# Guillaume-SOULIER/SOS-Radiative-Transfer

Hardware: AMD Instinct MI355X
Metric: SOS columns/sec to 1e-4 convergence (Ntau=200, Nmu=128) (higher is better)
Workload: dtype f64

## Files before the change

__graft_entry__.py:

```python
import os
import subprocess
import sys

ROOT = os.path.dirname(os.path.abspath(__file__))
PKG = os.path.join(ROOT, "sos-radiative-transfer_amd")
CSRC = os.path.join(PKG, "csrc")
LIB = os.path.join(PKG, "libsosrt.so")
SOURCES = ["api.hip", "kernels.hip", "jn_gemm.hip", "jn_gemm_f32.hip", "transport_fast.hip", "transport_ring.hip", "transport_scan.hip", "order_loop.hip", "epilogue.hip", "plan.cpp", "comm.cpp"]
HEADERS = ["kernels.hpp", "plan.hpp", "transport_util.hpp", "transport_scan_body.hpp", "jn_gemm_tile.hpp", "comm.hpp", os.path.join(ROOT, "include", "sosrt.h")]


OBJDIR = os.path.join(PKG, "build")
FLAGS = ["-O3", "--offload-arch=gfx950", "-std=c++17", "-fPIC", "-Wno-unused-value"]


def _deps():
    return [h if os.path.isabs(h) else os.path.join(CSRC, h) for h in HEADERS]


def _obj(src):
    return os.path.join(OBJDIR, src + ".o")


def _obj_stale(src):
    o = _obj(src)
    if not os.path.exists(o):
        return True
    t = os.path.getmtime(o)
    return any(os.path.getmtime(d) > t for d in [os.path.join(CSRC, src)] + _deps())


def _stale():
    if not os.path.exists(LIB):
        return True
    t = os.path.getmtime(LIB)
    deps = [os.path.join(CSRC, s) for s in SOURCES] + _deps()
    return any(os.path.getmtime(d) > t for d in deps)


def _hipcc():
    return os.environ.get("HIPCC") or ("/opt/rocm/bin/hipcc" if os.path.exists("/opt/rocm/bin/hipcc") else "hipcc")


def build(force: bool = False) -> None:
    if force or _stale():
        import fcntl
        with open(os.path.join(PKG, ".build.lock"), "w") as lock:
            fcntl.flock(lock, fcntl.LOCK_EX)
            if force or _stale():
                os.makedirs(OBJDIR, exist_ok=True)
                extra = os.environ.get("SOSRT_CXXFLAGS", "").split()
                todo = [s for s in SOURCES if force or extra or _obj_stale(s)]
                procs = []
                for src in todo:
                    cmd = [_hipcc()] + FLAGS + extra + ["-c", src, "-o", _obj(src)]
                    print("[build]", " ".join(cmd), file=sys.stderr, flush=True)
                    procs.append((src, subprocess.Popen(cmd, cwd=CSRC)))
                bad = [src for src, p in procs if p.wait() != 0]
                if bad:
                    raise RuntimeError("hipcc failed for: " + ", ".join(bad))
                tmp = LIB + ".tmp.%d" % os.getpid()
                cmd = [_hipcc(), "--offload-arch=gfx950", "-shared", "-fPIC", "-o", tmp] + [_obj(s) for s in SOURCES] + ["-ldl"]
# ... 35 lines not shown
```

include/sosrt.h:

```cpp
#ifndef SOSRT_H
#define SOSRT_H

#ifdef __cplusplus
extern "C" {
#endif

typedef struct sosrt_handle sosrt_t;

#define SOSRT_OK              0
#define SOSRT_E_INVALID      -1
#define SOSRT_E_HIP          -2
#define SOSRT_E_STATE        -3
#define SOSRT_E_NOMEM        -4

#define SOSRT_COL_OK           0
#define SOSRT_COL_INDEXERROR   1
#define SOSRT_COL_MAXORDERS    2
#define SOSRT_COL_INTERNAL     3

#define SOSRT_GEOM_THREE_ZONE  0
#define SOSRT_GEOM_SINGLE_SLAB 1

#define SOSRT_SURFACE_NONE       0
#define SOSRT_SURFACE_SPECULAR   1
#define SOSRT_SURFACE_LAMBERTIAN 2
#define SOSRT_SURFACE_LAMBERTIAN_README 3

const char* sosrt_last_error(void);
#define SOSRT_VERSION 105
int sosrt_version(void);

int sosrt_create(int device, int L, int N, int max_batch, int max_orders, sosrt_t** out);
int sosrt_destroy(sosrt_t* h);
int sosrt_set_stream(sosrt_t* h, void* hip_stream);
int sosrt_use_own_stream(sosrt_t* h);
int sosrt_synchronize(sosrt_t* h);
int sosrt_set_saved_orders(sosrt_t* h, int slots);
int sosrt_set_order_budget(sosrt_t* h, int max_orders);

int sosrt_set_grid(sosrt_t* h, const double* mu);
int sosrt_set_phase(sosrt_t* h, const double* P_atm, const double* P_aer);

#define SOSRT_MAX_PHASE_SETS 64
int sosrt_set_phase_sets(sosrt_t* h, const double* P_atm, int S, const double* P_aer );
int sosrt_set_phase_sets_dev(sosrt_t* h, const double* P_atm , int S, const double* d_P_aer );
int sosrt_set_aerosol_sets(sosrt_t* h, int B, int nzmax, const int* zone_set );
int sosrt_phase_sets_info(sosrt_t* h, int* out );

int sosrt_set_atm_phase_sets(sosrt_t* h, int S_atm, const double* P_atm_sets );
int sosrt_set_atmosphere_sets(sosrt_t* h, int B, const int* col_set );
int sosrt_atm_sets_info(sosrt_t* h, int* out );

#define SOSRT_FIRST_ORDER_CODED 0
#define SOSRT_FIRST_ORDER_README 1
int sosrt_set_first_order(sosrt_t* h, int mode);

#define SOSRT_CONTRACT_F64 0
#define SOSRT_CONTRACT_F32 1
#define SOSRT_CONTRACT_F64_FULL 2
#define SOSRT_CONTRACT_F64_DENSE 3
#define SOSRT_SYMMETRY_TOL 1e-12
#define SOSRT_LOWRANK_TOL 1e-12
int sosrt_set_contraction(sosrt_t* h, int mode);

int sosrt_set_order_loop(sosrt_t* h, int mode);
int sosrt_order_loop_stats(sosrt_t* h, int* launches, int* refused, long long* column_orders );
int sosrt_phase_asymmetry(sosrt_t* h, double* asymmetry, int* uses_symmetry);
int sosrt_phase_rank(sosrt_t* h, int* rank, double* residual, int* uses);

int sosrt_set_columns(sosrt_t* h, int B, int geometry, int surface,
                      const int* idx_up, const int* idx_down,
                      const double* mu0, const double* grd_alb,
                      const double* alb_atm, const double* alb_aer,
                      const double* dtau_atm, const double* dtau_aer,
                      const double* tauStar_tot);

#define SOSRT_MAX_ZONES 8
int sosrt_set_columns_zones(sosrt_t* h, int B, int surface, int nzmax, const int* nz, const int* zone_r0, const int* zone_mix,
                            const double* mu0, const double* grd_alb, const double* alb_atm, const double* dtau_atm,
                            const double* zone_alb_aer, const double* zone_dtau_aer, const double* tauStar_tot);

int sosrt_first_order(sosrt_t* h, int B, const double* tau, const double* P0_atm, const double* P0_aer,
                      double* I1_out);
int sosrt_source(sosrt_t* h, int B, const double* In_1, double* Jn_out);
int sosrt_transport(sosrt_t* h, int B, const double* tau, const double* Jn, double* In_out, int* status_out);

int sosrt_solve(sosrt_t* h, int B, const double* tau, const double* P0_atm, const double* P0_aer,
                double tol, const double* I1_in,
                double* I_out, double* I_saved_out, int* n_orders_out, int* status_out);
int sosrt_solve_dev(sosrt_t* h, int B, const double* d_tau, const double* d_P0_atm, const double* d_P0_aer,
                    double tol, const double* d_I1_in,
                    double* d_I_out, double* d_I_saved_out, int* d_n_orders_out, int* d_status_out);
int sosrt_last_solve_stats(sosrt_t* h, int* max_orders_run, long long* sum_orders);

int sosrt_fluxes(sosrt_t* h, int B, const double* tau, const double* I, int beam_norm,
                 double* flux_down, double* flux_up);

int sosrt_epilogue_dev(sosrt_t* h, int B, const double* d_tau, const double* d_I, int beam_norm,
                       const double* d_z_profile, double* d_flux_down, double* d_flux_up, double* d_diffusivity,
                       double* d_heating_rate, double* d_net_toa);
int sosrt_epilogue(sosrt_t* h, int B, int beam_norm, const double* z_profile, double* flux_down, double* flux_up,
                   double* diffusivity, double* heating_rate, double* net_toa);

#define SOSRT_PHASE_ISO       0
#define SOSRT_PHASE_RAYLEIGH  1
#define SOSRT_PHASE_HG        2
#define SOSRT_PHASE_TABLE     3
int sosrt_phase_table(sosrt_t* h, const double* tab_mu, const double* tab_p, int ntab);
int sosrt_phase_table_dev(sosrt_t* h, const double* d_tab_mu, const double* d_tab_p, int ntab);

#define SOSRT_MIE_MAX_X 20000.0
#define SOSRT_MIE_MAX_MX 200000.0
#define SOSRT_MIE_MAX_WORKSPACE (2ull << 30)
int sosrt_mie_ensembles(sosrt_t* h, int S, const double* wl, const double* m_re, const double* m_im, const double* r_m,
                        const double* sig, int nb_radius, double r_min, double r_max, int ntab, double* p_out, double* bulk_out);
int sosrt_mie_ensembles_dev(sosrt_t* h, int S, const double* wl, const double* m_re, const double* m_im, const double* r_m,
                            const double* sig, int nb_radius, double r_min, double r_max, int ntab, double* d_p_out,
                            double* d_bulk_out);
int sosrt_mie_efficiencies(sosrt_t* h, int K, const double* m_re, const double* m_im, const double* x, double* out);
// ... 63 lines not shown
```

sos-radiative-transfer_amd/csrc/api.hip:

```cpp
#include <hip/hip_runtime.h>

#include <algorithm>
#include <cmath>
#include <cstdarg>
#include <cstdio>
#include <cstdlib>
#include <chrono>
#include <cstring>
#include <mutex>
#include <new>
#include <string>
#include <vector>

#include "../../include/sosrt.h"
#include "comm.hpp"
#include "kernels.hpp"
#include "plan.hpp"

using namespace sosrt;

namespace {
thread_local std::string g_err;

int fail(int code, const char* fmt, ...) {
// ... 111 lines not shown
    int mix_groups = 0;
    bool mix_dirty = true;
    double *d_Wmix = nullptr, *d_mixca = nullptr, *d_mixcr = nullptr;
    int* d_mixgroup = nullptr;
    int* d_slabtilegroup = nullptr;
    int contraction = SOSRT_CONTRACT_F64;
    double asymmetry = 0;
    bool sym_ok = false;
    bool sym_dirty = true, symmix_dirty = true, symsets_dirty = true;
    double *d_Wa_s = nullptr, *d_Wr_s = nullptr, *d_Wmix_s = nullptr;
    int lr_rank = -1;
    double lr_residual = 0;
    double *d_lrU = nullptr, *d_lrV = nullptr;
    size_t mixs_capacity = 0;
    float *d_Wa32 = nullptr, *d_Wmix32 = nullptr;
    size_t mix32_capacity = 0;
    bool w32_dirty = true;
    int* d_livelist = nullptr;
    size_t mix_capacity = 0;
    double *d_tau = nullptr, *d_P0a = nullptr, *d_P0r = nullptr;
    double *d_Jn = nullptr, *d_InA = nullptr, *d_InB = nullptr, *d_I = nullptr, *d_E = nullptr;
    int use_etab = 1;
    int *d_active = nullptr, *d_norders = nullptr, *d_status = nullptr, *d_redo = nullptr, *d_erep = nullptr;
    int *d_nactive_sets = nullptr, *d_nactive = nullptr;
    int nactive_set = 0;
    unsigned long long* d_tauhash = nullptr;
    int transport_mode = 3;
    int scan_cols = 200;
    bool ring_ok = false, scan_ok = false, scan_split_ok = false;
    int scan_split = 1;
    int cu_count = 0;
    double* d_scan_scratch = nullptr;
    int* d_scan_sync = nullptr;
    int gemm_tail_cols = 1 << 30;
    double gemm_tail_frac = 0.6;
    int gemm_small_cols = 200;
    int dense_live_list = 1;
    int gemm_regs_cols = -1;
    bool fast_ok = false;
    double* d_ratio = nullptr;
    int* h_pub = nullptr;
    bool need_small = true;
    int pub_seq = 0;
    int last_max_orders = 0;
    long long last_sum_orders = 0;
    Prof prof[kMaxGroups];
    int order_loop = 0;
    double ol_frac = 0.5;
    int* d_olsync = nullptr;
    int* h_oldone = nullptr;
    unsigned long long* d_ollog = nullptr;
    int ol_launches = 0, ol_refused = 0;
    bool ol_group_used[kMaxGroups] = {false, false};
    Rccl::comm_t comm = nullptr;
    int comm_rank = -1, comm_world = 0;
};

namespace {

size_t field_elems(const sosrt_handle* h) { return (size_t)h->max_batch * h->L * h->D; }

template <class T>
int dalloc(T** p, size_t n) {
    hipError_t e = hipMalloc((void**)p, n * sizeof(T));
    if (e != hipSuccess) return fail(SOSRT_E_NOMEM, "hipMalloc of %zu bytes failed: %s", n * sizeof(T), hipGetErrorString(e));
    return 0;
}

void mie_linspace(double a, double b, int n, double* out) {
    if (n == 1) { out[0] = a; return; }
    const double step = (b - a) / (n - 1);
    for (int i = 0; i < n; ++i) {
        volatile double t = i * step;
        out[i] = t + a;
    }
    out[n - 1] = b;
}

bool prof_room(Prof& p) {
    if (p.used + 2 > p.ev.size()) {
        const size_t n0 = p.ev.size();
        p.ev.resize(n0 + 4096);
        for (size_t i = n0; i < p.ev.size(); ++i)
            if (hipEventCreateWithFlags(&p.ev[i], hipEventDisableSystemFence) != hipSuccess) { p.ev.resize(i); break; }
        if (p.used + 2 > p.ev.size()) return false;
    }
    if (p.nint >= p.kind.size()) {
        const size_t n = p.kind.size() + 4096;
        p.kind.resize(n, -1); p.first.resize(n, 0); p.last.resize(n, 0);
    }
    return true;
}
hipStream_t group_stream(sosrt_handle* h, int grp) { return grp == 0 ? h->stream : h->stream2; }
void prof_begin(sosrt_handle* h, int kind, int grp = 0) {
    Prof& p = h->prof[grp];
    p.open = -1;
    if (!p.on || !prof_room(p)) return;
    if (p.adjacent >= 0) {
        p.open = p.adjacent;
    } else {
        p.open = (int)p.used++;
        hipEventRecord(p.ev[p.open], group_stream(h, grp));
    }
}
void prof_end(sosrt_handle* h, int kind, int grp = 0) {
    Prof& p = h->prof[grp];
// ... 138 lines not shown
}

int ensure_matrices(sosrt_handle* h, hipStream_t s) {
    const Grid& g = h->g;
    const size_t per = (size_t)g.Dp * g.Wld;
    const bool mixed = h->mix_groups > 0 && h->mix_dirty;
    if (mixed) {
        prof_break(h);
        const bool sets = h->max_set_used > 0, atm = h->max_atm_used > 0;
        launch_wmix(s, per, h->mix_groups, atm ? h->d_Wasets : h->d_Wa, sets ? h->d_Wrsets : h->d_Wr, h->d_mixca, h->d_mixcr,
                    h->d_Wmix, sets ? h->d_mixset : nullptr, atm ? h->d_mixatm : nullptr);
        h->mix_dirty = false;
        h->symmix_dirty = true;
    }
    if (!use_sym(h)) return 0;
    if (h->sym_dirty) {
        prof_break(h);
        if (!h->d_Wa_s) { if (int e = dalloc(&h->d_Wa_s, per)) return e; }
        if (!h->d_Wr_s) { if (int e = dalloc(&h->d_Wr_s, per)) return e; }
        launch_symfold(s, 1, g.N, g.D, g.Dp, g.Wld, h->d_Wa, h->d_Wa_s);
        launch_symfold(s, 1, g.N, g.D, g.Dp, g.Wld, h->d_Wr, h->d_Wr_s);
        h->sym_dirty = false;
        h->symsets_dirty = true;
    }
    if (h->symsets_dirty && h->nsets > 1 && h->mix_groups == 0 && h->max_set_used > 0) {
        prof_break(h);
        {
            if (per * h->nsets > h->wrsets_s_capacity) {
                if (h->d_Wrsets_s) hipFree(h->d_Wrsets_s);
                h->d_Wrsets_s = nullptr; h->wrsets_s_capacity = 0;
                if (int e = dalloc(&h->d_Wrsets_s, per * h->nsets)) return e;
                h->wrsets_s_capacity = per * h->nsets;
            }
            launch_symfold(s, h->nsets, g.N, g.D, g.Dp, g.Wld, h->d_Wrsets, h->d_Wrsets_s);
        }
        h->symsets_dirty = false;
    }
    if (h->mix_groups > 0 && h->symmix_dirty) {
        prof_break(h);
        const size_t need = per * h->mix_groups;
        if (need > h->mixs_capacity) {
            if (h->d_Wmix_s) hipFree(h->d_Wmix_s);
            h->d_Wmix_s = nullptr; h->mixs_capacity = 0;
            if (int e = dalloc(&h->d_Wmix_s, need)) return e;
            h->mixs_capacity = need;
        }
        launch_symfold(s, h->mix_groups, g.N, g.D, g.Dp, g.Wld, h->d_Wmix, h->d_Wmix_s);
        h->symmix_dirty = false;
    }
    return 0;
}

void run_source(sosrt_handle* h, const double* In_1, double* Jn, const int* active, int tail_cols = 0, int pub_tag = 0,
                int grp = -1, bool all_live = false, bool regs_tile = false, int dense_live_cap = 0) {
    const int g0 = grp < 0 ? 0 : grp, g1 = grp < 0 ? h->ngroups : grp + 1;
    const int pg = grp < 0 ? 0 : grp;
    hipStream_t s = group_stream(h, pg);
    GemmArgs ga;
    ga.A = In_1; ga.Wa = h->d_Wa; ga.Wr = h->d_Wr; ga.ca = h->d_rca; ga.cr = h->d_rcr;
    if (h->nslab > 0) {
        ga.rows_main = h->d_mainrows + h->main_off[g0];
        ga.n_main = h->main_off[g1] - h->main_off[g0];
    } else {
        ga.rows_main = nullptr;
        ga.n_main = (h->gb[g1] - h->gb[g0]) * h->L;
        ga.A = In_1 + (size_t)h->gb[g0] * h->L * h->D;
        Jn += (size_t)h->gb[g0] * h->L * h->D;
        ga.ca = h->d_rca + (size_t)h->gb[g0] * h->L;
        ga.cr = h->d_rcr + (size_t)h->gb[g0] * h->L;
        if (active) active += h->gb[g0];
    }
    ga.rows_slab = h->d_slabrows + h->slab_off[g0]; ga.n_slab = h->slab_off[g1] - h->slab_off[g0];
    ga.D = h->g.D; ga.Dp = h->g.Dp; ga.Wld = h->g.Wld; ga.L = h->L; ga.C = Jn; ga.active = active;
    if (grp >= 0 && h->ngroups > 1) ga.pad_lds = h->coresident_pad;
    if (pub_tag) {
        ga.nactive = h->d_nactive + pg; ga.need_small = h->d_nactive + sosrt_handle::kMaxGroups;
        ga.host_pub = h->h_pub + 8 * pg; ga.tag = pub_tag;
    }
    ga.check_tiles = all_live ? 0 : 1;
    if (ensure_matrices(h, s)) return;
    if (h->mix_groups > 0) {
        ga.Wmix = h->d_Wmix; ga.mix_group = h->d_mixgroup; ga.slab_tile_group = h->d_slabtilegroup + h->slab_off[g0] / 32;
    }
    const bool two_pass_sets = h->mix_groups == 0 && h->max_set_used > 0 && h->nslab > 0;
    if (two_pass_sets) {
        ga.Wr = h->d_Wrsets; ga.mix_group = h->d_mixgroup; ga.slab_tile_group = h->d_slabtilegroup + h->slab_off[g0] / 32;
    }
    if (use_lowrank(h)) { ga.lr_rank = h->lr_rank; ga.lrU = h->d_lrU; ga.lrV = h->d_lrV; }
    AtmSets at;
    const AtmSets* atp = nullptr;
    if (h->max_atm_used > 0) {
        at.col_atm = h->d_colatm + (h->nslab > 0 ? 0 : h->gb[g0]);
        at.lr_ranks = h->d_lrranks;
        ga.lrU = h->d_lrUsets; ga.lrV = h->d_lrVsets;
        atp = &at;
    }
    if (use_sym(h)) {
        ga.sym = 1; ga.Ks = (h->g.N + GEMM_KC - 1) / GEMM_KC * GEMM_KC;
#ifdef SOSRT_DIAG
        if (h->diag_ks_mult > 1 && ga.Ks * h->diag_ks_mult <= h->g.Dp) ga.Ks *= h->diag_ks_mult;
#endif
        ga.Wa = h->d_Wa_s; ga.Wr = two_pass_sets ? h->d_Wrsets_s : h->d_Wr_s;
        if (ga.Wmix) ga.Wmix = h->d_Wmix_s;
    }
    if (h->contraction == SOSRT_CONTRACT_F32) {
        if (h->w32_dirty) {
            prof_break(h);
            const size_t per = (size_t)h->g.Dp * h->g.Wld;
            launch_to_float(s, per, h->d_Wa, h->d_Wa32);
            if (h->mix_groups > 0) launch_to_float(s, per * h->mix_groups, h->d_Wmix, h->d_Wmix32);
            h->w32_dirty = false;
        }
        prof_begin(h, SOSRT_K_GEMM, pg);
        launch_gemm_f32(s, ga, h->d_Wa32, h->d_Wmix32);
        prof_end(h, SOSRT_K_GEMM, pg);
        return;
    }
    prof_begin(h, SOSRT_K_GEMM, pg);
    if (tail_cols > 0 && active && h->nslab >= 0) {
        ga.col0 = h->nslab > 0 ? h->gb[g0] : 0; ga.B = h->gb[g1] - h->gb[g0];
        ga.max_main = h->max_main; ga.max_slab = h->max_slab;
        ga.idx_up = h->nslab > 0 ? h->d_idx_up : nullptr; ga.idx_down = h->nslab > 0 ? h->d_idx_down : nullptr;
        ga.live_list = h->d_livelist + h->gb[g0]; ga.live_cap = tail_cols;
        launch_gemm_tail(s, ga, tail_cols, tail_cols <= h->gemm_small_cols, regs_tile, atp);
    } else {
        if (dense_live_cap > 0 && active && h->nslab >= 0) {
            ga.col0 = h->nslab > 0 ? h->gb[g0] : 0; ga.B = h->gb[g1] - h->gb[g0];
            ga.live_list = h->d_livelist + h->gb[g0]; ga.live_cap = dense_live_cap;
        }
        launch_gemm(s, ga, atp);
    }
    prof_end(h, SOSRT_K_GEMM, pg);
}

struct SolveShape {
    bool ring_like = false;
    bool fast = false;
    int nzcap = kRingZones;
    int ring_mode = 1;
};
SolveShape solve_shape(const sosrt_handle* h, int max_nz) {
    SolveShape sh;
    sh.ring_like = h->transport_mode >= 2 && h->ring_ok && (max_nz <= kRingZones || transport_ring_fits(h->g, max_nz));
    sh.fast = h->transport_mode >= 1 && h->fast_ok && (max_nz <= kRingZones || sh.ring_like);
    sh.nzcap = max_nz > kRingZones ? max_nz : kRingZones;
    sh.ring_mode = (h->transport_mode >= 2 && h->ring_ok) ? 3 : 1;
    return sh;
}
struct OrderInputs {
    int nb = 0;
    int known = 0;
    int surface = SOSRT_SURFACE_NONE;
    bool simple_zones = true;
    bool slabs_mixed = true;
    bool need_small = false;
    bool saving = false;
    int orders_left = 1 << 30;
    int cu_share = 0;
};
struct LaunchPlan {
    int tail_cols = 0;
    int live_cap = 0;
    int gemm = SOSRT_PLAN_GEMM_DENSE;
    int transport = SOSRT_PLAN_TRANSPORT_GENERAL;
    int parts = 1;
    int repair = 0;
    int order_loop = 0;
    int ol_parts = 0;
    int ol_grid = 0;
};
LaunchPlan plan_order(const sosrt_handle* h, const SolveShape& sh, const OrderInputs& in) {
    LaunchPlan pl;
    const Grid& g = h->g;
    const bool live_tiling = h->contraction != SOSRT_CONTRACT_F32 && in.simple_zones && in.known <= h->gemm_tail_cols &&
                             (in.known <= h->gemm_tail_frac * in.nb || in.nb <= h->gemm_small_cols) &&
                             (in.known < in.nb || in.nb <= h->gemm_small_cols);
    pl.tail_cols = live_tiling ? in.known : 0;
    pl.gemm = !live_tiling ? SOSRT_PLAN_GEMM_DENSE
                           : (pl.tail_cols <= h->gemm_small_cols ? ((use_sym(h) && pl.tail_cols <= 32) ? SOSRT_PLAN_GEMM_LIVE32_DEEP : SOSRT_PLAN_GEMM_LIVE32)
                                                                 : SOSRT_PLAN_GEMM_LIVE64);
    {
        const int nct = (g.D + GEMM_BN - 1) / GEMM_BN;
        const int auto_cap = (3 * h->cu_count / 2) / (((g.L + 15) / 16 + 1) * nct);
        const int cap = h->gemm_regs_cols >= 0 ? h->gemm_regs_cols : auto_cap;
        if (live_tiling && use_sym(h) && pl.tail_cols <= cap && 16 * (g.D + 2) * 8 <= 150 * 1024 &&
            ((g.N + GEMM_KC - 1) / GEMM_KC * GEMM_KC) % 64 == 0) pl.gemm = SOSRT_PLAN_GEMM_LIVE16_REGS;
    }
    pl.live_cap = live_tiling ? pl.tail_cols : ((h->contraction != SOSRT_CONTRACT_F32 && h->dense_live_list && in.known < in.nb) ? in.known : 0);
    {
        const int cols_now = pl.live_cap > 0 ? pl.live_cap : in.nb;
        const int split_cap = sh.ring_mode == 3 ? h->cu_count : 4 * h->cu_count;
        const bool can_split = h->scan_split && h->scan_split_ok && transport_scan_parts(g) * cols_now <= split_cap &&
                               (in.surface == SOSRT_SURFACE_SPECULAR || in.surface == SOSRT_SURFACE_NONE);
        const bool want_scan = h->transport_mode == 4 || (h->transport_mode == 3 && cols_now <= h->scan_cols);
        const bool split = can_split && transport_scan_fits(g, sh.nzcap, true) && (sh.fast || (h->use_etab && h->transport_mode >= 3));
        const bool scan = want_scan && ((sh.fast && sh.ring_mode == 3 && h->scan_ok && transport_scan_fits(g, sh.nzcap, false)) || split);
        pl.transport = scan ? SOSRT_PLAN_TRANSPORT_SCAN
                            : (!sh.fast ? SOSRT_PLAN_TRANSPORT_GENERAL : (sh.ring_mode == 3 ? SOSRT_PLAN_TRANSPORT_RING : SOSRT_PLAN_TRANSPORT_FAST));
        if (scan && split) pl.parts = transport_scan_parts(g);
        pl.repair = (h->N - 3 > 61 && pl.transport == SOSRT_PLAN_TRANSPORT_FAST) ? 1 : 0;
    }
    if (h->order_loop && in.cu_share > 0 && h->transport_mode == 3 && sh.fast && sh.ring_mode == 3 && sh.nzcap <= kRingZones &&
        use_sym(h) && in.simple_zones && in.slabs_mixed && !in.saving && !in.need_small && in.orders_left >= 1 &&
        in.known <= kOrderLoopMaxCols) {
        Grid gt = g;
        gt.nsmall = 0;
        const bool split_ok = h->scan_split && (in.surface == SOSRT_SURFACE_SPECULAR || in.surface == SOSRT_SURFACE_NONE) && order_loop_ok(gt, true);
        const int sp = order_loop_parts(gt, true);
        if (split_ok && sp * in.known <= h->ol_frac * in.cu_share) {
            pl.order_loop = 1; pl.ol_parts = sp;
        } else if (order_loop_ok(gt, false) && in.known <= h->ol_frac * in.cu_share) {
            pl.order_loop = 1; pl.ol_parts = 1;
        }
        if (pl.order_loop) pl.ol_grid = in.cu_share;
    }
    return pl;
}

std::mutex g_ol_mutex;
int g_ol_held[64];
int ol_acquire(int device, int total, int want, int least) {
    if (device < 0 || device >= 64) return 0;
    std::lock_guard<std::mutex> lk(g_ol_mutex);
    int got = total - g_ol_held[device];
    if (got > want) got = want;
    if (got < least || got <= 0) return 0;
    g_ol_held[device] += got;
    return got;
}
void ol_release(int device, int n) {
    if (device < 0 || device >= 64 || n <= 0) return;
    std::lock_guard<std::mutex> lk(g_ol_mutex);
    g_ol_held[device] -= n;
}

}

extern "C" {

const char* sosrt_last_error(void) { return g_err.c_str(); }
int sosrt_version(void) { return SOSRT_VERSION; }

int sosrt_plan_fix_count(double tau_ref, int N) { return fix_count(tau_ref, N); }

int sosrt_create(int device, int L, int N, int max_batch, int max_orders, sosrt_t** out) {
    if (!out) return fail(SOSRT_E_INVALID, "out is null");
    *out = nullptr;
    if (L < 2) return fail(SOSRT_E_INVALID, "nb_layers must be >= 2 (got %d)", L);
    if (N < 4) return fail(SOSRT_E_INVALID, "nb_angles must be >= 4 (got %d)", N);
    if (N > 1024) return fail(SOSRT_E_INVALID, "nb_angles must be <= 1024 (got %d)", N);
    if (max_batch < 1 || max_orders < 1) return fail(SOSRT_E_INVALID, "max_batch and max_orders must be >= 1");
    {
        const int nt = (N + 63) / 64 * 64;
        const size_t need = (size_t)(3 * (size_t)L + nt + nt / 64 + 4) * sizeof(double);
        if (need > 64 * 1024)
            return fail(SOSRT_E_INVALID, "nb_layers = %d does not fit: at most %d layers at nb_angles = %d", L,
                        (int)((64 * 1024 / sizeof(double) - nt - nt / 64 - 4) / 3), N);
    }
    sosrt_handle* h = new (std::nothrow) sosrt_handle();
    if (!h) return fail(SOSRT_E_NOMEM, "out of host memory");
    h->device = device; h->L = L; h->N = N; h->D = 2 * N; h->max_batch = max_batch; h->max_orders = max_orders;
    h->order_budget = max_orders;
    h->saved_slots = max_orders;
    h->gpu = device >= 0;
    h->cu_count = 256;
    if (const char* ev = getenv("SOSRT_ETAB")) h->use_etab = atoi(ev);
    if (const char* ev = getenv("SOSRT_CONTRACT"))
        if (strcmp(ev, "full") == 0) h->contraction = SOSRT_CONTRACT_F64_FULL;
    if (const char* ev = getenv("SOSRT_TRANSPORT"))
        h->transport_mode = strcmp(ev, "general") == 0 ? 0 : (strcmp(ev, "ring") == 0 ? 2 : (strcmp(ev, "scan") == 0 ? 4 : (strcmp(ev, "auto") == 0 ? 3 : 1)));
    if (const char* ev = getenv("SOSRT_SCAN_COLS")) h->scan_cols = atoi(ev);
    if (const char* ev = getenv("SOSRT_SCAN_SPLIT")) h->scan_split = atoi(ev);
    if (const char* ev = getenv("SOSRT_GEMM_TAIL")) h->gemm_tail_cols = atoi(ev);
    if (const char* ev = getenv("SOSRT_GEMM_TAIL_FRAC")) h->gemm_tail_frac = atof(ev);
    if (const char* ev = getenv("SOSRT_GEMM_SMALL")) h->gemm_small_cols = atoi(ev);
    if (const char* ev = getenv("SOSRT_DENSE_LIVE_LIST")) h->dense_live_list = atoi(ev) != 0;
    if (const char* ev = getenv("SOSRT_GEMM_REGS")) h->gemm_regs_cols = atoi(ev);
    if (const char* ev = getenv("SOSRT_GROUPS")) h->want_groups = atoi(ev) >= 2 ? 2 : (atoi(ev) == 1 ? 1 : 0);
    if (const char* ev = getenv("SOSRT_SPLIT_MIN")) h->split_min = atoi(ev);
    if (const char* ev = getenv("SOSRT_MIX_GROUPS")) h->mix_groups_max = atoi(ev);
#ifdef SOSRT_DIAG
    if (const char* ev = getenv("SOSRT_STAGGER")) h->stagger = atof(ev);
    if (const char* ev = getenv("SOSRT_GROUP_SPLIT")) h->split_at = atoi(ev);
    if (const char* ev = getenv("SOSRT_GROUP_PRIO")) h->prio2 = atoi(ev);
    if (const char* ev = getenv("SOSRT_GEMM_PAD_LDS")) h->coresident_pad = atoi(ev);
    if (const char* ev = getenv("SOSRT_GEMM_KS_MULT")) h->diag_ks_mult = atoi(ev);
#endif
    if (const char* ev = getenv("SOSRT_GROUP_RING_SLOTS")) h->coresident_slots = atoi(ev);
    if (const char* ev = getenv("SOSRT_ORDER_LOOP")) h->order_loop = atoi(ev) != 0;
    if (const char* ev = getenv("SOSRT_RING_SLOTS")) g_ring_slots = atoi(ev);
#ifdef SOSRT_RING_DEBUG
    if (const char* ev = getenv("SOSRT_RING_DEBUG")) g_ring_debug = atoi(ev);
#endif
    Grid& g = h->g;
    g.L = L; g.N = N; g.D = 2 * N;
    g.Dp = (g.D + GEMM_KC - 1) / GEMM_KC * GEMM_KC;
    g.Wld = (g.D + GEMM_BN - 1) / GEMM_BN * GEMM_BN;
    if (h->gpu) {
        int e = 0;
        auto body = [&]() -> int {
            HIPCHK(hipSetDevice(device));
            HIPCHK(hipStreamCreateWithFlags(&h->own_stream, hipStreamDefault));
            h->stream = h->own_stream;
            HIPCHK(hipEventCreateWithFlags(&h->ev_fork, hipEventDisableTiming));
            HIPCHK(hipEventCreateWithFlags(&h->ev_join, hipEventDisableTiming));
            const size_t mb = max_batch, fe = field_elems(h);
            if ((e = dalloc(&h->d_mu, g.D))) return e;
            if ((e = dalloc(&h->d_Wa, (size_t)g.Dp * g.Wld))) return e;
            if ((e = dalloc(&h->d_Wr, (size_t)g.Dp * g.Wld))) return e;
            if ((e = dalloc(&h->d_lrU, (size_t)kLowRankMax * g.D))) return e;
            if ((e = dalloc(&h->d_lrV, (size_t)kLowRankMax * g.D))) return e;
            if ((e = dalloc(&h->d_wfdn, N))) return e;
            if ((e = dalloc(&h->d_wfup, N))) return e;
            if ((e = dalloc(&h->d_w, g.D))) return e;
            if ((e = dalloc(&h->d_phi, 2 * kNPhi))) return e;
            if ((e = dalloc(&h->d_z, L))) return e;
            if ((e = dalloc(&h->d_fix, 4))) return e;
            if ((e = dalloc(&h->d_small, N))) return e;
            if ((e = dalloc(&h->d_idx_up, mb))) return e;
            if ((e = dalloc(&h->d_idx_down, mb))) return e;
            if ((e = dalloc(&h->d_nz, mb))) return e;
            if ((e = dalloc(&h->d_zr0, mb * kMaxZones))) return e;
            if ((e = dalloc(&h->d_zmix, mb * kMaxZones))) return e;
            if ((e = dalloc(&h->d_zwr, mb * kMaxZones))) return e;
            if ((e = dalloc(&h->d_zdtr, mb * kMaxZones))) return e;
            if ((e = dalloc(&h->d_scal, 7 * mb))) return e;
            if ((e = dalloc(&h->d_desc, mb))) return e;
            if ((e = dalloc(&h->d_rca, mb * L))) return e;
            if ((e = dalloc(&h->d_rcr, mb * L))) return e;
            if ((e = dalloc(&h->d_slabrows, mb * L + 64 * (size_t)sosrt_handle::kMaxMixGroupsSets * sosrt_handle::kMaxGroups))) return e;
            if ((e = dalloc(&h->d_slabtilegroup, mb * L / 32 + 2 * sosrt_handle::kMaxMixGroupsSets * sosrt_handle::kMaxGroups + 2))) return e;
            if ((e = dalloc(&h->d_mainrows, mb * L))) return e;
            if ((e = dalloc(&h->d_tau, mb * L))) return e;
            if ((e = dalloc(&h->d_P0a, mb * g.D))) return e;
            if ((e = dalloc(&h->d_P0r, mb * g.D))) return e;
            if ((e = dalloc(&h->d_Jn, fe))) return e;
            if ((e = dalloc(&h->d_InA, fe))) return e;
            if ((e = dalloc(&h->d_InB, fe))) return e;
            if ((e = dalloc(&h->d_I, fe))) return e;
            if ((e = dalloc(&h->d_E, fe))) return e;
            if ((e = dalloc(&h->d_active, mb))) return e;
            if ((e = dalloc(&h->d_norders, mb))) return e;
            if ((e = dalloc(&h->d_status, mb))) return e;
            if ((e = dalloc(&h->d_nactive_sets, 2 * (sosrt_handle::kMaxGroups + 1)))) return e;
            HIPCHK(hipMemset(h->d_nactive_sets, 0, 2 * (sosrt_handle::kMaxGroups + 1) * sizeof(int)));
            h->d_nactive = h->d_nactive_sets;
            if ((e = dalloc(&h->d_redo, mb))) return e;
            if ((e = dalloc(&h->d_erep, mb))) return e;
            if ((e = dalloc(&h->d_mixgroup, mb))) return e;
            if ((e = dalloc(&h->d_livelist, mb))) return e;
            if ((e = dalloc(&h->d_mixca, sosrt_handle::kMaxMixGroupsSets))) return e;
            if ((e = dalloc(&h->d_mixcr, sosrt_handle::kMaxMixGroupsSets))) return e;
            if ((e = dalloc(&h->d_mixset, sosrt_handle::kMaxMixGroupsSets))) return e;
            if ((e = dalloc(&h->d_mixatm, sosrt_handle::kMaxMixGroupsSets))) return e;
            if ((e = dalloc(&h->d_colatm, mb))) return e;
            if ((e = dalloc(&h->d_tauhash, mb))) return e;
            if ((e = dalloc(&h->d_ratio, mb))) return e;
            if ((e = dalloc(&h->d_scan_scratch, mb * transport_scan_scratch_doubles()))) return e;
            if ((e = dalloc(&h->d_scan_sync, 2 * mb))) return e;
            if ((e = dalloc(&h->d_olsync, sosrt_handle::kMaxGroups * order_loop_sync_ints(kOrderLoopMaxCols)))) return e;
            HIPCHK(hipHostMalloc((void**)&h->h_oldone, 2 * sosrt_handle::kMaxGroups * sizeof(int), hipHostMallocCoherent));
            memset(h->h_oldone, 0, 2 * sosrt_handle::kMaxGroups * sizeof(int));
            HIPCHK(hipMemset(h->d_scan_sync, 0, 2 * mb * sizeof(int)));
            HIPCHK(hipDeviceGetAttribute(&h->cu_count, hipDeviceAttributeMultiprocessorCount, device));
            HIPCHK(hipHostMalloc((void**)&h->h_pub, (8 * sosrt_handle::kMaxGroups + 2) * sizeof(int), hipHostMallocCoherent));
            memset(h->h_pub, 0, (8 * sosrt_handle::kMaxGroups + 2) * sizeof(int));

            HIPCHK(hipMemset(h->d_Wa, 0, (size_t)g.Dp * g.Wld * sizeof(double)));
            HIPCHK(hipMemset(h->d_Wr, 0, (size_t)g.Dp * g.Wld * sizeof(double)));
            HIPCHK(hipMemset(h->d_status, 0, mb * sizeof(int)));
            HIPCHK(hipMemset(h->d_redo, 0, mb * sizeof(int)));
            HIPCHK(hipMemset(h->d_tau, 0, mb * L * sizeof(double)));
            return 0;
        };
        if ((e = body())) { sosrt_destroy(h); return e; }
        g.mu = h->d_mu; g.Wa = h->d_Wa; g.Wr = h->d_Wr; g.fix = h->d_fix; g.small_lanes = h->d_small;
        g.wflux_dn = h->d_wfdn; g.wflux_up = h->d_wfup; g.nsmall = 0;
    }
    *out = h;
    return 0;
}

int sosrt_destroy(sosrt_t* h) {
    if (!h) return 0;
    if (h->gpu) {
        hipSetDevice(h->device);
        if (h->comm) { rccl().CommDestroy(h->comm); h->comm = nullptr; }
        if (h->own_stream) hipStreamSynchronize(h->own_stream);
        void* ptrs[] = {h->d_mu, h->d_Wa, h->d_Wr, h->d_wfdn, h->d_wfup, h->d_fix, h->d_small, h->d_idx_up,
                        h->d_idx_down, h->d_scal, h->d_desc, h->d_rca, h->d_rcr, h->d_slabrows, h->d_mainrows, h->d_tau, h->d_P0a,
                        h->d_P0r, h->d_Jn, h->d_InA, h->d_InB, h->d_I, h->d_E, h->d_active, h->d_norders, h->d_status,
                        h->d_nactive_sets, h->d_ratio, h->d_redo, h->d_erep, h->d_tauhash, h->d_Wmix, h->d_mixca, h->d_mixcr,
                        h->d_mixgroup, h->d_Wa_s, h->d_Wr_s, h->d_Wmix_s, h->d_scan_scratch, h->d_scan_sync, h->d_w, h->d_phi, h->d_z, h->d_tab, h->d_slabtilegroup, h->d_livelist, h->d_Wa32, h->d_Wmix32, h->d_nz, h->d_zr0, h->d_zmix, h->d_zwr, h->d_zdtr, h->d_olsync, h->d_ollog, h->d_modetab, h->d_lrU, h->d_lrV, h->d_Wrsets, h->d_Wrsets_s, h->d_mixset, h->d_P0rz,
                        h->d_Wasets, h->d_lrUsets, h->d_lrVsets, h->d_lrranks, h->d_colatm, h->d_mixatm};
        for (void* p : ptrs)
            if (p) hipFree(p);
        if (h->h_pub) hipHostFree(h->h_pub);
        if (h->h_oldone) hipHostFree(h->h_oldone);
        if (h->d_mie) hipFree(h->d_mie);
        if (h->h_mie) hipHostFree(h->h_mie);
        if (h->mie_ev) hipEventDestroy(h->mie_ev);
        for (auto& e : h->mie_t)
            if (e) hipEventDestroy(e);

        for (auto& p : h->prof)
            for (auto& e : p.ev) hipEventDestroy(e);
        if (h->stream2) { hipStreamSynchronize(h->stream2); hipStreamDestroy(h->stream2); }
        if (h->ev_fork) hipEventDestroy(h->ev_fork);
        if (h->ev_join) hipEventDestroy(h->ev_join);
        if (h->own_stream) hipStreamDestroy(h->own_stream);
    }
    delete h;
    return 0;
}

int sosrt_set_stream(sosrt_t* h, void* s) {
    if (int e = need_gpu(h)) return e;
    h->stream = (hipStream_t)s;
    return 0;
}

int sosrt_use_own_stream(sosrt_t* h) {
    if (int e = need_gpu(h)) return e;
    h->stream = h->own_stream;
    return 0;
}

int sosrt_set_saved_orders(sosrt_t* h, int slots) {
    if (!h) return fail(SOSRT_E_INVALID, "null handle");
    if (slots < 1 || slots > h->max_orders) return fail(SOSRT_E_INVALID, "slots must be in 1..max_orders=%d (got %d)", h->max_orders, slots);
    h->saved_slots = slots;
    return 0;
}

int sosrt_set_order_budget(sosrt_t* h, int max_orders) {
    if (!h) return fail(SOSRT_E_INVALID, "null handle");
    if (max_orders < 1 || max_orders > h->max_orders)
        return fail(SOSRT_E_INVALID, "the order budget must be in 1..max_orders=%d of sosrt_create (got %d)", h->max_orders, max_orders);
    h->order_budget = max_orders;
    return 0;
}

int sosrt_set_first_order(sosrt_t* h, int mode) {
    if (int e = need_gpu(h)) return e;
    if (mode != SOSRT_FIRST_ORDER_CODED && mode != SOSRT_FIRST_ORDER_README) return fail(SOSRT_E_INVALID, "unknown first-order mode %d", mode);
    if (mode == SOSRT_FIRST_ORDER_README && (h->nsets > 1 || h->p0_zones > 0))
        return fail(SOSRT_E_INVALID, "SOSRT_FIRST_ORDER_README reads one aerosol matrix: it cannot be combined with several phase sets");
    if (mode == SOSRT_FIRST_ORDER_README && (h->natm > 1 || h->max_atm_used > 0))
        return fail(SOSRT_E_INVALID, "SOSRT_FIRST_ORDER_README reads one atmosphere matrix: it cannot be combined with atmosphere phase sets");
    if (mode == SOSRT_FIRST_ORDER_README && h->geom != SOSRT_GEOM_THREE_ZONE)
        return fail(SOSRT_E_INVALID, "the README's Lambertian first order needs the three-zone geometry (it has a surface)");
    h->first_order_mode = mode;
    return 0;
}

int sosrt_set_contraction(sosrt_t* h, int mode) {
    if (int e = need_gpu(h)) return e;
    if (mode != SOSRT_CONTRACT_F64 && mode != SOSRT_CONTRACT_F32 && mode != SOSRT_CONTRACT_F64_FULL && mode != SOSRT_CONTRACT_F64_DENSE) return fail(SOSRT_E_INVALID, "unknown contraction mode %d", mode);
    if (mode != SOSRT_CONTRACT_F64 && (h->natm > 1 || h->max_atm_used > 0))
        return fail(SOSRT_E_INVALID, "atmosphere phase sets are in use: their plain rows exist in the low-rank form of SOSRT_CONTRACT_F64 only "
                                     "(the other contractions tile row lists that straddle columns)");
    if (mode == SOSRT_CONTRACT_F32) {
        HIPCHK(hipSetDevice(h->device));
        const size_t per = (size_t)h->g.Dp * h->g.Wld;
        if (!h->d_Wa32) { if (int e = dalloc(&h->d_Wa32, per)) return e; }
        h->w32_dirty = true;
    }
    h->contraction = mode;
    return 0;
}

int sosrt_set_order_loop(sosrt_t* h, int mode) {
    if (!h) return fail(SOSRT_E_INVALID, "null handle");
    if (mode < 0 || mode > 2) return fail(SOSRT_E_INVALID, "order-loop mode must be 0, 1 or 2 (got %d)", mode);
    h->order_loop = mode;
    return 0;
}

int sosrt_order_loop_stats(sosrt_t* h, int* launches, int* refused, long long* column_orders) {
    if (!h) return fail(SOSRT_E_INVALID, "null handle");
    if (launches) *launches = h->ol_launches;
    if (refused) *refused = h->ol_refused;
    if (column_orders) {
        *column_orders = 0;
        if (h->gpu && h->ol_launches > 0) {
            HIPCHK(hipSetDevice(h->device));
            HIPCHK(hipStreamSynchronize(h->stream));
            if (h->stream2) HIPCHK(hipStreamSynchronize(h->stream2));
            for (int k = 0; k < sosrt_handle::kMaxGroups; ++k) {
                if (!h->ol_group_used[k]) continue;
                int v = 0;
                HIPCHK(hipMemcpy(&v, h->d_olsync + (size_t)k * order_loop_sync_ints(kOrderLoopMaxCols) + kOlOrders, sizeof v, hipMemcpyDeviceToHost));
                *column_orders += v;
            }
        }
    }
    return 0;
}

int sosrt_plan_launch(sosrt_t* h, int batch, int live, int surface, int zones, int cus, int* out) {
    if (!h || !out) return fail(SOSRT_E_INVALID, "null argument");
    if (!h->have_grid) return fail(SOSRT_E_STATE, "sosrt_set_grid has not been called");
    if (batch < 1 || live < 0 || live > batch) return fail(SOSRT_E_INVALID, "need 0 <= live <= batch, batch >= 1");
    if (zones < 1 || zones > kMaxZones) return fail(SOSRT_E_INVALID, "zones must be in 1..%d", kMaxZones);
    int want = h->want_groups;
    if (want == 0) want = batch > h->split_min ? 2 : 1;
    const int ng = (want >= 2 && batch >= h->split_min && batch >= 2) ? 2 : 1;
    const int nb = ng == 2 ? batch / 2 : batch;
    const int saved_cus = h->cu_count;
    if (cus > 0) h->cu_count = cus;
    const SolveShape sh = solve_shape(h, zones);
    OrderInputs oi;
    oi.nb = nb; oi.known = live < nb ? live : nb; oi.surface = surface;
    oi.simple_zones = zones == 3 || zones == 1;
    oi.cu_share = h->cu_count / ng;
    const bool saved_sym = h->sym_ok;
    if (!h->have_phase) h->sym_ok = true;
    const LaunchPlan pl = plan_order(h, sh, oi);
    h->sym_ok = saved_sym;
    h->cu_count = saved_cus;
    out[0] = ng; out[1] = pl.gemm; out[2] = pl.tail_cols; out[3] = pl.transport; out[4] = pl.parts; out[5] = pl.repair;
    out[6] = pl.order_loop; out[7] = pl.ol_parts; out[8] = pl.ol_grid;
    return 0;
}

int sosrt_phase_asymmetry(sosrt_t* h, double* asymmetry, int* uses_symmetry) {
    if (!h) return fail(SOSRT_E_INVALID, "null handle");
    if (!h->have_phase) return fail(SOSRT_E_STATE, "sosrt_set_phase has not been called");
    if (asymmetry) *asymmetry = h->asymmetry;
    if (uses_symmetry) *uses_symmetry = use_sym(h) ? 1 : 0;
    return 0;
}

int sosrt_phase_rank(sosrt_t* h, int* rank, double* residual, int* uses) {
    if (!h) return fail(SOSRT_E_INVALID, "null handle");
    if (!h->have_phase) return fail(SOSRT_E_STATE, "sosrt_set_phase has not been called");
    if (rank) *rank = h->lr_rank;
    if (residual) *residual = h->lr_residual;
    if (uses) *uses = use_lowrank(h) ? 1 : 0;
    return 0;
}

int sosrt_synchronize(sosrt_t* h) {
    if (int e = need_gpu(h)) return e;
    HIPCHK(hipStreamSynchronize(h->stream));
    return 0;
}

int sosrt_set_grid(sosrt_t* h, const double* mu) {
// ... 279 lines not shown
    if (h->ngroups > 1 && !h->stream2) {
        HIPCHK(hipSetDevice(h->device));
        if (h->prio2) {
            int least = 0, greatest = 0;
            HIPCHK(hipDeviceGetStreamPriorityRange(&least, &greatest));
            HIPCHK(hipStreamCreateWithPriority(&h->stream2, hipStreamNonBlocking, h->prio2 > 0 ? greatest : least));
        } else {
            HIPCHK(hipStreamCreateWithFlags(&h->stream2, hipStreamNonBlocking));
        }
    }
    h->gb[0] = 0; h->gb[1] = h->ngroups == 2 ? ((h->split_at > 0 && h->split_at < B) ? h->split_at : B / 2) : B; h->gb[2] = B;
    for (int k = 0; k <= sosrt_handle::kMaxGroups; ++k) { h->main_off[k] = 0; h->slab_off[k] = 0; }
    h->max_nz = 1;
    h->simple_zones = true;
    if (geometry == SOSRT_GEOM_THREE_ZONE) {
        for (int b = 0; b < B; ++b) {
            h->max_nz = nz[b] > h->max_nz ? nz[b] : h->max_nz;
            const int* m = &zmix[b * kMaxZones];
            if (!(nz[b] == 3 && m[0] == 0 && m[1] == 1 && m[2] == 0)) h->simple_zones = false;
            if (nz[b] == 3) { iup[b] = zr0[b * kMaxZones + 1]; idn[b] = zr0[b * kMaxZones + 2] - 1; }
        }
        for (int k = 0; k < h->ngroups; ++k) {
            for (int b = h->gb[k]; b < h->gb[k + 1]; ++b)
                for (int z = 0; z < nz[b]; ++z)
                    for (int t = zr0[b * kMaxZones + z]; t <= zone_end(b, z); ++t) (zmix[b * kMaxZones + z] ? slab : plain).push_back(b * L + t);
            h->main_off[k + 1] = (int)plain.size();
            h->slab_off[k + 1] = (int)slab.size();
        }
    }
    for (int b = 0; b < B; ++b) {
        if (!(mu0[b] > 0)) return fail(SOSRT_E_INVALID, "column %d: mu0 must be > 0", b);
        sc[0 * mb + b] = mu0[b];
        sc[1 * mb + b] = grd_alb ? grd_alb[b] : 0.0;
        sc[2 * mb + b] = alb_atm[b];
        sc[4 * mb + b] = dtau_atm ? dtau_atm[b] : 1.0;
        sc[6 * mb + b] = tauStar_tot[b];
    }
    HIPCHK(hipSetDevice(h->device));
    HIPCHK(hipMemcpyAsync(h->d_scal, sc.data(), 7 * mb * sizeof(double), hipMemcpyHostToDevice, h->stream));
    if (geometry == SOSRT_GEOM_THREE_ZONE) {
        HIPCHK(hipMemcpyAsync(h->d_nz, nz.data(), B * sizeof(int), hipMemcpyHostToDevice, h->stream));
        HIPCHK(hipMemcpyAsync(h->d_zr0, zr0.data(), (size_t)B * kMaxZones * sizeof(int), hipMemcpyHostToDevice, h->stream));
        HIPCHK(hipMemcpyAsync(h->d_zmix, zmix.data(), (size_t)B * kMaxZones * sizeof(int), hipMemcpyHostToDevice, h->stream));
        HIPCHK(hipMemcpyAsync(h->d_zwr, zwr.data(), (size_t)B * kMaxZones * sizeof(double), hipMemcpyHostToDevice, h->stream));
        HIPCHK(hipMemcpyAsync(h->d_zdtr, zdtr.data(), (size_t)B * kMaxZones * sizeof(double), hipMemcpyHostToDevice, h->stream));
        HIPCHK(hipMemcpyAsync(h->d_idx_up, iup.data(), B * sizeof(int), hipMemcpyHostToDevice, h->stream));
        HIPCHK(hipMemcpyAsync(h->d_idx_down, idn.data(), B * sizeof(int), hipMemcpyHostToDevice, h->stream));
        if (!slab.empty())
            HIPCHK(hipMemcpyAsync(h->d_slabrows, slab.data(), slab.size() * sizeof(int), hipMemcpyHostToDevice, h->stream));
        if (!plain.empty())
            HIPCHK(hipMemcpyAsync(h->d_mainrows, plain.data(), plain.size() * sizeof(int), hipMemcpyHostToDevice, h->stream));
    }
    HIPCHK(hipStreamSynchronize(h->stream));
    h->nslab = (int)slab.size();
    h->nmain = (int)plain.size();
    h->max_main = L; h->max_slab = 0;
    if (geometry == SOSRT_GEOM_THREE_ZONE) {
        h->max_main = 0;
        for (int b = 0; b < B; ++b) {
            int ns = 0;
            for (int z = 0; z < nz[b]; ++z)
                if (zmix[b * kMaxZones + z]) ns += zone_end(b, z) - zr0[b * kMaxZones + z] + 1;
            h->max_slab = ns > h->max_slab ? ns : h->max_slab;
            h->max_main = L - ns > h->max_main ? L - ns : h->max_main;
        }
    }
    h->mix_groups = 0;
    h->mix_dirty = true;
    h->w32_dirty = true;
    h->max_set_used = 0;
    h->max_atm_used = 0;
    h->c_atmset.assign(B, 0);
    h->p0_zones = 0;
    h->c_nz = nz; h->c_zr0 = zr0; h->c_zmix = zmix; h->c_zwr = zwr; h->c_zdtr = zdtr;
    h->c_zset.assign((size_t)B * kMaxZones, 0);
    h->c_alb_atm.assign(alb_atm, alb_atm + B);
    h->c_dtau_atm.assign(B, 1.0);
    if (dtau_atm) h->c_dtau_atm.assign(dtau_atm, dtau_atm + B);
    if (geometry == SOSRT_GEOM_THREE_ZONE && h->nslab > 0) {
        MixGroups mg;
        if (collect_mix_groups(h, B, h->c_zset, h->c_atmset, mix_group_cap(h, false), mg))
            if (int e = apply_mix_groups(h, B, mg)) return e;
    }
    h->B = B; h->geom = geometry; h->surface = surface;
    h->have_cols = true;
    return 0;
}

int sosrt_set_columns(sosrt_t* h, int B, int geometry, int surface, const int* idx_up, const int* idx_down,
                      const double* mu0, const double* grd_alb, const double* alb_atm, const double* alb_aer,
                      const double* dtau_atm, const double* dtau_aer, const double* tauStar_tot) {
    if (int e = need_gpu(h)) return e;
    if (B < 1 || B > h->max_batch) return fail(SOSRT_E_INVALID, "B=%d outside 1..max_batch=%d", B, h->max_batch);
    if (!mu0 || !alb_atm || !tauStar_tot) return fail(SOSRT_E_INVALID, "mu0, alb_atm and tauStar_tot are required");
    std::vector<int> nz(B, 1), zr0((size_t)B * kMaxZones, 0), zmix((size_t)B * kMaxZones, 0);
    std::vector<double> zwr((size_t)B * kMaxZones, 0.0), zdtr((size_t)B * kMaxZones, 0.0);
    if (geometry == SOSRT_GEOM_THREE_ZONE) {
        if (!idx_up || !idx_down || !grd_alb || !alb_aer || !dtau_atm || !dtau_aer)
            return fail(SOSRT_E_INVALID, "three-zone geometry needs idx_up, idx_down, grd_alb, alb_aer, dtau_atm, dtau_aer");
        if (surface != SOSRT_SURFACE_SPECULAR && surface != SOSRT_SURFACE_LAMBERTIAN && surface != SOSRT_SURFACE_LAMBERTIAN_README)
            return fail(SOSRT_E_INVALID, "three-zone geometry needs a specular or lambertian surface");
        for (int b = 0; b < B; ++b) {
            if (idx_up[b] < 1 || idx_down[b] < idx_up[b] || idx_down[b] > h->L - 2)
                return fail(SOSRT_E_INVALID, "column %d: need 1 <= idx_up <= idx_down <= nb_layers-2 (got %d, %d)", b,
                            idx_up[b], idx_down[b]);
            nz[b] = 3;
// ... 377 lines not shown
    if (int e = ensure_w32(h)) return e;
    hipStream_t s = h->stream;
    const Grid& g = h->g;
    const size_t LD = (size_t)h->L * h->D;
    const size_t saved_stride = (size_t)h->saved_slots * LD;
    const int NG = h->ngroups;

    prof_break(h);
    h->nactive_set ^= 1;
    h->d_nactive = h->d_nactive_sets + h->nactive_set * (sosrt_handle::kMaxGroups + 1);
    SolveSetup su;
    su.zero_next = h->d_nactive_sets + (h->nactive_set ^ 1) * (sosrt_handle::kMaxGroups + 1);
    su.n_zero = sosrt_handle::kMaxGroups + 1;
    su.redo = h->d_redo;
    su.hash = h->d_tauhash;
    su.scan_sync = h->d_scan_sync;
    launch_prepare(s, g, B, h->geom, h->surface, scalars_of(h), d_tau, h->d_desc, h->d_rca, h->d_rcr,
                   h->d_nactive + sosrt_handle::kMaxGroups, su);
    h->need_small = true;
    const int small_tag = ((++h->pub_seq) & 0x3fffffff) | 0x40000000;
    bool small_published = false;
    const SolveShape shape = solve_shape(h, h->max_nz);
    const bool fast = shape.fast;
    const int nzcap = shape.nzcap;
    if (h->use_etab || fast) {
        launch_tau_groups(s, g, B, d_tau, h->d_tauhash, h->d_erep, h->d_nactive + sosrt_handle::kMaxGroups,
                          h->h_pub + 8 * sosrt_handle::kMaxGroups, small_tag);
        launch_attenuation(s, g, B, d_tau, h->d_E, h->d_erep);
        small_published = true;
    }
    if (int e = ensure_matrices(h, s)) return e;
    bool forked = false;
    int ol_held[sosrt_handle::kMaxGroups] = {0, 0};
    auto bail = [&](int code) {
        if (forked && hipEventRecord(h->ev_join, h->stream2) == hipSuccess) (void)hipStreamWaitEvent(s, h->ev_join, 0);
        for (int k = 0; k < NG; ++k)
            if (ol_held[k]) {
                (void)hipStreamSynchronize(group_stream(h, k));
                ol_release(h->device, ol_held[k]);
                ol_held[k] = 0;
            }
        return code;
    };

    struct GroupState {
        int b0 = 0, nb = 0, n = 1, known = 0;
        bool done = false, started = false;
        bool ol_pending = false, ol_off = false;
        int ol_tag = 0;
        unsigned ol_polls = 0;
        double *In_1 = nullptr, *In = nullptr;
        Conv cv;
    } gs[sosrt_handle::kMaxGroups];
    h->ol_launches = 0; h->ol_refused = 0;
    for (bool& u : h->ol_group_used) u = false;
    bool used_order_loop = false;
    const int tagbase = ((++h->pub_seq) & 0x3fff) << 16;
    for (int k = 0; k < NG; ++k) {
        GroupState& q = gs[k];
        q.b0 = h->gb[k]; q.nb = h->gb[k + 1] - h->gb[k]; q.known = q.nb;
        q.In_1 = h->d_InA; q.In = h->d_InB;
        if (!d_I1_in && h->first_order_mode != SOSRT_FIRST_ORDER_README) q.In_1 = d_I_out;
        q.cv = make_conv(h, tol);
        q.cv.active += q.b0; q.cv.norders += q.b0; q.cv.status += q.b0; q.cv.ratio += q.b0; q.cv.redo += q.b0;
        q.cv.nactive = h->d_nactive + k;
        if (h->d_targets) q.cv.target = h->d_targets + q.b0;
    }
    auto start_group = [&](int k) {
        GroupState& q = gs[k];
        q.started = true;
        hipStream_t sg = group_stream(h, k);
        const size_t fo = (size_t)q.b0 * LD;
        prof_begin(h, SOSRT_K_FIRST, k);
        if (d_I1_in)
            hipLaunchKernelGGL(k_init_from_I1, dim3(q.nb), dim3(256), 0, sg, g, d_I1_in + fo, q.In_1 + fo, d_I_out + fo,
                               d_I_saved_out ? d_I_saved_out + (size_t)q.b0 * saved_stride : nullptr, saved_stride, q.cv);
        else if (h->first_order_mode == SOSRT_FIRST_ORDER_README)
            launch_first_order_readme(sg, g, h->d_w, q.nb, d_tau + (size_t)q.b0 * h->L, d_P0_atm + (size_t)q.b0 * g.D,
                                      d_P0_aer ? d_P0_aer + (size_t)q.b0 * g.D : nullptr, h->d_desc + q.b0, q.In_1 + fo,
                                      d_I_out + fo, d_I_saved_out ? d_I_saved_out + (size_t)q.b0 * saved_stride : nullptr,
                                      saved_stride, q.cv, 1);
        else
            launch_first_order(sg, g, q.nb, d_tau + (size_t)q.b0 * h->L, d_P0_atm + (size_t)q.b0 * g.D,
                               d_P0_aer ? d_P0_aer + (size_t)q.b0 * g.D * (h->p0_zones > 0 ? h->p0_zones : 1) : nullptr, h->d_desc + q.b0,
                               d_I_out + fo, nullptr, d_I_saved_out ? d_I_saved_out + (size_t)q.b0 * saved_stride : nullptr, saved_stride,
                               q.cv, 1, h->p0_zones);
        prof_end(h, SOSRT_K_FIRST, k);
    };
    start_group(0);
    if (NG > 1) {
        HIPCHK(hipEventRecord(h->ev_fork, s));
        HIPCHK(hipStreamWaitEvent(h->stream2, h->ev_fork, 0));
        forked = true;
    }
    if (small_published && g.nsmall > 0) {
        volatile int* slot = h->h_pub + 8 * sosrt_handle::kMaxGroups;
        const auto t0 = std::chrono::steady_clock::now();
        for (unsigned it = 1; __atomic_load_n(&slot[1], __ATOMIC_ACQUIRE) != small_tag; ++it) {
            if ((it & 0x3fff) == 0 && std::chrono::steady_clock::now() - t0 > std::chrono::seconds(120))
                return bail(fail(SOSRT_E_HIP, "order loop: no progress for 120 s"));
            __builtin_ia32_pause();
        }
        h->need_small = slot[0] != 0;
    }
    int live_groups = NG, n_max = 1;
    while (live_groups > 0) {
        bool progressed = false;
// ... 19 lines not shown
                if (h->d_ollog && getenv("SOSRT_OL_LOG")) {
                    std::vector<unsigned long long> lg(65001);
                    (void)hipStreamSynchronize(group_stream(h, k));
                    (void)hipMemcpy(lg.data(), h->d_ollog, lg.size() * 8, hipMemcpyDeviceToHost);
                    if (FILE* f = fopen(getenv("SOSRT_OL_LOG"), "a")) {
                        fprintf(f, "# launch columns<=%d order0=%d events=%llu\n", q.known, q.n + 1, lg[0]);
                        for (unsigned long long i = 0; i < lg[0] && i < 65000; ++i)
                            fprintf(f, "%llu %llu %llu %llu\n", lg[1 + i] >> 48, (lg[1 + i] >> 40) & 0xff, (lg[1 + i] >> 32) & 0xff, lg[1 + i] & 0xffffffffull);
                        fclose(f);
                    }
                }
#endif
                if (state == kOlReady) { q.done = true; --live_groups; h->ol_group_used[k] = true; continue; }
                if (state == kOlAborted) {
                    std::vector<int> w(order_loop_sync_ints(q.known < 6 ? q.known : 6));
                    (void)hipStreamSynchronize(group_stream(h, k));
                    (void)hipMemcpy(w.data(), h->d_olsync + (size_t)k * order_loop_sync_ints(kOrderLoopMaxCols), w.size() * sizeof(int), hipMemcpyDeviceToHost);
                    std::string cols;
                    for (int c = 0; c < (q.known < 6 ? q.known : 6); ++c) {
                        char buf[96];
                        const int* cs = w.data() + kOlCols + c * kOlColStride;
                        snprintf(buf, sizeof buf, " [%d: orders %d stop %d tiles %d]", c, cs[kOlOrdDone], cs[kOlColStop], cs[kOlJnDone]);
                        cols += buf;
                    }
                    return bail(fail(SOSRT_E_HIP, "order loop: a workgroup of the order-loop launch gave up waiting (arrived %d, left %d, order %d on, %d columns:%s)",
                                     w[kOlArrive], w[kOlLeft], q.n + 1, q.known, cols.c_str()));
                }
                q.ol_off = true;
                ++h->ol_refused;
            }
            if (!q.started) {
                const GroupState& p = gs[k - 1];
                if (!(p.done || (p.n >= 2 && p.known <= h->stagger * p.nb))) continue;
                start_group(k);
            }
            progressed = true;
            if (q.n >= h->order_budget) { q.done = true; --live_groups; continue; }
            if (q.n >= 2) {
                const int live = wait_published(h, k, tagbase + q.n - 1);
                if (live < 0) return bail(live);
                if (live == 0) { q.done = true; --live_groups; continue; }
                q.known = live;
            }
            hipStream_t sg = group_stream(h, k);
            const size_t fo = (size_t)q.b0 * LD;
            const double* tau_g = d_tau + (size_t)q.b0 * h->L;
            const int* erep_g = h->d_erep + q.b0;
            OrderInputs oi;
            oi.nb = q.nb; oi.known = q.known; oi.surface = h->surface;
            oi.simple_zones = h->simple_zones; oi.slabs_mixed = h->nslab == 0 || h->mix_groups > 0;
            oi.need_small = g.nsmall > 0 && h->need_small; oi.saving = d_I_saved_out != nullptr;
            oi.orders_left = h->order_budget - q.n;
            oi.cu_share = (q.ol_off || h->d_targets || h->max_atm_used > 0) ? 0 : h->cu_count / NG;
            LaunchPlan pl = plan_order(h, shape, oi);
            if (pl.order_loop) {
                const int got = ol_acquire(h->device, h->cu_count, pl.ol_grid, (int)(pl.ol_parts * q.known / h->ol_frac));
                if (got == 0) { oi.cu_share = 0; pl = plan_order(h, shape, oi); }
                else { pl.ol_grid = got; ol_held[k] = got; }
            }
            if (pl.order_loop && h->order_loop == 2) pl.ol_grid = 2 * h->cu_count;
            if (pl.order_loop) {
                OrderLoopArgs oa;
                Grid gt = g;
                gt.nsmall = 0;
                oa.t = TransportArgs{gt, tau_g, h->d_Jn + fo, nullptr, d_I_out + fo, nullptr, 0, h->d_desc + q.b0, q.cv, 0, 1, h->d_E, erep_g, nullptr};
                oa.t.nzcap = kRingZones;
                oa.t.scan_split = pl.ol_parts > 1 ? 1 : 0;
                oa.t.scan_scratch = h->d_scan_scratch + (size_t)q.b0 * transport_scan_scratch_doubles();
                oa.t.scan_sync = h->d_scan_sync + 2 * q.b0;
                GemmArgs& ga = oa.gm;
                ga.A = nullptr; ga.Wa = h->d_Wa_s; ga.Wr = h->d_Wr_s; ga.ca = h->d_rca; ga.cr = h->d_rcr;
                ga.D = g.D; ga.Dp = g.Dp; ga.Wld = g.Wld; ga.L = h->L; ga.C = h->d_Jn;
                ga.sym = 1; ga.Ks = (g.N + GEMM_KC - 1) / GEMM_KC * GEMM_KC;
                if (use_lowrank(h)) { ga.lr_rank = h->lr_rank; ga.lrU = h->d_lrU; ga.lrV = h->d_lrV; }
                ga.max_main = h->max_main; ga.max_slab = h->max_slab;
                ga.idx_up = h->nslab > 0 ? h->d_idx_up : nullptr; ga.idx_down = h->nslab > 0 ? h->d_idx_down : nullptr;
                if (h->mix_groups > 0) { ga.Wmix = h->d_Wmix_s; ga.mix_group = h->d_mixgroup; }
                oa.in0 = q.In_1;
                oa.gbufP = q.In;
                oa.gbufQ = (q.In_1 == d_I_out) ? h->d_InA : q.In_1;
                oa.bufP = oa.gbufP + fo; oa.bufQ = oa.gbufQ + fo;
                oa.order0 = q.n + 1; oa.kmax = h->order_budget - q.n;
                oa.B = q.nb; oa.col0 = q.b0;
                oa.fixcap = (int)(0.06 * g.N) + 1;
                oa.sync = h->d_olsync + (size_t)k * order_loop_sync_ints(kOrderLoopMaxCols);
                oa.host_done = h->h_oldone + 2 * k;
                oa.tag = q.ol_tag = ((++h->pub_seq) & 0x3fffffff) | 0x40000000;
#ifdef SOSRT_OL_STAMPS
                if (getenv("SOSRT_OL_LOG")) {
                    if (!h->d_ollog) { if (int e = dalloc(&h->d_ollog, 65001)) return bail(e); }
                    HIPCHK(hipMemsetAsync(h->d_ollog, 0, 8, sg));
                    oa.log = h->d_ollog;
                }
#endif
                prof_break(h);
                HIPCHK(hipMemsetAsync(oa.sync, 0, order_loop_sync_ints(q.known) * sizeof(int), sg));
                prof_begin(h, SOSRT_K_ORDER_LOOP, k);
                const hipError_t le = launch_order_loop(sg, pl.ol_grid, pl.ol_parts > 1, oa);
                prof_end(h, SOSRT_K_ORDER_LOOP, k);
                if (le != hipSuccess) return bail(fail(SOSRT_E_HIP, "order-loop launch failed: %s", hipGetErrorString(le)));
                q.ol_pending = true;
                used_order_loop = true;
                ++h->ol_launches;
                continue;
            }
            const int n = ++q.n;
            n_max = n > n_max ? n : n_max;
            const int tail_cols = pl.tail_cols;
            run_source(h, q.In_1, h->d_Jn, h->d_active, tail_cols, tagbase + n - 1, k, q.known == q.nb, pl.gemm == SOSRT_PLAN_GEMM_LIVE16_REGS,
                       tail_cols > 0 ? 0 : pl.live_cap);
            if (g.nsmall > 0 && h->need_small) {
                prof_begin(h, SOSRT_K_SMALLMU, k);
                launch_smallmu(sg, g, q.nb, tau_g, h->d_Jn + fo, q.In + fo, h->d_desc + q.b0, q.cv.active);
                prof_end(h, SOSRT_K_SMALLMU, k);
            }
            prof_begin(h, SOSRT_K_TRANSPORT, k);
            double* sv_n = (d_I_saved_out && n <= h->saved_slots) ? d_I_saved_out + (size_t)q.b0 * saved_stride + (size_t)(n - 1) * LD : nullptr;
            if (pl.transport != SOSRT_PLAN_TRANSPORT_GENERAL) {
                Grid gt = g;
                if (pl.transport >= SOSRT_PLAN_TRANSPORT_RING && !h->need_small) gt.nsmall = 0;
                launch_transport(sg, gt, q.nb, tau_g, h->d_Jn + fo, q.In + fo, d_I_out + fo, sv_n, saved_stride, h->d_desc + q.b0, q.cv, n, 1,
                                 h->d_E, pl.transport, erep_g, pl.live_cap, h->d_livelist + q.b0, NG > 1 ? h->coresident_slots : 0,
                                 pl.parts > 1 ? 1 : 0, h->d_scan_scratch + (size_t)q.b0 * transport_scan_scratch_doubles(),
                                 h->d_scan_sync + 2 * q.b0, nzcap);
                if (pl.repair)
                    launch_transport(sg, g, q.nb, tau_g, h->d_Jn + fo, q.In + fo, d_I_out + fo, sv_n, saved_stride, h->d_desc + q.b0, q.cv, n, 1,
                                     h->d_E, 2, erep_g);
            } else {
                launch_transport(sg, g, q.nb, tau_g, h->d_Jn + fo, q.In + fo, d_I_out + fo, sv_n, saved_stride, h->d_desc + q.b0, q.cv, n, 1,
                                 h->use_etab ? h->d_E : nullptr, 0, erep_g);
            }
            prof_end(h, SOSRT_K_TRANSPORT, k);
            if (q.In_1 == d_I_out) { q.In_1 = q.In; q.In = h->d_InA; }
            else { double* tmp = q.In_1; q.In_1 = q.In; q.In = tmp; }
        }
        if (!progressed) __builtin_ia32_pause();
    }
    if (NG > 1) {
        HIPCHK(hipEventRecord(h->ev_join, h->stream2));
        HIPCHK(hipStreamWaitEvent(s, h->ev_join, 0));
    }
    prof_break(h);
    launch_finalize(s, B, make_conv(h, tol), h->order_budget, d_n_orders_out, d_status_out);
    HIPCHK(hipGetLastError());
    h->last_max_orders = used_order_loop ? -1 : n_max;
    h->last_sum_orders = -1;
    return 0;
}

int sosrt_solve(sosrt_t* h, int B, const double* tau, const double* P0_atm, const double* P0_aer, double tol,
                const double* I1_in, double* I_out, double* I_saved_out, int* n_orders_out, int* status_out) {
    if (int e = check_ready(h, B, true)) return e;
    if (!tau) return fail(SOSRT_E_INVALID, "null argument");
    HIPCHK(hipSetDevice(h->device));
    hipStream_t s = h->stream;
    h->resident = false;
    const size_t LD = (size_t)h->L * h->D, n = (size_t)B * LD;
    HIPCHK(hipMemcpyAsync(h->d_tau, tau, (size_t)B * h->L * sizeof(double), hipMemcpyHostToDevice, s));
    if (P0_atm) HIPCHK(hipMemcpyAsync(h->d_P0a, P0_atm, (size_t)B * h->D * sizeof(double), hipMemcpyHostToDevice, s));
    const double* d_p0r = nullptr;
    if (int e = stage_p0_aer(h, B, P0_aer, s, &d_p0r)) return e;
    double* d_I1 = nullptr;
    double* d_saved = nullptr;
    int rc = 0;
    auto body = [&]() -> int {
        if (I1_in) {
            if (int e = dalloc(&d_I1, n)) return e;
            HIPCHK(hipMemcpyAsync(d_I1, I1_in, n * sizeof(double), hipMemcpyHostToDevice, s));
        }
        if (I_saved_out) {
            if (int e = dalloc(&d_saved, (size_t)B * h->saved_slots * LD)) return e;
            HIPCHK(hipMemsetAsync(d_saved, 0, (size_t)B * h->saved_slots * LD * sizeof(double), s));
        }
        if (int e = sosrt_solve_dev(h, B, h->d_tau, P0_atm ? h->d_P0a : nullptr, d_p0r, tol, d_I1,
                                    h->d_I, d_saved, nullptr, nullptr))
            return e;
        if (I_out) HIPCHK(hipMemcpyAsync(I_out, h->d_I, n * sizeof(double), hipMemcpyDeviceToHost, s));
// ... 792 lines not shown
```

sos-radiative-transfer_amd/csrc/jn_gemm_tile.hpp:

```cpp
#pragma once
#include "kernels.hpp"
#include "transport_util.hpp"

namespace sosrt {

namespace {

typedef double f64x4 __attribute__((ext_vector_type(4)));

constexpr int A_LD = GEMM_KC + 2;
constexpr int B_LD = GEMM_BN + 16;

struct ListRows {
    const int* rows;
    int n;
    __device__ int operator()(int lr) const { return lr < n ? (rows ? rows[lr] : lr) : -1; }
};
struct ColumnRows {
    int base, iu, ns, n;
    bool slab;
    __device__ int operator()(int lr) const {
        if (lr >= n) return -1;
        return base + (slab ? iu + lr : (lr < iu ? lr : lr + ns));
    }
};

template <int RT, bool SLAB, bool DEEP = false, bool SYM = false, class RowOf = ListRows, bool COH = false, bool ASTAGE = false>
__device__ __forceinline__ void gemm_tile(const GemmArgs& g, double* sA, double* sB, int* s_any, int tile, int bn0,
                                          RowOf row_of, bool check_active, const double* __restrict__ wmix = nullptr,
                                          double* sRaw = nullptr) {
    static_assert(!ASTAGE || (COH && DEEP), "ASTAGE is a form of the order-loop launch's tile");
    constexpr int BM = 16 * RT;
    double* const sAv = sA + BM * A_LD;
    const int Nn = g.D >> 1, Nh = g.Wld >> 1;
    int tid_ = threadIdx.x;
    if (COH) asm volatile("" : "+v"(tid_));
    const int tid = tid_, lane = tid & 63;
    const int wave = __builtin_amdgcn_readfirstlane(tid) >> 6;
    const int D = g.D, Dp = g.Dp, Wld = g.Wld;
    constexpr bool slab = SLAB;
    const int bm0 = tile * BM;

    const int arow = tid >> 2, akq = (tid & 3) * (GEMM_KC / 4);
    int grow = -1;
    if (arow < BM) grow = row_of(bm0 + arow);
    if (check_active && g.active && g.check_tiles) {
        if (tid == 0) *s_any = 0;
        __syncthreads();
        if ((tid & 3) == 0 && grow >= 0 && g.active[grow / g.L]) *s_any = 1;
        __syncthreads();
        if (!*s_any) return;
    }
    __shared__ int s_rowid[16 * (GEMM_RT > 2 ? GEMM_RT : 2)];
    if ((tid & 3) == 0 && arow < BM) s_rowid[arow] = grow;
// ... 323 lines not shown
        const int r = rows[i] >= 0 ? rows[i] : rows[0];
        const int bytes = rows[i] >= 0 ? D * 8 : 0;
        rA[i] = make_rsrc(g.A + (size_t)r * D, bytes);
        rC[i] = make_rsrc(g.C + (size_t)r * D, bytes);
        cf[i] = rows[i] >= 0 ? g.ca[rows[i]] : 0.0;
        if constexpr (ATM) {
            const int st = __builtin_amdgcn_readfirstlane(at.col_atm[r / g.L]);
            Ri[i] = __builtin_amdgcn_readfirstlane(at.lr_ranks[st]);
            Ui[i] = g.lrU + (size_t)st * kLowRankMax * D;
            Vi[i] = g.lrV + (size_t)st * kLowRankMax * D;
        }
    }
    const double* __restrict__ U = g.lrU;
    const double* __restrict__ V = g.lrV;
    double m[LR_ROWS][kLowRankMax];
#pragma unroll
    for (int i = 0; i < LR_ROWS; ++i)
#pragma unroll
        for (int q = 0; q < kLowRankMax; ++q) m[i][q] = 0.0;
#pragma unroll 2
    for (int k = 2 * lane; k < D; k += 128) {
        double2 x[LR_ROWS];
#pragma unroll
        for (int i = 0; i < LR_ROWS; ++i) x[i] = bload2_aux<COH ? 16 : 0>(rA[i], k * 8, 0);
#pragma unroll
        for (int q = 0; q < kLowRankMax; ++q) {
            if constexpr (ATM) {
#pragma unroll
                for (int i = 0; i < LR_ROWS; ++i)
                    if (q < Ri[i]) {
                        const double2 u = *reinterpret_cast<const double2*>(Ui[i] + (size_t)q * D + k);
                        m[i][q] = __builtin_fma(x[i].y, u.y, __builtin_fma(x[i].x, u.x, m[i][q]));
                    }
            } else if (q < R) {
                const double2 u = *reinterpret_cast<const double2*>(U + (size_t)q * D + k);
#pragma unroll
                for (int i = 0; i < LR_ROWS; ++i) m[i][q] = __builtin_fma(x[i].y, u.y, __builtin_fma(x[i].x, u.x, m[i][q]));
            }
        }
    }
#pragma unroll
    for (int s = 32; s >= 1; s >>= 1)
#pragma unroll
        for (int q = 0; q < kLowRankMax; ++q) {
            if constexpr (ATM) {
#pragma unroll
                for (int i = 0; i < LR_ROWS; ++i)
                    if (q < Ri[i]) m[i][q] += __shfl_xor(m[i][q], s);
            } else if (q < R) {
#pragma unroll
                for (int i = 0; i < LR_ROWS; ++i) m[i][q] += __shfl_xor(m[i][q], s);
            }
        }
#pragma unroll 2
    for (int k = 2 * lane; k < D; k += 128) {
        double2 o[LR_ROWS];
#pragma unroll
        for (int i = 0; i < LR_ROWS; ++i) o[i] = make_double2(0.0, 0.0);
#pragma unroll
        for (int q = 0; q < kLowRankMax; ++q) {
            if constexpr (ATM) {
#pragma unroll
                for (int i = 0; i < LR_ROWS; ++i)
                    if (q < Ri[i]) {
                        const double2 v = *reinterpret_cast<const double2*>(Vi[i] + (size_t)q * D + k);
                        o[i].x = __builtin_fma(m[i][q], v.x, o[i].x);
                        o[i].y = __builtin_fma(m[i][q], v.y, o[i].y);
                    }
            } else if (q < R) {
                const double2 v = *reinterpret_cast<const double2*>(V + (size_t)q * D + k);
#pragma unroll
                for (int i = 0; i < LR_ROWS; ++i) {
                    o[i].x = __builtin_fma(m[i][q], v.x, o[i].x);
                    o[i].y = __builtin_fma(m[i][q], v.y, o[i].y);
                }
            }
        }
#pragma unroll
        for (int i = 0; i < LR_ROWS; ++i) bstore2_aux<COH ? 17 : 0>(rC[i], k * 8, 0, make_double2(cf[i] * o[i].x, cf[i] * o[i].y));
    }
}
template <bool COH, class RowOf, bool ATM = false>
__device__ __forceinline__ void lowrank_tile(const GemmArgs& g, RowOf row_of, int tile, int BM, int bn0, bool check_active,
                                             const AtmSets& at = AtmSets()) {
    const int nct = (g.D + GEMM_BN - 1) / GEMM_BN, ct = bn0 / GEMM_BN;
    const int lane = threadIdx.x & 63, wave = __builtin_amdgcn_readfirstlane(threadIdx.x) >> 6;
    const int per = (BM - ct + nct - 1) / nct;
    const bool chk = check_active && g.active && g.check_tiles;
    for (int j = LR_ROWS * wave; j < per; j += 4 * LR_ROWS) {
        int rows[LR_ROWS];
        int n = 0;
#pragma unroll
        for (int i = 0; i < LR_ROWS; ++i) {
            int r = j + i < per ? __builtin_amdgcn_readfirstlane(row_of(tile * BM + ct + nct * (j + i))) : -1;
            if (chk && r >= 0 && !g.active[r / g.L]) r = -1;
            rows[i] = r;
            n += r >= 0 ? 1 : 0;
        }
        if (n == 0) continue;
        if (rows[0] < 0)
#pragma unroll
            for (int i = 1; i < LR_ROWS; ++i)
                if (rows[i] >= 0) { rows[0] = rows[i]; rows[i] = -1; break; }
        lowrank_rows<COH, ATM>(g, rows, lane, at);
    }
}

constexpr int TAIL_RT_SLAB = 1;
constexpr int TAIL_RT = 2;

}
}
```

sos-radiative-transfer_amd/csrc/kernels.hip:

```cpp
#include <cstdlib>

#include "kernels.hpp"

#include "../../include/sosrt.h"

namespace sosrt {


typedef double f64x4 __attribute__((ext_vector_type(4)));

#define SOSRT_PI 3.14159265358979323846

__device__ __forceinline__ double wave_fmax(double v) {
#pragma unroll
    for (int o = 32; o > 0; o >>= 1) v = fmax(v, __shfl_xor(v, o, 64));
    return v;
}
__device__ __forceinline__ double wave_sum(double v) {
#pragma unroll
    for (int o = 32; o > 0; o >>= 1) v += __shfl_xor(v, o, 64);
    return v;
}

__device__ double block_pymax(double x, bool valid, double* s_red, int first_tid = 0) {
// ... 957 lines not shown
            bool same = true;
            for (int i = lane; i < L; i += 64) same = same && (tb[i] == tc[i]);
            if (__ballot(!same) == 0) rep = cc;
        }
    }
    if (lane == 0) erep[b] = rep;
}
void launch_tau_groups(hipStream_t s, const Grid& g, int B, const double* tau, unsigned long long* hash, int* erep,
                       const int* need_small, int* host_flag, int tag) {
    hipLaunchKernelGGL(k_tau_rep, dim3(B), dim3(64), 0, s, g.L, tau, hash, erep, need_small, host_flag, tag);
}

template <int MAXT>
static void launch_transport_t(hipStream_t s, dim3 grid, dim3 block, size_t shm, const TransportArgs& a, int mode) {
    if (mode == 1) {
        launch_transport_fast(s, grid, block, a);
    } else if (mode == 3) {
        launch_transport_ring(s, grid, a, g_ring_slots);
    } else if (mode == 4) {
        launch_transport_scan(s, grid, a);
    } else if (mode == 2) {
        if (a.accumulate) {
            if (a.saved) hipLaunchKernelGGL((k_transport<MAXT, true, true, true, true>), grid, block, shm, s, a);
            else hipLaunchKernelGGL((k_transport<MAXT, true, false, true, true>), grid, block, shm, s, a);
        } else {
            hipLaunchKernelGGL((k_transport<MAXT, false, false, true, true>), grid, block, shm, s, a);
        }
    } else if (a.accumulate) {
        if (a.Etab) {
            if (a.saved) hipLaunchKernelGGL((k_transport<MAXT, true, true, true>), grid, block, shm, s, a);
            else hipLaunchKernelGGL((k_transport<MAXT, true, false, true>), grid, block, shm, s, a);
        } else {
            if (a.saved) hipLaunchKernelGGL((k_transport<MAXT, true, true, false>), grid, block, shm, s, a);
            else hipLaunchKernelGGL((k_transport<MAXT, true, false, false>), grid, block, shm, s, a);
        }
    } else {
        if (a.Etab) hipLaunchKernelGGL((k_transport<MAXT, false, false, true>), grid, block, shm, s, a);
        else hipLaunchKernelGGL((k_transport<MAXT, false, false, false>), grid, block, shm, s, a);
    }
}

unsigned long long* g_transport_stamps = nullptr;
int g_ring_slots = 3, g_ring_debug = 0;

bool transport_fast_ok(const Plan& plan) {
    for (int bkt = 0; bkt < 4; ++bkt)
        if (plan.fix[bkt].idx > 0 && (plan.fix[bkt].s0 >> 6) != ((plan.N - 1) >> 6)) return false;
    return true;
}

void launch_transport(hipStream_t s, const Grid& g, int B, const double* tau, const double* Jn, double* In, double* I,
                      double* saved, size_t saved_col_stride, const ColDesc* desc, Conv cv, int order,
                      int accumulate, const double* Etab, int mode, const int* erep, int live, const int* live_list,
                      int ring_slots, int scan_split, double* scan_scratch, int* scan_sync, int nzcap) {
    const int nt = round64(g.N);
    const size_t shm = (size_t)(g.L + 2 * TC * (nt + 2) + 2 * nt + nt / 64 + 2) * sizeof(double);
    TransportArgs a{g, tau, Jn, In, I, accumulate ? saved : nullptr, saved_col_stride, desc, cv, order, accumulate, Etab, Etab ? erep : nullptr, g_transport_stamps};
    a.slots = ring_slots;
    a.nzcap = nzcap > kRingZones ? nzcap : kRingZones;
    if (mode == 4 && scan_split && scan_scratch && scan_sync) { a.scan_split = 1; a.scan_scratch = scan_scratch; a.scan_sync = scan_sync; }
    if ((mode == 3 || mode == 4) && accumulate && live > 0 && live < B && live_list) {
        a.live = live;
        a.live_list = live_list;
        B = live;
    }
    if (nt <= 128) launch_transport_t<128>(s, dim3(B), dim3(nt), shm, a, mode);
    else if (nt <= 256) launch_transport_t<256>(s, dim3(B), dim3(nt), shm, a, mode);
    else if (nt <= 512) launch_transport_t<512>(s, dim3(B), dim3(nt), shm, a, mode);
    else launch_transport_t<1024>(s, dim3(B), dim3(nt), shm, a, mode);
}

__global__ void k_finalize(int B, Conv cv, int max_orders, int* __restrict__ n_out, int* __restrict__ status_out) {
    const int b = blockIdx.x * blockDim.x + threadIdx.x;
    if (b >= B) return;
    int st = cv.status[b];
    if (cv.active[b]) { st = SOSRT_COL_MAXORDERS; cv.status[b] = st; }
    if (n_out) n_out[b] = cv.norders[b];
    if (status_out) status_out[b] = st;
}
void launch_finalize(hipStream_t s, int B, Conv cv, int max_orders, int* n_out, int* status_out) {
    hipLaunchKernelGGL(k_finalize, dim3((B + 127) / 128), dim3(128), 0, s, B, cv, max_orders, n_out, status_out);
}

__global__ void k_fluxes(Grid g, int B, const double* __restrict__ tau_all, const double* __restrict__ I_all,
                         const ColDesc* __restrict__ desc, int beam_norm, double* __restrict__ fdn,
                         double* __restrict__ fup) {
    const int row = blockIdx.x * (blockDim.x >> 6) + (threadIdx.x >> 6);
    if (row >= B * g.L) return;
    const int lane = threadIdx.x & 63, b = row / g.L, t = row % g.L;
    const double* I = I_all + (size_t)row * g.D;
    double sd = 0, su = 0;
    for (int k = lane; k < g.N; k += 64) {
        sd += g.wflux_dn[k] * I[k];
        su += g.wflux_up[k] * I[g.N + k];
    }
    sd = wave_sum(sd);
    su = wave_sum(su);
    if (lane == 0) {
        const ColDesc& d = desc[b];
        const double* tau = tau_all + (size_t)b * g.L;
        const double F0 = SOSRT_PI / d.mu0;
        const double fb = beam_norm ? F0 : F0 / (4 * SOSRT_PI);
        fdn[row] = sd - fb * exp(-tau[t] / d.mu0);
        fup[row] = su + fb * d.rho * exp(-(2 * tau[g.L - 1] - tau[t]) / d.mu0);
    }
}
void launch_fluxes(hipStream_t s, const Grid& g, int B, const double* tau, const double* I, const ColDesc* desc,
                   int beam_norm, double* fdn, double* fup) {
    const int rows = B * g.L;
    hipLaunchKernelGGL(k_fluxes, dim3((rows + 3) / 4), dim3(256), 0, s, g, B, tau, I, desc, beam_norm, fdn, fup);
}

// ... 103 lines not shown
```

sos-radiative-transfer_amd/csrc/kernels.hpp:

```cpp
#pragma once
#include <hip/hip_runtime.h>

#include "plan.hpp"

namespace sosrt {

constexpr int kMaxZones = 8;
constexpr int kRingZones = 3;

struct alignas(16) ColDesc {
    int nz;
    int r0[kMaxZones];
    int r1[kMaxZones];
    int mix[kMaxZones];
    int nfix[kMaxZones];
    int fixtab[kMaxZones];
    int surface;
    int geom;
    double mu0, rho, T, tau_bottom;
    double wa;
    double wr[kMaxZones];
    double fa[kMaxZones];
    double fr[kMaxZones];
    double ca[kMaxZones];
// ... 35 lines not shown
    const double* wflux_dn;
    const double* wflux_up;
};

struct Conv {
    int* active;
    int* norders;
    int* status;
    int* nactive;
    double* ratio;
    int* redo;
    const int* target;
    double tol;
};

__device__ __forceinline__ bool conv_go(const Conv& cv, int b, int order, double r) {
    return cv.target ? order < cv.target[b] : r >= cv.tol;
}

constexpr int GEMM_BM = 64, GEMM_BN = 128, GEMM_KC = 16;
#ifndef SOSRT_GEMM_RT
#define SOSRT_GEMM_RT 4
#endif
#ifndef SOSRT_GEMM_WPS
#define SOSRT_GEMM_WPS 3
#endif
constexpr int GEMM_RT = SOSRT_GEMM_RT;
constexpr int GEMM_WPS = SOSRT_GEMM_WPS;

constexpr int TC = 8;

struct TransportArgs {
    Grid g;
    const double* tau;
    const double* Jn;
    double* In;
    double* I;
    double* saved;
    size_t saved_col_stride;
    const ColDesc* desc;
    Conv cv;
    int order;
    int accumulate;
    const double* Etab;
    const int* erep;
    unsigned long long* stamps;
    int live = 0;
    const int* live_list = nullptr;
    int slots = 0;
    int nzcap = kRingZones;
    int scan_split = 0;
    double* scan_scratch = nullptr;
    int* scan_sync = nullptr;
};
void launch_transport_fast(hipStream_t s, dim3 grid, dim3 block, const TransportArgs& a);
bool transport_ring_ok(const Grid& g);
bool transport_ring_fits(const Grid& g, int nzcap);
void launch_transport_ring(hipStream_t s, dim3 grid, const TransportArgs& a, int slots);
bool transport_scan_ok(const Grid& g);
bool transport_scan_split_ok(const Grid& g);
bool transport_scan_fits(const Grid& g, int nzcap, bool split);
int transport_scan_parts(const Grid& g);
size_t transport_scan_scratch_doubles();
void launch_transport_scan(hipStream_t s, dim3 grid, const TransportArgs& a);
constexpr int kOrderLoopMaxCols = 256;
constexpr int kOlArrive = 0, kOlState = 32, kOlLeft = 64, kOlAbort = 96, kOlOrders = 100, kOlCols = 128;
constexpr int kOlColStride = 64, kOlOrdDone = 0, kOlColStop = 1, kOlJnDone = 32;
constexpr int kOlReady = 1, kOlNotResident = 2, kOlAborted = 3;
inline size_t order_loop_sync_ints(int cols) { return (size_t)kOlCols + (size_t)cols * kOlColStride; }
extern int g_ring_slots, g_ring_debug;
extern unsigned long long* g_transport_stamps;

struct SolveSetup {
    int* zero_next = nullptr;
    int n_zero = 0;
    int* redo = nullptr;
    unsigned long long* hash = nullptr;
    int* scan_sync = nullptr;
};
void launch_prepare(hipStream_t s, const Grid& g, int B, int geom, int surface, ColScalars sc, const double* tau,
                    ColDesc* desc, double* rowcoef_a, double* rowcoef_r, int* need_small = nullptr, SolveSetup su = SolveSetup());
void launch_first_order_readme(hipStream_t s, const Grid& g, const double* w, int B, const double* tau, const double* P0a,
                               const double* P0r, const ColDesc* desc, double* I1_out, double* I_out, double* saved,
                               size_t saved_col_stride, Conv cv, int do_conv);
void launch_first_order(hipStream_t s, const Grid& g, int B, const double* tau, const double* P0a, const double* P0r,
                        const ColDesc* desc, double* I1_out, double* I_out, double* saved, size_t saved_col_stride,
                        Conv cv, int do_conv, int p0r_zones = 0 );
struct GemmArgs {
    const double* A;
    const double* Wa;
    const double* Wr;
    const double* ca;
    const double* cr;
    const int* rows_main;
    int n_main;
    const int* rows_slab;
    int n_slab;
    int D, Dp, Wld, L;
    double* C;
    const int* active;
    int B = 0;
    int col0 = 0;
    const int* idx_up = nullptr;
    const int* idx_down = nullptr;
    int max_main = 0, max_slab = 0;
    const double* Wmix = nullptr;
    const int* mix_group = nullptr;
    int pad_lds = 0;
    int* live_list = nullptr;
    int live_cap = 0;
    const int* slab_tile_group = nullptr;
    const int* nactive = nullptr;
    const int* need_small = nullptr;
    int* host_pub = nullptr;
    int tag = 0;
    int sym = 0;
    int Ks = 0;
    int check_tiles = 1;
    int lr_rank = -1;
    const double* lrU = nullptr;
    const double* lrV = nullptr;
};
struct AtmSets {
    const int* col_atm = nullptr;
    const int* lr_ranks = nullptr;
};
constexpr int kLowRankMax = 4;

__device__ inline void publish_live_now(const GemmArgs& g) {
    const int live = __hip_atomic_load(g.nactive, __ATOMIC_RELAXED, __HIP_MEMORY_SCOPE_AGENT);
    int* slot = g.host_pub + 4 * (g.tag & 1);
    __hip_atomic_store(slot, live, __ATOMIC_RELAXED, __HIP_MEMORY_SCOPE_SYSTEM);
    __hip_atomic_store(slot + 2, g.need_small ? g.need_small[0] : 1, __ATOMIC_RELAXED, __HIP_MEMORY_SCOPE_SYSTEM);
    __hip_atomic_store(slot + 1, g.tag, __ATOMIC_RELEASE, __HIP_MEMORY_SCOPE_SYSTEM);
}
__device__ inline void publish_live(const GemmArgs& g) {
    if (g.host_pub && blockIdx.x == 0 && blockIdx.y == 0 && threadIdx.x == 0) publish_live_now(g);
}
struct PerDeviceOnce {
    bool seen[64] = {};
    bool first() {
        int d = 0;
        if (hipGetDevice(&d) != hipSuccess || d < 0 || d >= 64) return true;
        if (seen[d]) return false;
        seen[d] = true;
        return true;
    }
};
void launch_gemm(hipStream_t s, const GemmArgs& a, const AtmSets* at = nullptr);
struct OrderLoopArgs {
    TransportArgs t;
    GemmArgs gm;
    const double* in0;
    double* gbufP;
    double* gbufQ;
    double* bufP;
    double* bufQ;
    int order0;
    int kmax;
    int B, col0;
    int fixcap;
    int* sync;
    int* host_done;
    int tag;
    unsigned long long* log = nullptr;
    int astage = 0;
};
bool order_loop_ok(const Grid& g, bool split);
int order_loop_parts(const Grid& g, bool split);
hipError_t launch_order_loop(hipStream_t s, int grid, bool split, const OrderLoopArgs& p);
void launch_gemm_f32(hipStream_t s, const GemmArgs& a, const float* Wa32, const float* Wmix32);
void launch_to_float(hipStream_t s, size_t n, const double* src, float* dst);
void launch_wmix(hipStream_t s, size_t n, int ngroups, const double* Wa, const double* Wr, const double* ca, const double* cr,
                 double* Wmix, const int* gset = nullptr ,
                 const int* gatm = nullptr );
void launch_fold_sets(hipStream_t s, int S, int D, int Wld, size_t per, const double* w, const double* P, double* W);
void launch_fold_asymmetry(hipStream_t s, int S, int nblk, int D, int Wld, size_t per, const double* W, double* out);
void launch_symfold(hipStream_t s, int nmat, int N, int D, int Dp, int Wld, const double* W, double* SA);
void launch_gemm_tail(hipStream_t s, const GemmArgs& a, int cols, bool small_tiles, bool regs = false, const AtmSets* at = nullptr);
void launch_smallmu(hipStream_t s, const Grid& g, int B, const double* tau, const double* Jn, double* In,
                    const ColDesc* desc, const int* active);
void launch_transport(hipStream_t s, const Grid& g, int B, const double* tau, const double* Jn, double* In, double* I,
                      double* saved, size_t saved_col_stride, const ColDesc* desc, Conv cv, int order, int accumulate,
                      const double* Etab, int mode, const int* erep = nullptr, int live = 0, const int* live_list = nullptr,
                      int ring_slots = 0, int scan_split = 0, double* scan_scratch = nullptr, int* scan_sync = nullptr,
                      int nzcap = kRingZones);
bool transport_fast_ok(const Plan& plan);
void launch_attenuation(hipStream_t s, const Grid& g, int B, const double* tau, double* Etab, const int* erep);
void launch_tau_groups(hipStream_t s, const Grid& g, int B, const double* tau, unsigned long long* hash, int* erep,
                       const int* need_small = nullptr, int* host_flag = nullptr, int tag = 0);
void launch_fluxes(hipStream_t s, const Grid& g, int B, const double* tau, const double* I, const ColDesc* desc,
                   int beam_norm, double* fdn, double* fup);
struct EpilogueOut {
    double* flux_down;
    double* flux_up;
    double* diffusivity;
    double* heating_rate;
    double* net_toa;
};
void launch_epilogue(hipStream_t s, const Grid& g, const double* w, int B, const double* tau, const double* I,
                     const ColDesc* desc, int beam_norm, const double* z_profile, const EpilogueOut& out);
void launch_phase_p0(hipStream_t s, const Grid& g, const double* w, int B, int kind, double gpar, const double* tab_mu,
                     const double* tab_p, int ntab, const double* cosphi, const double* wphi, int nphi,
                     const double* mu0, double* P0);
void launch_phase_matrix(hipStream_t s, const Grid& g, const double* w, int kind, double gpar, const double* tab_mu,
                         const double* tab_p, int ntab, const double* cosphi, const double* wphi, int nphi, double* P);
constexpr int kMaxModes = 64;
void launch_phase_modes(hipStream_t s, const Grid& g, const double* w, int kind, double gpar, const double* tab_mu,
                        const double* tab_p, int ntab, const double* cosphi, const double* tab, int nphi, int m_first,
                        int m_count, double* P_out);
void launch_phase_p0_modes(hipStream_t s, const Grid& g, const double* w, int B, int kind, double gpar, const double* tab_mu,
                           const double* tab_p, int ntab, const double* cosphi, const double* tab, int nphi, int m_first,
                           int m_count, const double* mu0, double* P0_out);
void launch_azimuth_accumulate(hipStream_t s, const Grid& g, int B, int m, const double* Im, int nlev, const int* levels,
                               int nphi_out, const double* phi, double* out);
void launch_azimuth_synthesize(hipStream_t s, const Grid& g, int B, int M, const double* I0, const double* Im, int nlev,
                               const int* levels, int nphi_out, const double* phi, double* out);
void launch_negate_odd_modes(hipStream_t s, size_t n, int m_first, int m_count, double* P);
constexpr int kMieQ = 6;
constexpr int kMieChunk = 4;
inline int mie_chunks(int R) { return (R + kMieChunk - 1) / kMieChunk; }
void launch_mie_coefficients(hipStream_t s, int nlanes, int R, int n_cap, const double* x, const int* nmax, const int* nstart,
                             const double* m_re, const double* m_im, const double* radii, const double* r_m, const double* sig,
                             double* ab, double* qw);
void launch_mie_angles(hipStream_t s, int S, int R, int ntab, int n_cap, const double* mu, const double* ab, const int* nmax,
                       const double* tn, const double* qw, double* part);
void launch_mie_integrate(hipStream_t s, int S, int R, int ntab, const double* part, const double* radii, const double* qw,
                          double* p, double* bulk);
void launch_limit_rows(hipStream_t s, const Grid& g, int R, int table, const double* rows, double* out);
void launch_asymptotic(hipStream_t s, int R, int stride, const int* len, const double* J, const double* tau,
                       const double* tau_t, const double* mu, double* out);
void launch_finalize(hipStream_t s, int B, Conv cv, int max_orders, int* n_out = nullptr, int* status_out = nullptr);
void launch_bench(hipStream_t s, int which, double* a, double* b, size_t n, int iters);

}
```

sos-radiative-transfer_amd/csrc/transport_ring.hip:

```cpp
#include <type_traits>

#include "../../include/sosrt.h"
#include "kernels.hpp"
#include "transport_util.hpp"

namespace sosrt {

namespace {

#ifndef SOSRT_RING_STORE_AUX
#define SOSRT_RING_STORE_AUX 0
#endif
__device__ __forceinline__ void rstore(__amdgpu_buffer_rsrc_t r, int voff, int soff, double x) { bstore_aux<SOSRT_RING_STORE_AUX>(r, voff, soff, x); }

typedef __attribute__((address_space(3))) void* lds_ptr_t;

constexpr size_t kRingLdsBytes = 152 * 1024;

template <int CNT>
__device__ __forceinline__ void wait_vm() {
    asm volatile("s_waitcnt vmcnt(%0)" ::"n"(CNT) : "memory");
}
__device__ __forceinline__ void wg_barrier() {
    asm volatile("s_waitcnt lgkmcnt(0)\n\ts_barrier" ::: "memory");
}

template <bool ACC, bool SAVED, int PIECES, bool MZ>
__global__ __launch_bounds__(512) void k_transport_ring(TransportArgs a, int NS, int dbg_arg, int fixcap) {
    constexpr int NWL = 2;
#ifdef SOSRT_RING_DEBUG
    const int dbg = dbg_arg;
#else
    constexpr int dbg = 0;
    (void)dbg_arg;
#endif
    int b = blockIdx.x;
    if (ACC && a.live > 0) {
        b = a.live_list[blockIdx.x];
        if (b < 0) return;
    } else if (ACC && !a.cv.active[b]) {
        return;
    }
    const Grid& g = a.g;
    const int tid = threadIdx.x, lane = tid & 63;
    const int wid = __builtin_amdgcn_readfirstlane(tid) >> 6;
    const int L = g.L, N = g.N, D = g.D;
    const int nwc = (N + 63) >> 6;
    const bool loader = wid >= nwc;
    const int lid = wid - nwc;
    const bool w0 = wid == 0 && !(dbg & 8);
    const bool wl = wid == ((N - 1) >> 6) && !(dbg & 4);
    auto stamp = [&](int i) {
        if (a.stamps && (tid == 0 || tid == 64)) a.stamps[((size_t)b * 2 + (tid >> 6)) * 8 + i] = clock64();
    };
    stamp(0);
    constexpr int NARR = ACC ? 3 : 2;
    constexpr int RS = 128 * PIECES;
    constexpr int SLOT = NARR * TC * RS;
    constexpr int IPC = NARR * TC * PIECES;
    extern __shared__ double sm[];
    double* ring = sm;
    double* s_sfc = ring + (size_t)NS * SLOT;
    double* s_fixc = s_sfc;
    double* s_red = s_sfc + max(RS, (MZ ? a.nzcap : kRingZones) * fixcap * kFixMaxSrc);
    double* s_hd = s_red + (blockDim.x >> 6) + 2;
    double* s_S = s_hd + L + 1;
    double* s_x = s_S + (size_t)g.nsmall * L;
    double* s_prmu = s_x + TC * 16;
    int* s_nf = reinterpret_cast<int*>(s_prmu + 16);
    const int xb_dn = max(((N - 1) & 63) - 15, 0);
    __shared__ int s_flag[3];
    const ColDesc* __restrict__ dg = a.desc + b;
    const int nz = dg->nz;
    const ZoneRows<MZ> zr(dg);
    const int nfix0 = dg->nfix[0], nfix1 = dg->nfix[1], nfix2 = dg->nfix[2];
    const int surface = dg->surface;
    const double rho = dg->rho;
    const int fbytes = L * D * 8, RB = D * 8;
    const int lbytes = (dbg & 1) ? 0 : fbytes, sbytes = (dbg & 2) ? 0 : fbytes;
    const __amdgpu_buffer_rsrc_t rJ = make_rsrc(a.Jn + (size_t)b * L * D, lbytes);
    const __amdgpu_buffer_rsrc_t rE = make_rsrc(a.Etab + (size_t)(a.erep ? a.erep[b] : b) * L * D, lbytes);
    const __amdgpu_buffer_rsrc_t rIn = make_rsrc(a.In + (size_t)b * L * D, sbytes);
    const __amdgpu_buffer_rsrc_t rIl = make_rsrc(ACC ? a.I + (size_t)b * L * D : a.In, ACC ? lbytes : 0);
    const __amdgpu_buffer_rsrc_t rI = make_rsrc(ACC ? a.I + (size_t)b * L * D : a.In, ACC ? sbytes : 0);
    const __amdgpu_buffer_rsrc_t rS = make_rsrc(SAVED ? a.saved + (size_t)b * a.saved_col_stride : a.In, SAVED ? sbytes : 0);
    const int NCH = (L + TC - 1) / TC, NQ = 2 * NCH, R = NS - 1;
    const bool valid = tid < N;
    const int tidc = valid ? tid : N - 1;
    unsigned long long sp_dn = NCH > 64 ? ~0ull : 1ull << (NCH - 1), sp_up = sp_dn;
    if (NCH <= 64) {
        sp_dn |= zr.boundary_chunks(L, TC, false);
        sp_up |= zr.boundary_chunks(L, TC, true);
    }
    auto plain_run = [&](unsigned long long mask, int j) {
        const unsigned long long rest = NCH > 64 ? 1ull : mask >> j;
        return rest ? __builtin_ctzll(rest) : 0;
    };
    double rdn_v = 0, rdn_i = 1, rup_v = 0, rup_i = 1;
    double sfc_own = 0;
    int slot_rd = 0;

    int slot_ld = 0;
    auto issue = [&](int q) {
        const bool up = q >= NCH;
        const int j = up ? q - NCH : q;
        double* dst = ring + (size_t)slot_ld * SLOT;
        slot_ld = slot_ld + 1 == NS ? 0 : slot_ld + 1;
        const int half = up ? N * 8 : 0;
        const int vo = lane * 16;
#pragma unroll
        for (int i = 0; i < TC / NWL; ++i) {
            const int u = i * NWL + lid;
            const int row = up ? max(L - 1 - j * TC - u, 0) : min(j * TC + u, L - 1);
#pragma unroll
            for (int p = 0; p < PIECES; ++p) {
                const int so = row * RB + half + p * 1024;
                __builtin_amdgcn_raw_ptr_buffer_load_lds(rJ, (lds_ptr_t)(dst + (0 * TC + u) * RS + p * 128), 16, vo, so, 0, 0);
                __builtin_amdgcn_raw_ptr_buffer_load_lds(rE, (lds_ptr_t)(dst + (1 * TC + u) * RS + p * 128), 16, vo, so, 0, 0);
                if (ACC) __builtin_amdgcn_raw_ptr_buffer_load_lds(rIl, (lds_ptr_t)(dst + (2 * TC + u) * RS + p * 128), 16, vo, so, 0, 0);
            }
        }
    };
    auto loader_phase = [&](auto keep_t, int qa, int qb) {
        constexpr int KEEP = decltype(keep_t)::value;
        for (int q = qa; q < qb; ++q) {
            if (q + R < NQ) {
                issue(q + R);
                wait_vm<KEEP>();
            } else {
                wait_vm<0>();
            }
            wg_barrier();
        }
    };
    const int ncomp = nwc * 64;
    if (loader) {
        for (int q = 0; q < min(R, NQ); ++q) issue(q);
    } else {
        for (int zz = 0; zz < (MZ ? nz : kRingZones); ++zz) {
            const FixTab& src = g.fix[dg->fixtab[zz]];
            for (int i = tid; i < fixcap * kFixMaxSrc; i += ncomp) s_fixc[zz * fixcap * kFixMaxSrc + i] = src.C[i];
        }
        if (tid < 3) s_flag[tid] = 0;
        for (int i = tid; i < (L + 31) / 32; i += ncomp) s_nf[i] = 0;
        const double* __restrict__ tau = a.tau + (size_t)b * L;
        for (int t = tid; t <= L; t += ncomp) s_hd[t] = (t == 0 || t == L) ? 0.0 : (tau[t] - tau[t - 1]) * 0.5;
        if (tid < 16) s_prmu[tid] = (tid > 0 && tid < N) ? 1.0 / g.mu[N + tid] : 0.0;
        const double* __restrict__ In0 = a.In + (size_t)b * L * D;
        for (int i = tid; i < g.nsmall * L; i += ncomp) {
            const int k = i / L, t = i - k * L;
            s_S[i] = In0[(size_t)t * D + g.small_lanes[k]];
        }
    }
    __syncthreads();

    const int seam_barriers = surface == SOSRT_SURFACE_NONE ? 0 : (surface == SOSRT_SURFACE_SPECULAR ? 1 : 3);
    double Bv = 0;
    if (loader) {
        constexpr int PER = IPC / NWL;
        auto run = [&](auto keep_t) {
            loader_phase(keep_t, 0, NCH);
            for (int i = 0; i < seam_barriers; ++i) wg_barrier();
            loader_phase(keep_t, NCH, NQ);
            wait_vm<0>();
        };
        if (R <= 1) run(std::integral_constant<int, 0>{});
        else if (R == 2) run(std::integral_constant<int, (PER < 60 ? PER : 60)>{});
        else if (R == 3) run(std::integral_constant<int, (2 * PER < 60 ? 2 * PER : 60)>{});
        else run(std::integral_constant<int, (3 * PER < 60 ? 3 * PER : 60)>{});
    } else {
    stamp(1);
    const double mu_up = (valid && tid > 0) ? g.mu[N + tidc] : 1.0;
    const int uT = lane >> 3, pT = lane & 7;
    const double muT = (pT + 1 < N) ? g.mu[N + pT + 1] : 1.0;
    const double* xrow = s_x + uT * 16;
    {
        const int m = tidc;
        const int vo = m * 8;
        const double mu = g.mu[m];
        const bool tr = valid && m <= N - 2;
        const bool small = tr && fabs(mu) < kMuThreshold;
        const bool stdl = tr && !small;
        const double nrmu = stdl ? -1.0 / mu : 0.0;
        const bool has_small = wl && g.nsmall > 0;
        double Dv = 0, Jprev = 0;
        double c[kFixMaxSrc] = {0, 0, 0, 0, 0};
        double cT[kFixMaxSrc] = {0, 0, 0, 0, 0};
        int sl[kFixMaxSrc] = {0, 0, 0, 0, 0};
        int nfx = 0;
        bool fixlane = false;
        auto load_fix = [&](int zz) {
            const double* ftC = s_fixc + zz * fixcap * kFixMaxSrc;
            nfx = zz == 0 ? nfix0 : (zz == 1 ? nfix1 : ((!MZ || zz == 2) ? nfix2 : zr.nfix(zz)));
            const int ns = nfx < 2 ? 2 : (nfx < kFixMaxSrc ? nfx : kFixMaxSrc);
            fixlane = valid && nfx > 0 && m >= N - nfx;
            const int i = fixlane ? N - 1 - m : 0;
            const int s0 = nfx < 2 ? N - nfx - 2 : N - nfx - ns;
#pragma unroll
            for (int q = 0; q < kFixMaxSrc; ++q) {
                c[q] = (fixlane && q < ns) ? ftC[i * ns + min(q, ns - 1)] : 0.0;
                cT[q] = (pT < nfx && q < ns) ? ftC[pT * ns + min(q, ns - 1)] : 0.0;
                sl[q] = (s0 + min(q, ns - 1)) & 63;
            }
        };
        if (wl) load_fix(0);
        const int sbase = small ? (m - g.small_lanes[0]) * L : 0;
        int t0 = 0, q = 0;
        auto process = [&](auto special_t, auto mode_t, const double* slot, double (&Jc)[TC], double (&Ic)[TC], double (&Ec)[TC]) __attribute__((always_inline)) {
            constexpr bool SP = decltype(special_t)::value;
            constexpr int MODE = decltype(mode_t)::value;
            double cc[TC], v[TC], Sc[TC];
#pragma unroll
            for (int u = 0; u < TC; ++u) Sc[u] = 0;
            if ((SP || MODE == 2) && has_small) {
#pragma unroll
                for (int u = 0; u < TC; ++u) {
                    const double sv = s_S[sbase + min(t0 + u, L - 1)];
                    Sc[u] = small ? sv : 0.0;
                }
            }
#pragma unroll
            for (int u = 0; u < TC; ++u) {
                const int t = SP ? min(t0 + u, L - 1) : t0 + u;
                const double hk = s_hd[t];
                const double Jp = u == 0 ? Jprev : Jc[u - 1];
                cc[u] = rec_src(rec_hr(hk, nrmu), Jp, Ec[u], Jc[u]);
            }
            if (!SP) {
// ... 29 lines not shown
                        if (ACC) rstore(rI, voT, 0, IcT + acc);
                        if (SAVED) rstore(rS, voT, 0, acc);
                    }
                } else if (MODE == 2 && wl && nfx > 0) {
#pragma unroll
                    for (int u = 0; u < TC; ++u) {
                        double acc = 0;
#pragma unroll
                        for (int k = 0; k < kFixMaxSrc; ++k) acc = fix_acc(c[k], readlane_f64(v[u], sl[k]), acc);
                        v[u] = fixlane ? acc : v[u];
                    }
                }
                if (valid && !(tfix && fixlane)) {
#pragma unroll
                    for (int u = 0; u < TC; ++u) {
                        const int so = (t0 + u) * RB;
                        rstore(rIn, vo, so, v[u]);
                        if (ACC) rstore(rI, vo, so, Ic[u] + v[u]);
                        if (SAVED) rstore(rS, vo, so, v[u]);
                    }
                }
            } else {
#pragma unroll
                for (int u = 0; u < TC; ++u) {
                    const int t = t0 + u;
                    if (wl) { const int zs = zr.starts(t); if (zs) load_fix(zs); }
                    const double Dn = rec_step(Dv, Ec[u], cc[u]);
                    double x = has_small ? rec_add(Dn, Sc[u]) : Dn;
                    if (wl && nfx > 0) {
                        double acc = 0;
#pragma unroll
                        for (int k = 0; k < kFixMaxSrc; ++k) acc = fix_acc(c[k], readlane_f64(x, sl[k]), acc);
                        x = fixlane ? acc : x;
                    }
                    v[u] = x;
                    const bool zone_end = zr.ends(t);
                    Dv = t < L ? (zone_end ? (stdl ? x : 0.0) : Dn) : Dv;
                    if (valid && t < L) {
                        const int so = t * RB;
                        rstore(rIn, vo, so, x);
                        if (ACC) rstore(rI, vo, so, Ic[u] + x);
                        if (SAVED) rstore(rS, vo, so, x);
                    }
                }
            }
            if (SP && t0 + TC >= L) {
#pragma unroll
                for (int u = 0; u < TC; ++u)
                    if (t0 + u == L - 1) { sfc_own = v[u]; rdn_v = v[u]; rdn_i = Ic[u] + v[u]; }
            }
            Jprev = Jc[TC - 1];
            t0 += TC;
        };
        auto chunk = [&](auto special_t, auto mode_t) __attribute__((always_inline)) {
            const double* sp = ring + (size_t)slot_rd * SLOT + tid;
            slot_rd = slot_rd + 1 == NS ? 0 : slot_rd + 1;
            double Jc[TC], Ic[TC], Ec[TC];
#pragma unroll
            for (int u = 0; u < TC; ++u) {
                Jc[u] = sp[(0 * TC + u) * RS];
                Ec[u] = sp[(1 * TC + u) * RS];
                Ic[u] = ACC ? sp[(2 * TC + u) * RS] : 0.0;
            }
            process(special_t, mode_t, sp - tid, Jc, Ic, Ec);
            wg_barrier();
        };
        using M0 = std::integral_constant<int, 0>;
        using M1 = std::integral_constant<int, 1>;
        using M2 = std::integral_constant<int, 2>;
        while (q < NCH) {
            const int qe = q + plain_run(sp_dn, q);
            const int mode = (!wl || (nfx == 0 && !has_small)) ? 0 : ((!has_small && nfx <= 8 && sl[0] >= xb_dn) ? 1 : 2);
            if (mode == 0) for (; q < qe; ++q) chunk(std::false_type{}, M0{});
            else if (mode == 1) for (; q < qe; ++q) chunk(std::false_type{}, M1{});
            else for (; q < qe; ++q) chunk(std::false_type{}, M2{});
            if (q < NCH) { chunk(std::true_type{}, M2{}); ++q; }
        }
    }

    stamp(2);
    if (surface != SOSRT_SURFACE_NONE) {
        if (valid) s_sfc[tid] = sfc_own;
        wg_barrier();
    }
    if (surface == SOSRT_SURFACE_SPECULAR) {
        Bv = valid ? rho * s_sfc[N - 1 - tid] : 0.0;
    } else if (surface == SOSRT_SURFACE_LAMBERTIAN || surface == SOSRT_SURFACE_LAMBERTIAN_README) {
        double term = 0;
        if (tid <= N - 3) {
            const int k0 = N - 2 - tid, k1 = k0 - 1;
            const double x0 = g.mu[k0], x1 = g.mu[k1];
            term = (x1 - x0) * (s_sfc[k1] * x1 + s_sfc[k0] * x0) / 2;
        }
        double ws = wave_sum_(term);
        wg_barrier();
        if (lane == 0) s_red[tid >> 6] = ws;
        wg_barrier();
        double S = 0;
        for (int i = 0; i < nwc; ++i) S += s_red[i];
        Bv = (surface == SOSRT_SURFACE_LAMBERTIAN_README ? 2 : -2) * rho * S;
    }

    stamp(3);
    {
        const int mj = N + tidc;
        const int vo = mj * 8;
        const bool tr = valid && tid > 0;
        const double mu = mu_up;
        const double prmu = tr ? 1.0 / mu : 0.0;
        const int last_cand = min(N - 3, 61);
        bool notfound = false;
        double U = Bv, Jnext = 0;
        auto blend = [&](double x, int t) {
            const double x1 = lane_up1(x), x2 = lane_up1(x1);
            const bool stop = lane >= 1 && lane <= last_cand && !(fabs((x - x1) - (x1 - x2)) > 0.0001);
            const unsigned long long mk = __ballot(stop);
            const int kf = mk ? __ffsll((long long)mk) : 1;
            if (mk == 0) {
                notfound = true;
                if (N - 3 > 61 && lane == 0) {
                    if (zr.starts(t)) s_flag[0] = 1;
                    else { flag_row(s_nf, t); s_flag[2] = 1; }
                }
            }
            const double r0 = readlane_f64(x, 0), rk = readlane_f64(x, kf);
            const double w = blend_weight(mu, readlane_f64(prmu, kf));
            const double bl = blend_val(w, r0, rk);
            return (tr && tid < kf) ? bl : x;
        };
// ... 47 lines not shown
                            const int voT = (t0 - uT) * RB + (N + k) * 8;
                            rstore(rIn, voT, 0, val);
                            if (ACC) rstore(rI, voT, 0, IcT + val);
                            if (SAVED) rstore(rS, voT, 0, val);
                        }
                    } else {
#pragma unroll
                        for (int u = 0; u < TC; ++u) {
                            const double xb_ = blend(v[u], t0 - u);
                            if (valid) {
                                const int so = (t0 - u) * RB;
                                rstore(rIn, vo, so, xb_);
                                if (ACC) rstore(rI, vo, so, Ic[u] + xb_);
                                if (SAVED) rstore(rS, vo, so, xb_);
                            }
                        }
                    }
                }
                if (valid && (MODE == 0 || (tblend && !(tid >= 1 && tid <= 8)))) {
#pragma unroll
                    for (int u = 0; u < TC; ++u) {
                        const int so = (t0 - u) * RB;
                        rstore(rIn, vo, so, v[u]);
                        if (ACC) rstore(rI, vo, so, Ic[u] + v[u]);
                        if (SAVED) rstore(rS, vo, so, v[u]);
                    }
                }
            } else {
#pragma unroll
                for (int u = 0; u < TC; ++u) {
                    const int t = t0 - u;
                    const double Un = rec_step(U, Ec[u], cc[u]);
                    double x = Un;
                    if (w0 && t >= 0) x = blend(tid == 0 ? Jc[u] : Un, t);
                    v[u] = x;
                    const bool zone_start = zr.starts(t) != 0;
                    U = t >= 0 ? ((zone_start && tr) ? x : Un) : U;
                    if (valid && t >= 0) {
                        const int so = t * RB;
                        rstore(rIn, vo, so, x);
                        if (ACC) rstore(rI, vo, so, Ic[u] + x);
                        if (SAVED) rstore(rS, vo, so, x);
                    }
                }
            }
            if (SP && t0 - TC < 0) {
#pragma unroll
                for (int u = 0; u < TC; ++u)
                    if (t0 - u == 0) { rup_v = v[u]; rup_i = Ic[u] + v[u]; }
            }
            Jnext = Jc[TC - 1];
            t0 -= TC;
        };
        auto chunk = [&](auto special_t, auto mode_t) __attribute__((always_inline)) {
            const double* sp = ring + (size_t)slot_rd * SLOT + tid;
            slot_rd = slot_rd + 1 == NS ? 0 : slot_rd + 1;
            double Jc[TC], Ic[TC], Ec[TC];
#pragma unroll
            for (int u = 0; u < TC; ++u) {
                Jc[u] = sp[(0 * TC + u) * RS];
                Ec[u] = sp[(1 * TC + u) * RS];
                Ic[u] = ACC ? sp[(2 * TC + u) * RS] : 0.0;
            }
            process(special_t, mode_t, sp - tid, Jc, Ic, Ec);
            wg_barrier();
        };
        using M0 = std::integral_constant<int, 0>;
        using M1 = std::integral_constant<int, 1>;
        while (q < NQ) {
            const int qe = q + plain_run(sp_up, q - NCH);
            if (!w0) for (; q < qe; ++q) chunk(std::false_type{}, M0{});
            else for (; q < qe; ++q) chunk(std::false_type{}, M1{});
            if (q < NQ) { chunk(std::true_type{}, M1{}); ++q; }
        }
        if (w0 && notfound && lane == 0 && N - 3 <= 61) s_flag[1] = 1;
    }
    }
    stamp(4);
    __syncthreads();
    stamp(5);
    if (s_flag[1]) {
        if (tid == 0) {
            a.cv.status[b] = SOSRT_COL_INDEXERROR;
            if (ACC) { a.cv.active[b] = 0; a.cv.norders[b] = a.order; atomicSub(a.cv.nactive, 1); }
        }
        return;
    }
    if (!s_flag[0] && s_flag[2]) {
        if (finish_flagged_rows<ACC, SAVED>(s_nf, L, N, RB, g.mu, rIn, rI, rS, ring, rup_v, rup_i)) {
            if (tid == 0) {
                a.cv.status[b] = SOSRT_COL_INDEXERROR;
                if (ACC) { a.cv.active[b] = 0; a.cv.norders[b] = a.order; atomicSub(a.cv.nactive, 1); }
            }
            return;
        }
    }
    if (s_flag[0]) {
        const bool missing = redo_upward_sweep<ACC, SAVED, MZ>(L, N, RB, zr, s_hd, g.mu, rJ, rE, rIn, rI, rS, Bv, ring,
                                                            rup_v, rup_i);
        if (missing) {
            if (tid == 0) {
                a.cv.status[b] = SOSRT_COL_INDEXERROR;
                if (ACC) { a.cv.active[b] = 0; a.cv.norders[b] = a.order; atomicSub(a.cv.nactive, 1); }
            }
            return;
        }
    }
    if (ACC) {
        const double ra = block_pymax_(rup_v / rup_i, valid, s_red, 0);
        const double rb = block_pymax_(rdn_v / rdn_i, valid, s_red, 0);
        const double r = (rb > ra) ? rb : ra;
        if (tid == 0) {
            a.cv.ratio[b] = r;
            a.cv.norders[b] = a.order;
            if (!conv_go(a.cv, b, a.order, r)) {
                a.cv.active[b] = 0;
                atomicSub(a.cv.nactive, 1);
            }
        }
    } else if (tid == 0 && a.cv.status) {
        a.cv.status[b] = SOSRT_COL_OK;
    }
}

inline int ring_fixcap(const Grid& g) { return (int)(0.06 * g.N) + 1; }
inline size_t ring_extra_doubles(const Grid& g, int nt, int nzcap = kRingZones) {
    const int rs = g.N <= 128 ? 128 : 256, fc = nzcap * ring_fixcap(g) * kFixMaxSrc;
    return (size_t)(rs > fc ? rs : fc) + nt / 64 + 2 + g.L + 1 + (size_t)g.nsmall * g.L + TC * 16 + 16 + (g.L + 63) / 64;
}

template <int PIECES>
void launch_p(hipStream_t s, dim3 grid, dim3 block, const TransportArgs& a, int NS) {
    const int nt = (int)block.x;
    const int narr = a.accumulate ? 3 : 2;
    const size_t shm = ((size_t)NS * narr * TC * 128 * PIECES + ring_extra_doubles(a.g, nt, a.nzcap)) * sizeof(double);
#define SOSRT_RING_LAUNCH_Z(ACC_, SAVED_, MZ_)                                                                 \
    do {                                                                                                       \
        auto kern = k_transport_ring<ACC_, SAVED_, PIECES, MZ_>;                                               \
        static PerDeviceOnce big_lds;                                                                                 \
        if (big_lds.first()) {                                                                                        \
            hipFuncSetAttribute(reinterpret_cast<const void*>(kern), hipFuncAttributeMaxDynamicSharedMemorySize, \
                                (int)kRingLdsBytes);                                                                   \
        }                                                                                                      \
        hipLaunchKernelGGL(kern, grid, block, shm, s, a, NS, g_ring_debug, ring_fixcap(a.g));                           \
    } while (0)
#define SOSRT_RING_LAUNCH(ACC_, SAVED_)                                                                        \
    do {                                                                                                       \
        if (a.nzcap > kRingZones) SOSRT_RING_LAUNCH_Z(ACC_, SAVED_, true);                                     \
        else SOSRT_RING_LAUNCH_Z(ACC_, SAVED_, false);                                                         \
    } while (0)
    if (a.accumulate) {
        if (a.saved) SOSRT_RING_LAUNCH(true, true);
        else SOSRT_RING_LAUNCH(true, false);
    } else {
        SOSRT_RING_LAUNCH(false, false);
    }
#undef SOSRT_RING_LAUNCH
#undef SOSRT_RING_LAUNCH_Z
}

}

bool transport_ring_ok(const Grid& g) {
    if (g.N % 2 || g.N < 4 || g.N > 256) return false;
    const int nwc = (g.N + 63) / 64, pieces = g.N <= 128 ? 1 : 2;
    const size_t slot_bytes = (size_t)3 * TC * 128 * pieces * sizeof(double);
    if (flagged_rows_work_doubles(g.L, g.N) * sizeof(double) > 2 * slot_bytes * 2 / 3) return false;
    return 2 * slot_bytes + ring_extra_doubles(g, (nwc + 4) * 64) * sizeof(double) <= kRingLdsBytes;
}

bool transport_ring_fits(const Grid& g, int nzcap) {
    if (!transport_ring_ok(g)) return false;
    const int nwc = (g.N + 63) / 64, pieces = g.N <= 128 ? 1 : 2;
    const size_t slot_bytes = (size_t)3 * TC * 128 * pieces * sizeof(double);
    return 2 * slot_bytes + ring_extra_doubles(g, (nwc + 4) * 64, nzcap < kRingZones ? kRingZones : nzcap) * sizeof(double) <= kRingLdsBytes;
}

void launch_transport_ring(hipStream_t s, dim3 grid, const TransportArgs& a, int slots) {
    if (a.slots > 0) slots = a.slots;
    const int N = a.g.N;
    const int nwc = (N + 63) / 64;
    const int pieces = N <= 128 ? 1 : 2;
    const int narr = a.accumulate ? 3 : 2;
    const dim3 block((nwc + 2) * 64);
    const size_t slot_bytes = (size_t)narr * TC * 128 * pieces * sizeof(double);
    const size_t extra = ring_extra_doubles(a.g, (int)block.x, a.nzcap) * sizeof(double);
    int NS = slots < 2 ? 2 : slots;
    while (NS > 2 && NS * slot_bytes + extra > kRingLdsBytes) --NS;
    if (pieces == 1) launch_p<1>(s, grid, block, a, NS);
    else launch_p<2>(s, grid, block, a, NS);
}

}
```

sos-radiative-transfer_amd/csrc/transport_util.hpp:

```cpp
#pragma once
#include <hip/hip_runtime.h>

#include "kernels.hpp"

namespace sosrt {
namespace {

__device__ __forceinline__ double readlane_f64(double v, int srclane) {
    int lo = __double2loint(v), hi = __double2hiint(v);
    lo = __builtin_amdgcn_readlane(lo, srclane);
    hi = __builtin_amdgcn_readlane(hi, srclane);
    return __hiloint2double(hi, lo);
}

typedef unsigned int u32x2 __attribute__((ext_vector_type(2)));

__device__ __forceinline__ __amdgpu_buffer_rsrc_t make_rsrc(const void* p, int bytes) {
    return __builtin_amdgcn_make_buffer_rsrc(const_cast<void*>(p), 0, bytes, 0x00020000);
}
__device__ __forceinline__ double bload(__amdgpu_buffer_rsrc_t r, int voff, int soff) {
    const u32x2 v = __builtin_amdgcn_raw_buffer_load_b64(r, voff, soff, 0);
    return __hiloint2double((int)v.y, (int)v.x);
}
__device__ __forceinline__ double bload_glc(__amdgpu_buffer_rsrc_t r, int voff, int soff) {
// ... 185 lines not shown
    __syncthreads();
    const int cnt = *s_cnt;
    const bool act = tid < N, tr = act && tid > 0;
    const int j = act ? tid : 0;
    const double mu = tr ? gmu[N + j] : 1.0;
    const int vo = (N + j) * 8;
    bool missing = false;
    for (int c0 = 0; c0 < cnt; c0 += kNfBatch) {
        const int nb = min(kNfBatch, cnt - c0);
        double xo[kNfBatch], Io[kNfBatch];
#pragma unroll
        for (int i = 0; i < kNfBatch; ++i) {
            const int t = s_list[c0 + min(i, nb - 1)];
            xo[i] = bload_aux<LDX ? LDX : 1>(rIn, vo, t * RB);
            Io[i] = ACC ? bload_aux<LDX ? LDX : 1>(rI, vo, t * RB) : 0.0;
        }
#pragma unroll
        for (int i = 0; i < kNfBatch; ++i)
            if (act) s_rows[i * NP + j] = xo[i];
        if (tid < kNfBatch) s_kf[tid] = 1 << 30;
        __syncthreads();
#pragma unroll
        for (int i = 0; i < kNfBatch; ++i) {
            const double* r = s_rows + i * NP;
            if (i < nb && act && j >= 1 && j <= N - 3 && !(fabs((r[j] - r[j + 1]) - (r[j + 1] - r[j + 2])) > 0.0001)) atomicMin(&s_kf[i], j);
        }
        __syncthreads();
#pragma unroll
        for (int i = 0; i < kNfBatch; ++i) {
            if (i >= nb) continue;
            const double* r = s_rows + i * NP;
            const int ks = s_kf[i];
            missing |= ks == (1 << 30);
            const int kf = ks == (1 << 30) ? 1 : ks + 1;
            const int t = s_list[c0 + i];
            if (tr && tid < kf) {
                const double x = blend_val(blend_weight(mu, 1.0 / gmu[N + kf]), r[0], r[kf]);
                bstore_aux<STX>(rIn, vo, t * RB, x);
                double It = 0;
                if (ACC) {
                    It = Io[i] + (x - xo[i]);
                    bstore_aux<STX>(rI, vo, t * RB, It);
                }
                if (SAVED) bstore_aux<STX>(rS, vo, t * RB, x);
                if (t == 0) { rup_v = x; rup_i = It; }
            }
        }
        __syncthreads();
    }
    return missing;
}

constexpr int kRedoRows = 8;
template <bool ACC, bool SAVED, bool MZ, int LDX = 0, int STX = 0>
__device__ SOSRT_HELPER_INLINE bool redo_upward_sweep(int L, int N, int RB, const ZoneRows<MZ>& zr, const double* s_hd,
                                  const double* __restrict__ gmu, __amdgpu_buffer_rsrc_t rJ, __amdgpu_buffer_rsrc_t rE,
                                  __amdgpu_buffer_rsrc_t rIn, __amdgpu_buffer_rsrc_t rI, __amdgpu_buffer_rsrc_t rS, double U0,
                                  double* s_work, double& rup_v, double& rup_i) {
    const int tid = threadIdx.x;
    double* s_row = s_work;
    int* s_kf = reinterpret_cast<int*>(s_work + 2 * (N + 2));
    const bool act = tid < N, tr = act && tid > 0;
    const int j = act ? tid : 0;
    const double mu = tr ? gmu[N + j] : 1.0;
    const double prmu = tr ? 1.0 / mu : 0.0;
    const int vo = (N + j) * 8;
    double U = U0, Jnext = 0;
    bool missing = false;
    if (tid < 2) s_kf[tid] = 1 << 30;
    __syncthreads();
    int par = 0;
    for (int t0 = L - 1; t0 >= 0; t0 -= kRedoRows) {
        double Jc[kRedoRows], Ec[kRedoRows], xo[kRedoRows], Io[kRedoRows];
#pragma unroll
        for (int u = 0; u < kRedoRows; ++u) {
            const int t = max(t0 - u, 0);
            Jc[u] = bload_aux<LDX>(rJ, vo, t * RB);
            Ec[u] = bload(rE, vo, t * RB);
            xo[u] = bload_aux<LDX ? LDX : 1>(rIn, vo, t * RB);
            Io[u] = ACC ? bload_aux<LDX ? LDX : 1>(rI, vo, t * RB) : 0.0;
        }
#pragma unroll
        for (int u = 0; u < kRedoRows; ++u) {
            const int t = t0 - u;
            if (t < 0) break;
            double* row = s_row + par * (N + 2);
            const double src = rec_src(rec_hr(s_hd[t + 1], prmu), Jnext, Ec[u], Jc[u]);
            const double Un = rec_step(U, Ec[u], zr.ends(t) ? 0.0 : src);
            if (act) row[j] = tid == 0 ? Jc[u] : Un;
            __syncthreads();
            if (act && j >= 1 && j <= N - 3 && !(fabs((row[j] - row[j + 1]) - (row[j + 1] - row[j + 2])) > 0.0001)) atomicMin(&s_kf[par], j);
            if (tid == 0) s_kf[par ^ 1] = 1 << 30;
            __syncthreads();
            const int ks = s_kf[par];
            missing |= ks == (1 << 30);
            const int kf = ks == (1 << 30) ? 1 : ks + 1;
            double x = act ? row[j] : 0.0;
            if (tr && tid < kf) x = blend_val(blend_weight(mu, 1.0 / gmu[N + kf]), row[0], row[kf]);
            const bool zone_start = zr.starts(t) != 0;
            U = (zone_start && tr) ? x : Un;
            Jnext = Jc[u];
            if (act) {
                bstore_aux<STX>(rIn, vo, t * RB, x);
                double It = 0;
                if (ACC) {
                    It = Io[u] + (x - xo[u]);
                    bstore_aux<STX>(rI, vo, t * RB, It);
                }
                if (SAVED) bstore_aux<STX>(rS, vo, t * RB, x);
                if (t == 0) { rup_v = x; rup_i = It; }
            }
            par ^= 1;
        }
    }
    __syncthreads();
    return missing;
}

__device__ __forceinline__ double block_pymax_(double x, bool valid, double* s_red, int first_tid) {
    const int tid = threadIdx.x, nw = blockDim.x >> 6;
    double v = wave_fmax_(valid ? x : __builtin_nan(""));
    __syncthreads();
    if ((tid & 63) == 0) s_red[tid >> 6] = v;
    if (tid == first_tid) s_red[nw] = x;
    __syncthreads();
    double r = s_red[0];
    for (int i = 1; i < nw; ++i) r = fmax(r, s_red[i]);
    const double first = s_red[nw];
    return (first != first) ? first : r;
}
// ... 4 lines not shown
```

sos-radiative-transfer_amd/sosrt/_lib.py:

```python
import ctypes
import os
from ctypes import POINTER, c_char_p, c_double, c_int, c_longlong, c_void_p

_HERE = os.path.dirname(os.path.abspath(__file__))
LIB_PATH = os.environ.get("SOSRT_LIB") or os.path.join(os.path.dirname(_HERE), "libsosrt.so")

SOSRT_OK, E_INVALID, E_HIP, E_STATE, E_NOMEM = 0, -1, -2, -3, -4
COL_OK, COL_INDEXERROR, COL_MAXORDERS, COL_INTERNAL = 0, 1, 2, 3
GEOM_THREE_ZONE, GEOM_SINGLE_SLAB = 0, 1
SURFACE_NONE, SURFACE_SPECULAR, SURFACE_LAMBERTIAN, SURFACE_LAMBERTIAN_README = 0, 1, 2, 3
K_GEMM, K_TRANSPORT, K_FIRST, K_SMALLMU, K_ORDER_LOOP = 0, 1, 2, 3, 4
PLAN_GEMM_DENSE, PLAN_GEMM_LIVE64, PLAN_GEMM_LIVE32, PLAN_GEMM_LIVE32_DEEP, PLAN_GEMM_LIVE16_REGS = 0, 1, 2, 3, 4
PLAN_TRANSPORT_GENERAL, PLAN_TRANSPORT_FAST, PLAN_TRANSPORT_RING, PLAN_TRANSPORT_SCAN = 0, 1, 3, 4
CONTRACT_F64, CONTRACT_F32, CONTRACT_F64_FULL, CONTRACT_F64_DENSE = 0, 1, 2, 3
FIRST_ORDER_CODED, FIRST_ORDER_README = 0, 1
PHASE_ISO, PHASE_RAYLEIGH, PHASE_HG, PHASE_TABLE = 0, 1, 2, 3
MAX_MODES = 64
MAX_PHASE_SETS = 64

_dp = POINTER(c_double)
_ip = POINTER(c_int)

SIGNATURES = {
    "sosrt_last_error": (c_char_p, []),
    "sosrt_version": (c_int, []),
    "sosrt_create": (c_int, [c_int, c_int, c_int, c_int, c_int, POINTER(c_void_p)]),
    "sosrt_destroy": (c_int, [c_void_p]),
    "sosrt_set_stream": (c_int, [c_void_p, c_void_p]),
    "sosrt_use_own_stream": (c_int, [c_void_p]),
    "sosrt_synchronize": (c_int, [c_void_p]),
    "sosrt_set_saved_orders": (c_int, [c_void_p, c_int]),
    "sosrt_set_order_budget": (c_int, [c_void_p, c_int]),
    "sosrt_set_contraction": (c_int, [c_void_p, c_int]),
    "sosrt_phase_asymmetry": (c_int, [c_void_p, POINTER(c_double), _ip]),
    "sosrt_phase_rank": (c_int, [c_void_p, _ip, POINTER(c_double), _ip]),
    "sosrt_set_order_loop": (c_int, [c_void_p, c_int]),
    "sosrt_order_loop_stats": (c_int, [c_void_p, _ip, _ip, POINTER(c_longlong)]),
    "sosrt_plan_launch": (c_int, [c_void_p, c_int, c_int, c_int, c_int, c_int, _ip]),
    "sosrt_set_first_order": (c_int, [c_void_p, c_int]),
    "sosrt_set_grid": (c_int, [c_void_p, c_void_p]),
    "sosrt_set_phase": (c_int, [c_void_p, c_void_p, c_void_p]),
    "sosrt_set_phase_sets": (c_int, [c_void_p, c_void_p, c_int, c_void_p]),
    "sosrt_set_phase_sets_dev": (c_int, [c_void_p, c_void_p, c_int, c_void_p]),
    "sosrt_phase_matrix_dev": (c_int, [c_void_p, c_int, c_double, c_void_p]),
    "sosrt_set_aerosol_sets": (c_int, [c_void_p, c_int, c_int, c_void_p]),
    "sosrt_phase_sets_info": (c_int, [c_void_p, _ip]),
    "sosrt_set_atm_phase_sets": (c_int, [c_void_p, c_int, c_void_p]),
    "sosrt_set_atmosphere_sets": (c_int, [c_void_p, c_int, c_void_p]),
    "sosrt_atm_sets_info": (c_int, [c_void_p, _ip]),
    "sosrt_set_columns": (c_int, [c_void_p, c_int, c_int, c_int] + [c_void_p] * 9),
    "sosrt_set_columns_zones": (c_int, [c_void_p, c_int, c_int, c_int] + [c_void_p] * 10),
    "sosrt_first_order": (c_int, [c_void_p, c_int, c_void_p, c_void_p, c_void_p, c_void_p]),
    "sosrt_source": (c_int, [c_void_p, c_int, c_void_p, c_void_p]),
    "sosrt_transport": (c_int, [c_void_p, c_int, c_void_p, c_void_p, c_void_p, c_void_p]),
    "sosrt_solve": (c_int, [c_void_p, c_int, c_void_p, c_void_p, c_void_p, c_double, c_void_p, c_void_p, c_void_p, c_void_p, c_void_p]),
    "sosrt_solve_dev": (c_int, [c_void_p, c_int, c_void_p, c_void_p, c_void_p, c_double, c_void_p, c_void_p, c_void_p, c_void_p, c_void_p]),
    "sosrt_last_solve_stats": (c_int, [c_void_p, _ip, POINTER(c_longlong)]),
    "sosrt_fluxes": (c_int, [c_void_p, c_int, c_void_p, c_void_p, c_int, c_void_p, c_void_p]),
    "sosrt_epilogue_dev": (c_int, [c_void_p, c_int, c_void_p, c_void_p, c_int] + [c_void_p] * 6),
    "sosrt_epilogue": (c_int, [c_void_p, c_int, c_int] + [c_void_p] * 6),
    "sosrt_phase_table": (c_int, [c_void_p, c_void_p, c_void_p, c_int]),
    "sosrt_phase_table_dev": (c_int, [c_void_p, c_void_p, c_void_p, c_int]),
    "sosrt_mie_ensembles": (c_int, [c_void_p, c_int] + [c_void_p] * 5 + [c_int, c_double, c_double, c_int, c_void_p, c_void_p]),
    "sosrt_mie_ensembles_dev": (c_int, [c_void_p, c_int] + [c_void_p] * 5 + [c_int, c_double, c_double, c_int, c_void_p, c_void_p]),
    "sosrt_mie_efficiencies": (c_int, [c_void_p, c_int, c_void_p, c_void_p, c_void_p, c_void_p]),
    "sosrt_mie_timing": (c_int, [c_void_p, _dp]),
    "sosrt_phase_p0_dev": (c_int, [c_void_p, c_int, c_int, c_double, c_void_p, c_void_p]),
    "sosrt_phase_p0": (c_int, [c_void_p, c_int, c_int, c_double, c_void_p, c_void_p]),
    "sosrt_phase_matrix": (c_int, [c_void_p, c_int, c_double, c_void_p]),
    "sosrt_phase_modes": (c_int, [c_void_p, c_int, c_double, c_int, c_int, c_int, c_void_p]),
    "sosrt_phase_modes_dev": (c_int, [c_void_p, c_int, c_double, c_int, c_int, c_int, c_int, c_void_p]),
    "sosrt_phase_p0_modes_dev": (c_int, [c_void_p, c_int, c_int, c_double, c_int, c_int, c_int, c_void_p, c_void_p]),
    "sosrt_phase_p0_modes": (c_int, [c_void_p, c_int, c_int, c_double, c_int, c_int, c_int, c_void_p, c_void_p]),
    "sosrt_set_order_targets": (c_int, [c_void_p, c_void_p]),
    "sosrt_azimuth_accumulate_dev": (c_int, [c_void_p, c_int, c_int, c_void_p, c_int, c_void_p, c_int, c_void_p, c_void_p]),
    "sosrt_azimuth_synthesize_dev": (c_int, [c_void_p, c_int, c_int, c_void_p, c_void_p, c_int, c_void_p, c_int, c_void_p, c_void_p]),
    "sosrt_comm_unique_id": (c_int, [c_void_p]),
    "sosrt_comm_init": (c_int, [c_void_p, c_int, c_int, c_void_p]),
    "sosrt_gather": (c_int, [c_void_p, c_int, c_void_p, c_void_p, c_void_p]),
    "sosrt_comm_destroy": (c_int, [c_void_p]),
    "sosrt_limit_mu_down": (c_int, [c_void_p, c_int, c_int, c_void_p, c_void_p]),
    "sosrt_asymptotic_down": (c_int, [c_void_p, c_int, c_int, c_void_p, c_void_p, c_void_p, c_void_p, c_void_p, c_void_p]),
    "sosrt_plan_weights": (c_int, [c_void_p, c_void_p]),
    "sosrt_plan_fold": (c_int, [c_void_p, c_int, c_void_p]),
    "sosrt_plan_fix_table": (c_int, [c_void_p, c_int, _ip, _ip, c_void_p]),
    "sosrt_plan_fix_count": (c_int, [c_double, c_int]),
    "sosrt_debug_stamps": (c_int, [c_void_p, c_void_p]),
    "sosrt_microbench": (c_int, [c_void_p, c_int, _dp]),
    "sosrt_profile_enable": (c_int, [c_void_p, c_int]),
    "sosrt_profile_reset": (c_int, [c_void_p]),
# ... 53 lines not shown
```

sos-radiative-transfer_amd/sosrt/solver.py:

```python
from __future__ import annotations

import ctypes
from dataclasses import dataclass
from typing import Optional

import numpy as np

from . import _lib
from ._lib import check, lib


def _f64(a, shape=None, name="array"):
    a = np.ascontiguousarray(a, dtype=np.float64)
    if shape is not None and a.shape != tuple(shape):
        raise ValueError("%s has shape %s, expected %s" % (name, a.shape, tuple(shape)))
    return a


def _i32(a, n, name):
    a = np.ascontiguousarray(a, dtype=np.int32)
    if a.shape != (n,):
        raise ValueError("%s has shape %s, expected (%d,)" % (name, a.shape, n))
    return a

# ... 23 lines not shown


class Solver:

    def __init__(self, nb_layers: int, nb_angles: int, max_batch: int = 1, max_orders: int = 64, device: int = 0):
        self.L, self.N, self.D = int(nb_layers), int(nb_angles), 2 * int(nb_angles)
        self.max_batch, self.max_orders, self.device = int(max_batch), int(max_orders), int(device)
        self._h = ctypes.c_void_p()
        check(lib().sosrt_create(self.device, self.L, self.N, self.max_batch, self.max_orders, ctypes.byref(self._h)))
        self.B = 0
        self.order_budget = self.max_orders
        self.mu = None
        self._P = (None, None)
        self._p0_zones = 0

    def close(self):
        if getattr(self, "_h", None) is not None and self._h.value:
            lib().sosrt_destroy(self._h)
            self._h = ctypes.c_void_p()

    def __del__(self):
        try:
            self.close()
        except Exception:
            pass

    def set_stream(self, stream_handle: Optional[int]):
        if stream_handle is None:
            check(lib().sosrt_use_own_stream(self._h))
        else:
            check(lib().sosrt_set_stream(self._h, ctypes.c_void_p(stream_handle) if stream_handle else None))

    def synchronize(self):
        check(lib().sosrt_synchronize(self._h))

    def set_contraction(self, mode="f64"):
        m = {"f64": _lib.CONTRACT_F64, "f32": _lib.CONTRACT_F32, "f64_full": _lib.CONTRACT_F64_FULL,
             "f64_dense": _lib.CONTRACT_F64_DENSE}.get(mode)
        if m is None:
            raise ValueError("contraction must be 'f64', 'f64_dense', 'f64_full' or 'f32'")
        check(lib().sosrt_set_contraction(self._h, m))

    def set_order_budget(self, max_orders: int):
        check(lib().sosrt_set_order_budget(self._h, int(max_orders)))
        self.order_budget = int(max_orders)

    def set_order_loop(self, on=True):
        check(lib().sosrt_set_order_loop(self._h, int(on) if on in (0, 1, 2) else (1 if on else 0)))

    def order_loop_stats(self, column_orders=False):
        a, b, c = ctypes.c_int(), ctypes.c_int(), ctypes.c_longlong()
        check(lib().sosrt_order_loop_stats(self._h, ctypes.byref(a), ctypes.byref(b), ctypes.byref(c) if column_orders else None))
        return (a.value, b.value, c.value) if column_orders else (a.value, b.value)

    def phase_asymmetry(self):
        a, u = ctypes.c_double(), ctypes.c_int()
        check(lib().sosrt_phase_asymmetry(self._h, ctypes.byref(a), ctypes.byref(u)))
        return a.value, bool(u.value)

    def phase_rank(self):
        r, a, u = ctypes.c_int(), ctypes.c_double(), ctypes.c_int()
        check(lib().sosrt_phase_rank(self._h, ctypes.byref(r), ctypes.byref(a), ctypes.byref(u)))
        return r.value, a.value, bool(u.value)

    def set_first_order(self, mode="coded"):
        m = {"coded": _lib.FIRST_ORDER_CODED, "readme": _lib.FIRST_ORDER_README}.get(mode)
        if m is None:
            raise ValueError("first_order must be 'coded' or 'readme'")
        check(lib().sosrt_set_first_order(self._h, m))

    def set_grid(self, mu):
        mu = _f64(mu, (self.D,), "mu")
        check(lib().sosrt_set_grid(self._h, _ptr(mu)))
        self.mu = mu.copy()
        self._P = (None, None)

    def set_phase(self, P_atm, P_aer=None):
        Pa = _f64(P_atm, (self.D, self.D), "P_atm")
        Pr = None if P_aer is None else _f64(P_aer, (self.D, self.D), "P_aer")
        check(lib().sosrt_set_phase(self._h, _ptr(Pa), _ptr(Pr)))
        self._P = (Pa.copy(), None if Pr is None else Pr.copy())

    def set_phase_sets(self, P_atm, P_aer_sets):
        Pa = _f64(P_atm, (self.D, self.D), "P_atm")
        Pr = np.ascontiguousarray(P_aer_sets, dtype=np.float64)
        if Pr.ndim != 3 or Pr.shape[1:] != (self.D, self.D):
            raise ValueError("P_aer_sets has shape %s, expected (S, %d, %d)" % (Pr.shape, self.D, self.D))
        check(lib().sosrt_set_phase_sets(self._h, _ptr(Pa), int(Pr.shape[0]), _ptr(Pr)))
        self._P = (Pa.copy(), Pr.copy())

    def set_phase_sets_device(self, P_atm, d_P_aer: int, S: int):
        Pa = _f64(P_atm, (self.D, self.D), "P_atm")
        check(lib().sosrt_set_phase_sets_dev(self._h, _ptr(Pa), int(S), ctypes.c_void_p(d_P_aer) if d_P_aer else None))
        self._P = (None, None)

    def set_aerosol_sets(self, sets):
        z = np.ascontiguousarray(sets, dtype=np.int32)
        if z.ndim == 1:
            z = z.reshape(-1, 1)
        if z.ndim != 2 or z.shape[0] != self.B:
            raise ValueError("sets has shape %s, expected (%d,) or (%d, nzmax)" % (np.shape(sets), self.B, self.B))
        check(lib().sosrt_set_aerosol_sets(self._h, int(z.shape[0]), int(z.shape[1]), _ptr(z)))
        self._p0_zones = int(z.shape[1]) if z.shape[1] > 1 else 0

    def phase_sets_info(self):
        out = (ctypes.c_int * 4)()
# ... 280 lines not shown

    def gather_device(self, root: int, counts, d_send: int, d_recv: int):
        c = np.ascontiguousarray(counts, dtype=np.int64)
        check(lib().sosrt_gather(self._h, int(root), _ptr(c), ctypes.c_void_p(d_send) if d_send else None,
                                 ctypes.c_void_p(d_recv) if d_recv else None))

    def comm_destroy(self):
        check(lib().sosrt_comm_destroy(self._h))

    def limit_mu_down(self, rows, idx):
        rows = np.ascontiguousarray(rows, dtype=np.float64)
        if rows.ndim != 2 or rows.shape[1] != self.N:
            raise ValueError("rows must be [R, nb_angles]")
        out = np.empty((rows.shape[0], idx))
        if idx:
            check(lib().sosrt_limit_mu_down(self._h, rows.shape[0], int(idx), _ptr(rows), _ptr(out)))
        return out

    def asymptotic_down(self, J, tau, lens, tau_t, mu):
        J = np.ascontiguousarray(J, dtype=np.float64)
        tau = _f64(tau, J.shape, "tau")
        R, stride = J.shape
        lens = _i32(lens, R, "len")
        tt = _f64(tau_t, (R,), "tau_t")
        m = _f64(mu, (R,), "mu")
        out = np.empty(R)
        check(lib().sosrt_asymptotic_down(self._h, R, stride, _ptr(lens), _ptr(J), _ptr(tau), _ptr(tt), _ptr(m), _ptr(out)))
        return out

    def plan_weights(self):
        w = np.empty(self.D)
        check(lib().sosrt_plan_weights(self._h, _ptr(w)))
        return w

    def plan_fold(self, which=0):
        W = np.empty((self.D, self.D))
        check(lib().sosrt_plan_fold(self._h, which, _ptr(W)))
        return W

    def plan_fix_table(self, idx):
        s0, ns = ctypes.c_int(), ctypes.c_int()
        C = np.zeros((max(idx, 1), 5))
        check(lib().sosrt_plan_fix_table(self._h, int(idx), ctypes.byref(s0), ctypes.byref(ns), _ptr(C)))
        return s0.value, ns.value, C.reshape(-1)[: idx * ns.value].reshape(idx, ns.value).copy()

    def plan_launch(self, batch, live, surface="specular", zones=3, cus=0):
        sf = {"none": _lib.SURFACE_NONE, "specular": _lib.SURFACE_SPECULAR, "lambertian": _lib.SURFACE_LAMBERTIAN,
              "lambertian_readme": _lib.SURFACE_LAMBERTIAN_README}[surface]
        out = (ctypes.c_int * 9)()
        check(lib().sosrt_plan_launch(self._h, int(batch), int(live), sf, int(zones), int(cus), out))
        keys = ("groups", "gemm", "tail_cols", "transport", "parts", "repair", "order_loop", "ol_parts", "ol_grid")
        return dict(zip(keys, list(out)))

    def microbench(self, which):
        r = ctypes.c_double()
        check(lib().sosrt_microbench(self._h, int(which), ctypes.byref(r)))
        return r.value

    def profile_enable(self, on=True):
        check(lib().sosrt_profile_enable(self._h, 1 if on else 0))

    def profile_reset(self):
        check(lib().sosrt_profile_reset(self._h))

    def profile_get(self, kernel):
        ms, cnt, w = ctypes.c_double(), ctypes.c_longlong(), ctypes.c_double()
        check(lib().sosrt_profile_get(self._h, kernel, ctypes.byref(ms), ctypes.byref(cnt), ctypes.byref(w)))
        return ms.value, cnt.value


def fix_count(tau_ref: float, nb_angles: int) -> int:
    return lib().sosrt_plan_fix_count(float(tau_ref), int(nb_angles))
```

Measured before the change: 118,900.

## Fuse low-rank source expansion into ring transport via stored moments

When the phase matrix is low-rank and the ring transport runs, the source GEMM now writes only the per-row low-rank moments (rank coefficients) instead of expanding the full Jn rows. The ring transport kernel then rebuilds Jn on the fly from those moments and the V factors held in LDS. This removes the full Jn write and read through global memory. In exchange it adds moment buffers, extra LDS per ring block, a planner gate covering many conditions, and a row-layout consistency check at column setup.

Result: slower. 78660 (-33.8%).

```diff
diff --git a/__graft_entry__.py b/__graft_entry__.py
--- a/__graft_entry__.py
+++ b/__graft_entry__.py
@@ -7,7 +7,7 @@
 CSRC = os.path.join(PKG, "csrc")
 LIB = os.path.join(PKG, "libsosrt.so")
 SOURCES = ["api.hip", "kernels.hip", "jn_gemm.hip", "jn_gemm_f32.hip", "transport_fast.hip", "transport_ring.hip", "transport_scan.hip", "order_loop.hip", "epilogue.hip", "plan.cpp", "comm.cpp"]
-HEADERS = ["kernels.hpp", "plan.hpp", "transport_util.hpp", "transport_scan_body.hpp", "jn_gemm_tile.hpp", "comm.hpp", os.path.join(ROOT, "include", "sosrt.h")]
+HEADERS = ["kernels.hpp", "plan.hpp", "transport_util.hpp", "transport_scan_body.hpp", "jn_gemm_tile.hpp", "lowrank_expand.hpp", "comm.hpp", os.path.join(ROOT, "include", "sosrt.h")]
 
 
 OBJDIR = os.path.join(PKG, "build")
diff --git a/include/sosrt.h b/include/sosrt.h
--- a/include/sosrt.h
+++ b/include/sosrt.h
@@ -65,6 +65,13 @@
 
 int sosrt_set_order_loop(sosrt_t* h, int mode);
 int sosrt_order_loop_stats(sosrt_t* h, int* launches, int* refused, long long* column_orders );
+
+#define SOSRT_PLAN_FLAG_NEED_SMALL 1
+#define SOSRT_PLAN_FLAG_SAVING 2
+#define SOSRT_PLAN_FLAG_ATM_SETS 4
+int sosrt_set_source_moments(sosrt_t* h, int on);
+int sosrt_source_moments_stats(sosrt_t* h, int* launches);
+int sosrt_plan_source_moments(sosrt_t* h, int batch, int live, int surface, int zones, int flags, int* moments);
 int sosrt_phase_asymmetry(sosrt_t* h, double* asymmetry, int* uses_symmetry);
 int sosrt_phase_rank(sosrt_t* h, int* rank, double* residual, int* uses);
 
diff --git a/sos-radiative-transfer_amd/csrc/api.hip b/sos-radiative-transfer_amd/csrc/api.hip
--- a/sos-radiative-transfer_amd/csrc/api.hip
+++ b/sos-radiative-transfer_amd/csrc/api.hip
@@ -187,6 +187,10 @@
     unsigned long long* d_ollog = nullptr;
     int ol_launches = 0, ol_refused = 0;
     bool ol_group_used[kMaxGroups] = {false, false};
+    int source_moments = 1;
+    double* d_mom = nullptr;
+    int mom_launches = 0;
+    bool mom_rows_ok = false;
     Rccl::comm_t comm = nullptr;
     int comm_rank = -1, comm_world = 0;
 };
@@ -431,7 +435,7 @@
 }
 
 void run_source(sosrt_handle* h, const double* In_1, double* Jn, const int* active, int tail_cols = 0, int pub_tag = 0,
-                int grp = -1, bool all_live = false, bool regs_tile = false, int dense_live_cap = 0) {
+                int grp = -1, bool all_live = false, bool regs_tile = false, int dense_live_cap = 0, bool moments = false) {
     const int g0 = grp < 0 ? 0 : grp, g1 = grp < 0 ? h->ngroups : grp + 1;
     const int pg = grp < 0 ? 0 : grp;
     hipStream_t s = group_stream(h, pg);
@@ -466,6 +470,7 @@
         ga.Wr = h->d_Wrsets; ga.mix_group = h->d_mixgroup; ga.slab_tile_group = h->d_slabtilegroup + h->slab_off[g0] / 32;
     }
     if (use_lowrank(h)) { ga.lr_rank = h->lr_rank; ga.lrU = h->d_lrU; ga.lrV = h->d_lrV; }
+    if (moments && use_lowrank(h)) ga.mom = h->d_mom + (h->nslab > 0 ? 0 : (size_t)h->gb[g0] * h->L * kLowRankMax);
     AtmSets at;
     const AtmSets* atp = nullptr;
     if (h->max_atm_used > 0) {
@@ -536,6 +541,9 @@
     bool saving = false;
     int orders_left = 1 << 30;
     int cu_share = 0;
+    bool atm_sets = false;
+    bool rows_agree = true;
+    int ring_slots = 0;
 };
 struct LaunchPlan {
     int tail_cols = 0;
@@ -547,6 +555,7 @@
     int order_loop = 0;
     int ol_parts = 0;
     int ol_grid = 0;
+    int moments = 0;
 };
 LaunchPlan plan_order(const sosrt_handle* h, const SolveShape& sh, const OrderInputs& in) {
     LaunchPlan pl;
@@ -593,6 +602,9 @@
         }
         if (pl.order_loop) pl.ol_grid = in.cu_share;
     }
+    pl.moments = (h->source_moments && pl.transport == SOSRT_PLAN_TRANSPORT_RING && use_lowrank(h) && !in.atm_sets && in.simple_zones &&
+                  in.rows_agree && sh.nzcap <= kRingZones && !in.need_small && !in.saving && !pl.order_loop && !pl.repair &&
+                  transport_ring_moments_ok([&] { Grid gt = g; gt.nsmall = 0; return gt; }(), h->lr_rank, in.ring_slots)) ? 1 : 0;
     return pl;
 }
 
@@ -667,6 +679,7 @@
 #endif
     if (const char* ev = getenv("SOSRT_GROUP_RING_SLOTS")) h->coresident_slots = atoi(ev);
     if (const char* ev = getenv("SOSRT_ORDER_LOOP")) h->order_loop = atoi(ev) != 0;
+    if (const char* ev = getenv("SOSRT_SOURCE_MOMENTS")) h->source_moments = atoi(ev) != 0;
     if (const char* ev = getenv("SOSRT_RING_SLOTS")) g_ring_slots = atoi(ev);
 #ifdef SOSRT_RING_DEBUG
     if (const char* ev = getenv("SOSRT_RING_DEBUG")) g_ring_debug = atoi(ev);
@@ -689,6 +702,8 @@
             if ((e = dalloc(&h->d_Wr, (size_t)g.Dp * g.Wld))) return e;
             if ((e = dalloc(&h->d_lrU, (size_t)kLowRankMax * g.D))) return e;
             if ((e = dalloc(&h->d_lrV, (size_t)kLowRankMax * g.D))) return e;
+            if ((e = dalloc(&h->d_mom, (size_t)max_batch * L * kLowRankMax))) return e;
+            HIPCHK(hipMemset(h->d_mom, 0, (size_t)max_batch * L * kLowRankMax * sizeof(double)));
             if ((e = dalloc(&h->d_wfdn, N))) return e;
             if ((e = dalloc(&h->d_wfup, N))) return e;
             if ((e = dalloc(&h->d_w, g.D))) return e;
@@ -771,7 +786,7 @@
                         h->d_P0r, h->d_Jn, h->d_InA, h->d_InB, h->d_I, h->d_E, h->d_active, h->d_norders, h->d_status,
                         h->d_nactive_sets, h->d_ratio, h->d_redo, h->d_erep, h->d_tauhash, h->d_Wmix, h->d_mixca, h->d_mixcr,
                         h->d_mixgroup, h->d_Wa_s, h->d_Wr_s, h->d_Wmix_s, h->d_scan_scratch, h->d_scan_sync, h->d_w, h->d_phi, h->d_z, h->d_tab, h->d_slabtilegroup, h->d_livelist, h->d_Wa32, h->d_Wmix32, h->d_nz, h->d_zr0, h->d_zmix, h->d_zwr, h->d_zdtr, h->d_olsync, h->d_ollog, h->d_modetab, h->d_lrU, h->d_lrV, h->d_Wrsets, h->d_Wrsets_s, h->d_mixset, h->d_P0rz,
-                        h->d_Wasets, h->d_lrUsets, h->d_lrVsets, h->d_lrranks, h->d_colatm, h->d_mixatm};
+                        h->d_Wasets, h->d_lrUsets, h->d_lrVsets, h->d_lrranks, h->d_colatm, h->d_mixatm, h->d_mom};
         for (void* p : ptrs)
             if (p) hipFree(p);
         if (h->h_pub) hipHostFree(h->h_pub);
@@ -874,6 +889,45 @@
             }
         }
     }
+    return 0;
+}
+
+int sosrt_set_source_moments(sosrt_t* h, int on) {
+    if (!h) return fail(SOSRT_E_INVALID, "null handle");
+    if (on != 0 && on != 1) return fail(SOSRT_E_INVALID, "source moments: 0 or 1 (got %d)", on);
+    h->source_moments = on;
+    return 0;
+}
+
+int sosrt_source_moments_stats(sosrt_t* h, int* launches) {
+    if (!h) return fail(SOSRT_E_INVALID, "null handle");
+    if (launches) *launches = h->mom_launches;
+    return 0;
+}
+
+int sosrt_plan_source_moments(sosrt_t* h, int batch, int live, int surface, int zones, int flags, int* moments) {
+    if (!h || !moments) return fail(SOSRT_E_INVALID, "null argument");
+    if (!h->have_grid) return fail(SOSRT_E_STATE, "sosrt_set_grid has not been called");
+    if (batch < 1 || live < 0 || live > batch) return fail(SOSRT_E_INVALID, "need 0 <= live <= batch, batch >= 1");
+    if (zones < 1 || zones > kMaxZones) return fail(SOSRT_E_INVALID, "zones must be in 1..%d", kMaxZones);
+    int want = h->want_groups;
+    if (want == 0) want = batch > h->split_min ? 2 : 1;
+    const int ng = (want >= 2 && batch >= h->split_min && batch >= 2) ? 2 : 1;
+    const int nb = ng == 2 ? batch / 2 : batch;
+    const SolveShape sh = solve_shape(h, zones);
+    OrderInputs oi;
+    oi.nb = nb; oi.known = live < nb ? live : nb; oi.surface = surface;
+    oi.simple_zones = zones == 3 || zones == 1;
+    oi.cu_share = h->cu_count / ng;
+    oi.need_small = (flags & SOSRT_PLAN_FLAG_NEED_SMALL) != 0;
+    oi.saving = (flags & SOSRT_PLAN_FLAG_SAVING) != 0;
+    oi.atm_sets = (flags & SOSRT_PLAN_FLAG_ATM_SETS) != 0;
+    oi.ring_slots = ng > 1 ? h->coresident_slots : 0;
+    const bool saved_sym = h->sym_ok;
+    if (!h->have_phase) h->sym_ok = true;
+    const LaunchPlan pl = plan_order(h, sh, oi);
+    h->sym_ok = saved_sym;
+    *moments = pl.moments;
     return 0;
 }
 
@@ -1259,6 +1313,19 @@
             HIPCHK(hipMemcpyAsync(h->d_mainrows, plain.data(), plain.size() * sizeof(int), hipMemcpyHostToDevice, h->stream));
     }
     HIPCHK(hipStreamSynchronize(h->stream));
+    h->mom_rows_ok = true;
+    if (geometry == SOSRT_GEOM_THREE_ZONE && h->simple_zones) {
+        size_t at = 0;
+        for (int b = 0; b < B && h->mom_rows_ok; ++b) {
+            const int s0 = zr0[b * kMaxZones + 1], s1 = zone_end(b, 1);
+            if (iup[b] != s0 || idn[b] != s1) h->mom_rows_ok = false;
+            for (int t = 0; t < L && h->mom_rows_ok; ++t)
+                if (t < s0 || t > s1) h->mom_rows_ok = at < plain.size() && plain[at++] == b * L + t;
+        }
+        if (at != plain.size()) h->mom_rows_ok = false;
+    } else if (geometry == SOSRT_GEOM_THREE_ZONE) {
+        h->mom_rows_ok = false;
+    }
     h->nslab = (int)slab.size();
     h->nmain = (int)plain.size();
     h->max_main = L; h->max_slab = 0;
@@ -1742,7 +1809,7 @@
         double *In_1 = nullptr, *In = nullptr;
         Conv cv;
     } gs[sosrt_handle::kMaxGroups];
-    h->ol_launches = 0; h->ol_refused = 0;
+    h->ol_launches = 0; h->ol_refused = 0; h->mom_launches = 0;
     for (bool& u : h->ol_group_used) u = false;
     bool used_order_loop = false;
     const int tagbase = ((++h->pub_seq) & 0x3fff) << 16;
@@ -1868,6 +1935,7 @@
             oi.need_small = g.nsmall > 0 && h->need_small; oi.saving = d_I_saved_out != nullptr;
             oi.orders_left = h->order_budget - q.n;
             oi.cu_share = (q.ol_off || h->d_targets || h->max_atm_used > 0) ? 0 : h->cu_count / NG;
+            oi.atm_sets = h->max_atm_used > 0; oi.rows_agree = h->mom_rows_ok; oi.ring_slots = NG > 1 ? h->coresident_slots : 0;
             LaunchPlan pl = plan_order(h, shape, oi);
             if (pl.order_loop) {
                 const int got = ol_acquire(h->device, h->cu_count, pl.ol_grid, (int)(pl.ol_parts * q.known / h->ol_frac));
@@ -1924,7 +1992,7 @@
             n_max = n > n_max ? n : n_max;
             const int tail_cols = pl.tail_cols;
             run_source(h, q.In_1, h->d_Jn, h->d_active, tail_cols, tagbase + n - 1, k, q.known == q.nb, pl.gemm == SOSRT_PLAN_GEMM_LIVE16_REGS,
-                       tail_cols > 0 ? 0 : pl.live_cap);
+                       tail_cols > 0 ? 0 : pl.live_cap, pl.moments != 0);
             if (g.nsmall > 0 && h->need_small) {
                 prof_begin(h, SOSRT_K_SMALLMU, k);
                 launch_smallmu(sg, g, q.nb, tau_g, h->d_Jn + fo, q.In + fo, h->d_desc + q.b0, q.cv.active);
@@ -1938,7 +2006,9 @@
                 launch_transport(sg, gt, q.nb, tau_g, h->d_Jn + fo, q.In + fo, d_I_out + fo, sv_n, saved_stride, h->d_desc + q.b0, q.cv, n, 1,
                                  h->d_E, pl.transport, erep_g, pl.live_cap, h->d_livelist + q.b0, NG > 1 ? h->coresident_slots : 0,
                                  pl.parts > 1 ? 1 : 0, h->d_scan_scratch + (size_t)q.b0 * transport_scan_scratch_doubles(),
-                                 h->d_scan_sync + 2 * q.b0, nzcap);
+                                 h->d_scan_sync + 2 * q.b0, nzcap, pl.moments ? h->d_mom + (size_t)q.b0 * h->L * kLowRankMax : nullptr,
+                                 h->d_lrV, h->lr_rank);
+                if (pl.moments) ++h->mom_launches;
                 if (pl.repair)
                     launch_transport(sg, g, q.nb, tau_g, h->d_Jn + fo, q.In + fo, d_I_out + fo, sv_n, saved_stride, h->d_desc + q.b0, q.cv, n, 1,
                                      h->d_E, 2, erep_g);
diff --git a/sos-radiative-transfer_amd/csrc/jn_gemm_tile.hpp b/sos-radiative-transfer_amd/csrc/jn_gemm_tile.hpp
--- a/sos-radiative-transfer_amd/csrc/jn_gemm_tile.hpp
+++ b/sos-radiative-transfer_amd/csrc/jn_gemm_tile.hpp
@@ -1,5 +1,6 @@
 #pragma once
 #include "kernels.hpp"
+#include "lowrank_expand.hpp"
 #include "transport_util.hpp"
 
 namespace sosrt {
@@ -429,32 +430,52 @@
                 for (int i = 0; i < LR_ROWS; ++i) m[i][q] += __shfl_xor(m[i][q], s);
             }
         }
+    if constexpr (!ATM && !COH) {
+        if (g.mom) {
+            if (lane == 0) {
+#pragma unroll
+                for (int i = 0; i < LR_ROWS; ++i)
+                    if (rows[i] >= 0) {
+                        double2* dst = reinterpret_cast<double2*>(g.mom + (size_t)rows[i] * kLowRankMax);
+#pragma unroll
+                        for (int q = 0; q < kLowRankMax; q += 2) dst[q >> 1] = make_double2(m[i][q], m[i][q + 1]);
+                    }
+            }
+            return;
+        }
+    }
 #pragma unroll 2
     for (int k = 2 * lane; k < D; k += 128) {
         double2 o[LR_ROWS];
-#pragma unroll
-        for (int i = 0; i < LR_ROWS; ++i) o[i] = make_double2(0.0, 0.0);
-#pragma unroll
-        for (int q = 0; q < kLowRankMax; ++q) {
-            if constexpr (ATM) {
+        if constexpr (ATM) {
+#pragma unroll
+            for (int i = 0; i < LR_ROWS; ++i) o[i] = make_double2(0.0, 0.0);
+#pragma unroll
+            for (int q = 0; q < kLowRankMax; ++q)
 #pragma unroll
                 for (int i = 0; i < LR_ROWS; ++i)
                     if (q < Ri[i]) {
                         const double2 v = *reinterpret_cast<const double2*>(Vi[i] + (size_t)q * D + k);
-                        o[i].x = __builtin_fma(m[i][q], v.x, o[i].x);
-                        o[i].y = __builtin_fma(m[i][q], v.y, o[i].y);
+                        o[i].x = lowrank_term(m[i][q], v.x, o[i].x);
+                        o[i].y = lowrank_term(m[i][q], v.y, o[i].y);
                     }
-            } else if (q < R) {
-                const double2 v = *reinterpret_cast<const double2*>(V + (size_t)q * D + k);
-#pragma unroll
-                for (int i = 0; i < LR_ROWS; ++i) {
-                    o[i].x = __builtin_fma(m[i][q], v.x, o[i].x);
-                    o[i].y = __builtin_fma(m[i][q], v.y, o[i].y);
+#pragma unroll
+            for (int i = 0; i < LR_ROWS; ++i) o[i] = make_double2(lowrank_scale(cf[i], o[i].x), lowrank_scale(cf[i], o[i].y));
+        } else {
+            double vx[kLowRankMax], vy[kLowRankMax];
+#pragma unroll
+            for (int q = 0; q < kLowRankMax; ++q) {
+                vx[q] = 0.0; vy[q] = 0.0;
+                if (q < R) {
+                    const double2 v = *reinterpret_cast<const double2*>(V + (size_t)q * D + k);
+                    vx[q] = v.x; vy[q] = v.y;
                 }
             }
-        }
-#pragma unroll
-        for (int i = 0; i < LR_ROWS; ++i) bstore2_aux<COH ? 17 : 0>(rC[i], k * 8, 0, make_double2(cf[i] * o[i].x, cf[i] * o[i].y));
+#pragma unroll
+            for (int i = 0; i < LR_ROWS; ++i) o[i] = make_double2(lowrank_expand(m[i], vx, R, cf[i]), lowrank_expand(m[i], vy, R, cf[i]));
+        }
+#pragma unroll
+        for (int i = 0; i < LR_ROWS; ++i) bstore2_aux<COH ? 17 : 0>(rC[i], k * 8, 0, o[i]);
     }
 }
 template <bool COH, class RowOf, bool ATM = false>
diff --git a/sos-radiative-transfer_amd/csrc/kernels.hip b/sos-radiative-transfer_amd/csrc/kernels.hip
--- a/sos-radiative-transfer_amd/csrc/kernels.hip
+++ b/sos-radiative-transfer_amd/csrc/kernels.hip
@@ -1033,12 +1033,14 @@
 void launch_transport(hipStream_t s, const Grid& g, int B, const double* tau, const double* Jn, double* In, double* I,
                       double* saved, size_t saved_col_stride, const ColDesc* desc, Conv cv, int order,
                       int accumulate, const double* Etab, int mode, const int* erep, int live, const int* live_list,
-                      int ring_slots, int scan_split, double* scan_scratch, int* scan_sync, int nzcap) {
+                      int ring_slots, int scan_split, double* scan_scratch, int* scan_sync, int nzcap, const double* mom,
+                      const double* lrV, int lr_rank) {
     const int nt = round64(g.N);
     const size_t shm = (size_t)(g.L + 2 * TC * (nt + 2) + 2 * nt + nt / 64 + 2) * sizeof(double);
     TransportArgs a{g, tau, Jn, In, I, accumulate ? saved : nullptr, saved_col_stride, desc, cv, order, accumulate, Etab, Etab ? erep : nullptr, g_transport_stamps};
     a.slots = ring_slots;
     a.nzcap = nzcap > kRingZones ? nzcap : kRingZones;
+    if (mode == 3 && mom) { a.mom = mom; a.lrV = lrV; a.lr_rank = lr_rank; }
     if (mode == 4 && scan_split && scan_scratch && scan_sync) { a.scan_split = 1; a.scan_scratch = scan_scratch; a.scan_sync = scan_sync; }
     if ((mode == 3 || mode == 4) && accumulate && live > 0 && live < B && live_list) {
         a.live = live;
diff --git a/sos-radiative-transfer_amd/csrc/kernels.hpp b/sos-radiative-transfer_amd/csrc/kernels.hpp
--- a/sos-radiative-transfer_amd/csrc/kernels.hpp
+++ b/sos-radiative-transfer_amd/csrc/kernels.hpp
@@ -111,10 +111,14 @@
     int scan_split = 0;
     double* scan_scratch = nullptr;
     int* scan_sync = nullptr;
+    const double* mom = nullptr;
+    const double* lrV = nullptr;
+    int lr_rank = 0;
 };
 void launch_transport_fast(hipStream_t s, dim3 grid, dim3 block, const TransportArgs& a);
 bool transport_ring_ok(const Grid& g);
 bool transport_ring_fits(const Grid& g, int nzcap);
+bool transport_ring_moments_ok(const Grid& g, int rank, int slots);
 void launch_transport_ring(hipStream_t s, dim3 grid, const TransportArgs& a, int slots);
 bool transport_scan_ok(const Grid& g);
 bool transport_scan_split_ok(const Grid& g);
@@ -179,6 +183,7 @@
     int lr_rank = -1;
     const double* lrU = nullptr;
     const double* lrV = nullptr;
+    double* mom = nullptr;
 };
 struct AtmSets {
     const int* col_atm = nullptr;
@@ -243,7 +248,7 @@
                       double* saved, size_t saved_col_stride, const ColDesc* desc, Conv cv, int order, int accumulate,
                       const double* Etab, int mode, const int* erep = nullptr, int live = 0, const int* live_list = nullptr,
                       int ring_slots = 0, int scan_split = 0, double* scan_scratch = nullptr, int* scan_sync = nullptr,
-                      int nzcap = kRingZones);
+                      int nzcap = kRingZones, const double* mom = nullptr, const double* lrV = nullptr, int lr_rank = 0);
 bool transport_fast_ok(const Plan& plan);
 void launch_attenuation(hipStream_t s, const Grid& g, int B, const double* tau, double* Etab, const int* erep);
 void launch_tau_groups(hipStream_t s, const Grid& g, int B, const double* tau, unsigned long long* hash, int* erep,
diff --git a/sos-radiative-transfer_amd/csrc/lowrank_expand.hpp b/sos-radiative-transfer_amd/csrc/lowrank_expand.hpp
--- /dev/null
+++ b/sos-radiative-transfer_amd/csrc/lowrank_expand.hpp
@@ -0,0 +1,21 @@
+#pragma once
+#include "kernels.hpp"
+
+namespace sosrt {
+namespace {
+
+__device__ __forceinline__ double lowrank_term(double M, double V, double o) { return __builtin_fma(M, V, o); }
+__device__ __forceinline__ double lowrank_scale(double ca, double o) {
+#pragma clang fp contract(off)
+    return ca * o;
+}
+__device__ __forceinline__ double lowrank_expand(const double (&M)[kLowRankMax], const double (&V)[kLowRankMax], int R, double ca) {
+    double o = 0.0;
+#pragma unroll
+    for (int q = 0; q < kLowRankMax; ++q)
+        if (q < R) o = lowrank_term(M[q], V[q], o);
+    return lowrank_scale(ca, o);
+}
+
+}
+}
diff --git a/sos-radiative-transfer_amd/csrc/transport_ring.hip b/sos-radiative-transfer_amd/csrc/transport_ring.hip
--- a/sos-radiative-transfer_amd/csrc/transport_ring.hip
+++ b/sos-radiative-transfer_amd/csrc/transport_ring.hip
@@ -2,6 +2,7 @@
 
 #include "../../include/sosrt.h"
 #include "kernels.hpp"
+#include "lowrank_expand.hpp"
 #include "transport_util.hpp"
 
 namespace sosrt {
@@ -25,7 +26,22 @@
     asm volatile("s_waitcnt lgkmcnt(0)\n\ts_barrier" ::: "memory");
 }
 
-template <bool ACC, bool SAVED, int PIECES, bool MZ>
+struct MomentRows {
+    static constexpr bool any = true;
+    const double* s_mom;
+    int R, slab0, slab1;
+    double ca_top, ca_bot;
+    double V[kLowRankMax];
+    __device__ __forceinline__ bool plain(int t) const { return !(t >= slab0 && t <= slab1); }
+    __device__ __forceinline__ double value(int t) const {
+        double M[kLowRankMax];
+#pragma unroll
+        for (int q = 0; q < kLowRankMax; ++q) M[q] = q < R ? s_mom[t * R + q] : 0.0;
+        return lowrank_expand(M, V, R, t < slab0 ? ca_top : ca_bot);
+    }
+};
+
+template <bool ACC, bool SAVED, int PIECES, bool MZ, bool MOM = false>
 __global__ __launch_bounds__(512) void k_transport_ring(TransportArgs a, int NS, int dbg_arg, int fixcap) {
     constexpr int NWL = 2;
 #ifdef SOSRT_RING_DEBUG
@@ -68,6 +84,7 @@
     double* s_x = s_S + (size_t)g.nsmall * L;
     double* s_prmu = s_x + TC * 16;
     int* s_nf = reinterpret_cast<int*>(s_prmu + 16);
+    double* s_mom = s_prmu + 16 + (L + 63) / 64;
     const int xb_dn = max(((N - 1) & 63) - 15, 0);
     __shared__ int s_flag[3];
     const ColDesc* __restrict__ dg = a.desc + b;
@@ -84,6 +101,12 @@
     const __amdgpu_buffer_rsrc_t rIl = make_rsrc(ACC ? a.I + (size_t)b * L * D : a.In, ACC ? lbytes : 0);
     const __amdgpu_buffer_rsrc_t rI = make_rsrc(ACC ? a.I + (size_t)b * L * D : a.In, ACC ? sbytes : 0);
     const __amdgpu_buffer_rsrc_t rS = make_rsrc(SAVED ? a.saved + (size_t)b * a.saved_col_stride : a.In, SAVED ? sbytes : 0);
+    const __amdgpu_buffer_rsrc_t rJz = make_rsrc(a.Jn + (size_t)b * L * D, 0);
+    const bool has_slab = MOM && nz > 1 && dg->mix[1] != 0;
+    const int slab0 = has_slab ? dg->r0[1] : L, slab1 = has_slab ? dg->r1[1] : -1;
+    const int Rk = MOM ? a.lr_rank : 0;
+    const double ca_top = MOM ? dg->ca[0] : 0.0, ca_bot = MOM ? dg->ca[nz > 2 ? 2 : 0] : 0.0;
+    auto is_plain = [&](int t) { return MOM && !(t >= slab0 && t <= slab1); };
     const int NCH = (L + TC - 1) / TC, NQ = 2 * NCH, R = NS - 1;
     const bool valid = tid < N;
     const int tidc = valid ? tid : N - 1;
@@ -112,10 +135,12 @@
         for (int i = 0; i < TC / NWL; ++i) {
             const int u = i * NWL + lid;
             const int row = up ? max(L - 1 - j * TC - u, 0) : min(j * TC + u, L - 1);
+            __amdgpu_buffer_rsrc_t rJr = rJ;
+            if constexpr (MOM) rJr = is_plain(row) ? rJz : rJ;
 #pragma unroll
             for (int p = 0; p < PIECES; ++p) {
                 const int so = row * RB + half + p * 1024;
-                __builtin_amdgcn_raw_ptr_buffer_load_lds(rJ, (lds_ptr_t)(dst + (0 * TC + u) * RS + p * 128), 16, vo, so, 0, 0);
+                __builtin_amdgcn_raw_ptr_buffer_load_lds(rJr, (lds_ptr_t)(dst + (0 * TC + u) * RS + p * 128), 16, vo, so, 0, 0);
                 __builtin_amdgcn_raw_ptr_buffer_load_lds(rE, (lds_ptr_t)(dst + (1 * TC + u) * RS + p * 128), 16, vo, so, 0, 0);
                 if (ACC) __builtin_amdgcn_raw_ptr_buffer_load_lds(rIl, (lds_ptr_t)(dst + (2 * TC + u) * RS + p * 128), 16, vo, so, 0, 0);
             }
@@ -150,6 +175,13 @@
         for (int i = tid; i < g.nsmall * L; i += ncomp) {
             const int k = i / L, t = i - k * L;
             s_S[i] = In0[(size_t)t * D + g.small_lanes[k]];
+        }
+        if constexpr (MOM) {
+            const double* __restrict__ mg = a.mom + (size_t)b * L * kLowRankMax;
+            for (int i = tid; i < L * Rk; i += ncomp) {
+                const int t = i / Rk, q = i - t * Rk;
+                s_mom[i] = mg[t * kLowRankMax + q];
+            }
         }
     }
     __syncthreads();
@@ -174,6 +206,18 @@
     const int uT = lane >> 3, pT = lane & 7;
     const double muT = (pT + 1 < N) ? g.mu[N + pT + 1] : 1.0;
     const double* xrow = s_x + uT * 16;
+    double Vd[kLowRankMax] = {0, 0, 0, 0}, Vu[kLowRankMax] = {0, 0, 0, 0};
+    if constexpr (MOM) {
+#pragma unroll
+        for (int q = 0; q < kLowRankMax; ++q)
+            if (q < Rk) { Vd[q] = a.lrV[(size_t)q * D + tidc]; Vu[q] = a.lrV[(size_t)q * D + N + tidc]; }
+    }
+    auto jplain = [&](int t, const double (&V)[kLowRankMax]) __attribute__((always_inline)) {
+        double M[kLowRankMax];
+#pragma unroll
+        for (int q = 0; q < kLowRankMax; ++q) M[q] = q < Rk ? s_mom[t * Rk + q] : 0.0;
+        return lowrank_expand(M, V, Rk, t < slab0 ? ca_top : ca_bot);
+    };
     {
         const int m = tidc;
         const int vo = m * 8;
@@ -309,13 +353,21 @@
             Jprev = Jc[TC - 1];
             t0 += TC;
         };
-        auto chunk = [&](auto special_t, auto mode_t) __attribute__((always_inline)) {
+        auto chunk = [&](auto special_t, auto mode_t, auto plain_t) __attribute__((always_inline)) {
             const double* sp = ring + (size_t)slot_rd * SLOT + tid;
             slot_rd = slot_rd + 1 == NS ? 0 : slot_rd + 1;
             double Jc[TC], Ic[TC], Ec[TC];
 #pragma unroll
             for (int u = 0; u < TC; ++u) {
-                Jc[u] = sp[(0 * TC + u) * RS];
+                if constexpr (MOM && decltype(special_t)::value) {
+                    const int t = min(t0 + u, L - 1);
+                    const double js = sp[(0 * TC + u) * RS];
+                    Jc[u] = is_plain(t) ? jplain(t, Vd) : js;
+                } else if constexpr (MOM && decltype(plain_t)::value) {
+                    Jc[u] = jplain(t0 + u, Vd);
+                } else {
+                    Jc[u] = sp[(0 * TC + u) * RS];
+                }
                 Ec[u] = sp[(1 * TC + u) * RS];
                 Ic[u] = ACC ? sp[(2 * TC + u) * RS] : 0.0;
             }
@@ -325,13 +377,23 @@
         using M0 = std::integral_constant<int, 0>;
         using M1 = std::integral_constant<int, 1>;
         using M2 = std::integral_constant<int, 2>;
+#define SOSRT_RING_RUN(MODE_)                                                                   \
+    do {                                                                                        \
+        if constexpr (MOM) {                                                                    \
+            if (is_plain(t0)) {                                                                 \
+                for (; q < qe; ++q) chunk(std::false_type{}, MODE_{}, std::true_type{});        \
+                break;                                                                          \
+            }                                                                                   \
+        }                                                                                       \
+        for (; q < qe; ++q) chunk(std::false_type{}, MODE_{}, std::false_type{});               \
+    } while (0)
         while (q < NCH) {
             const int qe = q + plain_run(sp_dn, q);
             const int mode = (!wl || (nfx == 0 && !has_small)) ? 0 : ((!has_small && nfx <= 8 && sl[0] >= xb_dn) ? 1 : 2);
-            if (mode == 0) for (; q < qe; ++q) chunk(std::false_type{}, M0{});
-            else if (mode == 1) for (; q < qe; ++q) chunk(std::false_type{}, M1{});
-            else for (; q < qe; ++q) chunk(std::false_type{}, M2{});
-            if (q < NCH) { chunk(std::true_type{}, M2{}); ++q; }
+            if (mode == 0) SOSRT_RING_RUN(M0);
+            else if (mode == 1) SOSRT_RING_RUN(M1);
+            else SOSRT_RING_RUN(M2);
+            if (q < NCH) { chunk(std::true_type{}, M2{}, std::false_type{}); ++q; }
         }
     }
 
@@ -485,13 +547,21 @@
             Jnext = Jc[TC - 1];
             t0 -= TC;
         };
-        auto chunk = [&](auto special_t, auto mode_t) __attribute__((always_inline)) {
+        auto chunk = [&](auto special_t, auto mode_t, auto plain_t) __attribute__((always_inline)) {
             const double* sp = ring + (size_t)slot_rd * SLOT + tid;
             slot_rd = slot_rd + 1 == NS ? 0 : slot_rd + 1;
             double Jc[TC], Ic[TC], Ec[TC];
 #pragma unroll
             for (int u = 0; u < TC; ++u) {
-                Jc[u] = sp[(0 * TC + u) * RS];
+                if constexpr (MOM && decltype(special_t)::value) {
+                    const int t = max(t0 - u, 0);
+                    const double js = sp[(0 * TC + u) * RS];
+                    Jc[u] = is_plain(t) ? jplain(t, Vu) : js;
+                } else if constexpr (MOM && decltype(plain_t)::value) {
+                    Jc[u] = jplain(t0 - u, Vu);
+                } else {
+                    Jc[u] = sp[(0 * TC + u) * RS];
+                }
                 Ec[u] = sp[(1 * TC + u) * RS];
                 Ic[u] = ACC ? sp[(2 * TC + u) * RS] : 0.0;
             }
@@ -502,10 +572,11 @@
         using M1 = std::integral_constant<int, 1>;
         while (q < NQ) {
             const int qe = q + plain_run(sp_up, q - NCH);
-            if (!w0) for (; q < qe; ++q) chunk(std::false_type{}, M0{});
-            else for (; q < qe; ++q) chunk(std::false_type{}, M1{});
-            if (q < NQ) { chunk(std::true_type{}, M1{}); ++q; }
-        }
+            if (!w0) SOSRT_RING_RUN(M0);
+            else SOSRT_RING_RUN(M1);
+            if (q < NQ) { chunk(std::true_type{}, M1{}, std::false_type{}); ++q; }
+        }
+#undef SOSRT_RING_RUN
         if (w0 && notfound && lane == 0 && N - 3 <= 61) s_flag[1] = 1;
     }
     }
@@ -529,8 +600,16 @@
         }
     }
     if (s_flag[0]) {
-        const bool missing = redo_upward_sweep<ACC, SAVED, MZ>(L, N, RB, zr, s_hd, g.mu, rJ, rE, rIn, rI, rS, Bv, ring,
-                                                            rup_v, rup_i);
+        bool missing;
+        if constexpr (MOM) {
+            MomentRows pj{s_mom, Rk, slab0, slab1, ca_top, ca_bot, {0, 0, 0, 0}};
+#pragma unroll
+            for (int q = 0; q < kLowRankMax; ++q)
+                if (q < Rk) pj.V[q] = a.lrV[(size_t)q * D + N + tidc];
+            missing = redo_upward_sweep<ACC, SAVED, MZ>(L, N, RB, zr, s_hd, g.mu, rJ, rE, rIn, rI, rS, Bv, ring, rup_v, rup_i, pj);
+        } else {
+            missing = redo_upward_sweep<ACC, SAVED, MZ>(L, N, RB, zr, s_hd, g.mu, rJ, rE, rIn, rI, rS, Bv, ring, rup_v, rup_i);
+        }
         if (missing) {
             if (tid == 0) {
                 a.cv.status[b] = SOSRT_COL_INDEXERROR;
@@ -557,19 +636,22 @@
 }
 
 inline int ring_fixcap(const Grid& g) { return (int)(0.06 * g.N) + 1; }
-inline size_t ring_extra_doubles(const Grid& g, int nt, int nzcap = kRingZones) {
+inline size_t ring_extra_doubles(const Grid& g, int nt, int nzcap = kRingZones, int mom_rank = 0) {
     const int rs = g.N <= 128 ? 128 : 256, fc = nzcap * ring_fixcap(g) * kFixMaxSrc;
-    return (size_t)(rs > fc ? rs : fc) + nt / 64 + 2 + g.L + 1 + (size_t)g.nsmall * g.L + TC * 16 + 16 + (g.L + 63) / 64;
-}
+    return (size_t)(rs > fc ? rs : fc) + nt / 64 + 2 + g.L + 1 + (size_t)g.nsmall * g.L + TC * 16 + 16 + (g.L + 63) / 64 +
+           (size_t)mom_rank * g.L;
+}
+inline bool ring_moments(const TransportArgs& a) { return a.mom && a.accumulate && !a.saved && a.nzcap <= kRingZones; }
 
 template <int PIECES>
 void launch_p(hipStream_t s, dim3 grid, dim3 block, const TransportArgs& a, int NS) {
     const int nt = (int)block.x;
     const int narr = a.accumulate ? 3 : 2;
-    const size_t shm = ((size_t)NS * narr * TC * 128 * PIECES + ring_extra_doubles(a.g, nt, a.nzcap)) * sizeof(double);
-#define SOSRT_RING_LAUNCH_Z(ACC_, SAVED_, MZ_)                                                                 \
+    const bool mom = ring_moments(a);
+    const size_t shm = ((size_t)NS * narr * TC * 128 * PIECES + ring_extra_doubles(a.g, nt, a.nzcap, mom ? a.lr_rank : 0)) * sizeof(double);
+#define SOSRT_RING_LAUNCH_Z(ACC_, SAVED_, MZ_, ...)                                                            \
     do {                                                                                                       \
-        auto kern = k_transport_ring<ACC_, SAVED_, PIECES, MZ_>;                                               \
+        auto kern = k_transport_ring<ACC_, SAVED_, PIECES, MZ_, ##__VA_ARGS__>;                                \
         static PerDeviceOnce big_lds;                                                                                 \
         if (big_lds.first()) {                                                                                        \
             hipFuncSetAttribute(reinterpret_cast<const void*>(kern), hipFuncAttributeMaxDynamicSharedMemorySize, \
@@ -584,6 +666,7 @@
     } while (0)
     if (a.accumulate) {
         if (a.saved) SOSRT_RING_LAUNCH(true, true);
+        else if (mom) SOSRT_RING_LAUNCH_Z(true, false, false, true);
         else SOSRT_RING_LAUNCH(true, false);
     } else {
         SOSRT_RING_LAUNCH(false, false);
@@ -607,6 +690,25 @@
     const int nwc = (g.N + 63) / 64, pieces = g.N <= 128 ? 1 : 2;
     const size_t slot_bytes = (size_t)3 * TC * 128 * pieces * sizeof(double);
     return 2 * slot_bytes + ring_extra_doubles(g, (nwc + 4) * 64, nzcap < kRingZones ? kRingZones : nzcap) * sizeof(double) <= kRingLdsBytes;
+}
+
+bool transport_ring_moments_ok(const Grid& g, int rank, int slots) {
+    if (rank < 0 || rank > kLowRankMax || !transport_ring_ok(g)) return false;
+    const int nwc = (g.N + 63) / 64, pieces = g.N <= 128 ? 1 : 2, nt = (nwc + 2) * 64;
+    const size_t slot_bytes = (size_t)3 * TC * 128 * pieces * sizeof(double);
+    auto need = [&](int mom_rank, int* ns_out) {
+        const size_t extra = ring_extra_doubles(g, nt, kRingZones, mom_rank) * sizeof(double) + 16;
+        int NS = slots > 0 ? slots : g_ring_slots;
+        NS = NS < 2 ? 2 : NS;
+        while (NS > 2 && NS * slot_bytes + extra > kRingLdsBytes) --NS;
+        *ns_out = NS;
+        return NS * slot_bytes + extra;
+    };
+    auto per_cu = [](size_t bytes) { return (size_t)128 / ((bytes + 1279) / 1280); };
+    int ns0 = 0, ns1 = 0;
+    const size_t b0 = need(0, &ns0), b1 = need(rank, &ns1);
+    if (b1 > kRingLdsBytes || ns1 != ns0) return false;
+    return per_cu(b1) >= (per_cu(b0) < 2 ? per_cu(b0) : 2);
 }
 
 void launch_transport_ring(hipStream_t s, dim3 grid, const TransportArgs& a, int slots) {
@@ -617,7 +719,7 @@
     const int narr = a.accumulate ? 3 : 2;
     const dim3 block((nwc + 2) * 64);
     const size_t slot_bytes = (size_t)narr * TC * 128 * pieces * sizeof(double);
-    const size_t extra = ring_extra_doubles(a.g, (int)block.x, a.nzcap) * sizeof(double);
+    const size_t extra = ring_extra_doubles(a.g, (int)block.x, a.nzcap, ring_moments(a) ? a.lr_rank : 0) * sizeof(double);
     int NS = slots < 2 ? 2 : slots;
     while (NS > 2 && NS * slot_bytes + extra > kRingLdsBytes) --NS;
     if (pieces == 1) launch_p<1>(s, grid, block, a, NS);
diff --git a/sos-radiative-transfer_amd/csrc/transport_util.hpp b/sos-radiative-transfer_amd/csrc/transport_util.hpp
--- a/sos-radiative-transfer_amd/csrc/transport_util.hpp
+++ b/sos-radiative-transfer_amd/csrc/transport_util.hpp
@@ -261,11 +261,12 @@
 }
 
 constexpr int kRedoRows = 8;
-template <bool ACC, bool SAVED, bool MZ, int LDX = 0, int STX = 0>
+struct NoPlainRows { static constexpr bool any = false; };
+template <bool ACC, bool SAVED, bool MZ, int LDX = 0, int STX = 0, class PlainJ = NoPlainRows>
 __device__ SOSRT_HELPER_INLINE bool redo_upward_sweep(int L, int N, int RB, const ZoneRows<MZ>& zr, const double* s_hd,
                                   const double* __restrict__ gmu, __amdgpu_buffer_rsrc_t rJ, __amdgpu_buffer_rsrc_t rE,
                                   __amdgpu_buffer_rsrc_t rIn, __amdgpu_buffer_rsrc_t rI, __amdgpu_buffer_rsrc_t rS, double U0,
-                                  double* s_work, double& rup_v, double& rup_i) {
+                                  double* s_work, double& rup_v, double& rup_i, const PlainJ& pj = PlainJ()) {
     const int tid = threadIdx.x;
     double* s_row = s_work;
     int* s_kf = reinterpret_cast<int*>(s_work + 2 * (N + 2));
@@ -285,6 +286,7 @@
         for (int u = 0; u < kRedoRows; ++u) {
             const int t = max(t0 - u, 0);
             Jc[u] = bload_aux<LDX>(rJ, vo, t * RB);
+            if constexpr (PlainJ::any) { if (pj.plain(t)) Jc[u] = pj.value(t); }
             Ec[u] = bload(rE, vo, t * RB);
             xo[u] = bload_aux<LDX ? LDX : 1>(rIn, vo, t * RB);
             Io[u] = ACC ? bload_aux<LDX ? LDX : 1>(rI, vo, t * RB) : 0.0;
diff --git a/sos-radiative-transfer_amd/sosrt/_lib.py b/sos-radiative-transfer_amd/sosrt/_lib.py
--- a/sos-radiative-transfer_amd/sosrt/_lib.py
+++ b/sos-radiative-transfer_amd/sosrt/_lib.py
@@ -13,6 +13,7 @@
 PLAN_GEMM_DENSE, PLAN_GEMM_LIVE64, PLAN_GEMM_LIVE32, PLAN_GEMM_LIVE32_DEEP, PLAN_GEMM_LIVE16_REGS = 0, 1, 2, 3, 4
 PLAN_TRANSPORT_GENERAL, PLAN_TRANSPORT_FAST, PLAN_TRANSPORT_RING, PLAN_TRANSPORT_SCAN = 0, 1, 3, 4
 CONTRACT_F64, CONTRACT_F32, CONTRACT_F64_FULL, CONTRACT_F64_DENSE = 0, 1, 2, 3
+PLAN_FLAG_NEED_SMALL, PLAN_FLAG_SAVING, PLAN_FLAG_ATM_SETS = 1, 2, 4
 FIRST_ORDER_CODED, FIRST_ORDER_README = 0, 1
 PHASE_ISO, PHASE_RAYLEIGH, PHASE_HG, PHASE_TABLE = 0, 1, 2, 3
 MAX_MODES = 64
@@ -36,6 +37,9 @@
     "sosrt_phase_rank": (c_int, [c_void_p, _ip, POINTER(c_double), _ip]),
     "sosrt_set_order_loop": (c_int, [c_void_p, c_int]),
     "sosrt_order_loop_stats": (c_int, [c_void_p, _ip, _ip, POINTER(c_longlong)]),
+    "sosrt_set_source_moments": (c_int, [c_void_p, c_int]),
+    "sosrt_source_moments_stats": (c_int, [c_void_p, _ip]),
+    "sosrt_plan_source_moments": (c_int, [c_void_p, c_int, c_int, c_int, c_int, c_int, _ip]),
     "sosrt_plan_launch": (c_int, [c_void_p, c_int, c_int, c_int, c_int, c_int, _ip]),
     "sosrt_set_first_order": (c_int, [c_void_p, c_int]),
     "sosrt_set_grid": (c_int, [c_void_p, c_void_p]),
diff --git a/sos-radiative-transfer_amd/sosrt/solver.py b/sos-radiative-transfer_amd/sosrt/solver.py
--- a/sos-radiative-transfer_amd/sosrt/solver.py
+++ b/sos-radiative-transfer_amd/sosrt/solver.py
@@ -99,6 +99,14 @@
         a, b, c = ctypes.c_int(), ctypes.c_int(), ctypes.c_longlong()
         check(lib().sosrt_order_loop_stats(self._h, ctypes.byref(a), ctypes.byref(b), ctypes.byref(c) if column_orders else None))
         return (a.value, b.value, c.value) if column_orders else (a.value, b.value)
+
+    def set_source_moments(self, on=True):
+        check(lib().sosrt_set_source_moments(self._h, 1 if on else 0))
+
+    def source_moments_stats(self):
+        a = ctypes.c_int()
+        check(lib().sosrt_source_moments_stats(self._h, ctypes.byref(a)))
+        return a.value
 
     def phase_asymmetry(self):
         a, u = ctypes.c_double(), ctypes.c_int()
@@ -485,6 +493,15 @@
         keys = ("groups", "gemm", "tail_cols", "transport", "parts", "repair", "order_loop", "ol_parts", "ol_grid")
         return dict(zip(keys, list(out)))
 
+    def plan_source_moments(self, batch, live, surface="specular", zones=3, need_small=False, saving=False, atm_sets=False):
+        sf = {"none": _lib.SURFACE_NONE, "specular": _lib.SURFACE_SPECULAR, "lambertian": _lib.SURFACE_LAMBERTIAN,
+              "lambertian_readme": _lib.SURFACE_LAMBERTIAN_README}[surface]
+        flags = ((_lib.PLAN_FLAG_NEED_SMALL if need_small else 0) | (_lib.PLAN_FLAG_SAVING if saving else 0) |
+                 (_lib.PLAN_FLAG_ATM_SETS if atm_sets else 0))
+        out = ctypes.c_int()
+        check(lib().sosrt_plan_source_moments(self._h, int(batch), int(live), sf, int(zones), flags, ctypes.byref(out)))
+        return bool(out.value)
+
     def microbench(self, which):
         r = ctypes.c_double()
         check(lib().sosrt_microbench(self._h, int(which), ctypes.byref(r)))
```
